# medical-genomics-group/hydra

Hardware: AMD Instinct MI355X
Metric: Gibbs markers/sec/iter (higher is better)
Workload: dtype f64

## Files before the change

### hydra_amd/capi.py

```python
import ctypes as C
import os
import numpy as np

_HERE = os.path.dirname(os.path.abspath(__file__))
LIB_PATH = os.path.join(_HERE, "libhgibbs.so")

ABI_SYMBOLS = [
    "hgibbs_last_error", "hgibbs_version", "hgibbs_create", "hgibbs_destroy", "hgibbs_comm_unique_id",
    "hgibbs_comm_init", "hgibbs_comm_init_external", "hgibbs_p2p_export", "hgibbs_p2p_import", "hgibbs_load_bed", "hgibbs_synth_bed", "hgibbs_dims", "hgibbs_get_bed",
    "hgibbs_marker_stats", "hgibbs_set_residual", "hgibbs_get_residual", "hgibbs_reduce_eps", "hgibbs_add_scalar",
    "hgibbs_update_marker", "hgibbs_dot_marker", "hgibbs_set_covariates", "hgibbs_cov_dot", "hgibbs_cov_update",
    "hydra_chain_set_covariates", "hydra_chain_gamma", "hgibbs_set_components", "hydra_chain_restore",
    "hydra_rng_to_boost_words", "hydra_rng_from_boost_words", "hgibbs_set_model", "hgibbs_set_beta", "hgibbs_get_beta",
    "hgibbs_beta_sqnorm", "hgibbs_sweep", "hgibbs_set_option", "hgibbs_last_sweep_stats", "hgibbs_stream_ceiling", "hgibbs_debug_times", "hgibbs_resident_trace", "hydra_chain_create",
    "hydra_chain_destroy", "hydra_chain_iterate", "hydra_chain_state", "hydra_chain_csv_line", "hydra_chain_order",
    "hydra_chain_last_nnz", "hgibbs_score", "hgibbs_last_score_ms", "hgibbs_ld", "hgibbs_last_ld_ms",
    "hgibbs_marker_dots", "hgibbs_last_marker_dots_ms", "hgibbs_king", "hgibbs_king_pairs", "hgibbs_king_pairs_get", "hgibbs_last_king_ms",
    "hgibbs_pca", "hgibbs_last_pca_ms",
    "hgibbs_grand_seed", "hgibbs_grand_next", "hgibbs_ars_sample", "hgibbs_w_init", "hgibbs_w_marker_stats", "hgibbs_w_set_model",
    "hgibbs_w_reduce", "hgibbs_w_refresh_vi", "hgibbs_w_get_vi", "hgibbs_w_marker_sums", "hgibbs_w_sweep", "hgibbs_w_last_sweep_stats", "hgibbs_w_ars_device_probe",
    "hgibbs_w_get_beta", "hgibbs_w_set_beta", "hydraw_chain_create", "hydraw_chain_destroy", "hydraw_chain_set_covariates",
    "hydraw_chain_reseed_ars", "hydraw_chain_iterate", "hydraw_chain_state", "hydraw_chain_gamma", "hydraw_chain_order",
    "hydraw_chain_last_nnz", "hydraw_chain_csv_line", "hydraw_chain_restore",
]


class RngState(C.Structure):
    _fields_ = [("x", C.c_uint32 * 624), ("idx", C.c_uint32)]


class SweepStats(C.Structure):
    _fields_ = [("launches", C.c_uint64), ("nnz_updates", C.c_uint64), ("device_ms", C.c_double),
                ("kernel_ms_avg", C.c_double), ("carried_columns", C.c_uint64), ("working_launches", C.c_uint64),
                ("accepted_markers", C.c_uint64), ("streamed_columns", C.c_uint64), ("tiles_per_workgroup_min", C.c_uint32),
                ("tiles_per_workgroup_max", C.c_uint32), ("engine", C.c_uint32), ("walker", C.c_uint32), ("eps_sum_drift", C.c_double),
                ("rounds", C.c_uint64), ("events", C.c_uint64), ("advances", C.c_uint64), ("chunks", C.c_uint64), ("refolds", C.c_uint64), ("pivots", C.c_uint64), ("predicted", C.c_uint64), ("shader_mhz", C.c_double),
                ("ticks", C.c_uint64 * 16), ("refill", C.c_uint32), ("reserved_", C.c_uint32)]


class PcaReport(C.Structure):
    _fields_ = [("iters_run", C.c_int32), ("m_used", C.c_uint32), ("ritz_change", C.c_double), ("resid", C.c_double * 32)]


class RestartState(C.Structure):
    _fields_ = [("iteration", C.c_uint32), ("sigmaE", C.c_double), ("mu", C.c_double),
                ("sigmaG", C.POINTER(C.c_double)), ("estPi", C.POINTER(C.c_double)), ("beta", C.POINTER(C.c_double)),
                ("components", C.POINTER(C.c_int32)), ("eps", C.POINTER(C.c_double)), ("order", C.POINTER(C.c_int32)),
                ("gamma", C.POINTER(C.c_double)), ("xI", C.POINTER(C.c_int32)), ("rng", RngState)]


class GrandState(C.Structure):
    _fields_ = [("r", C.c_int32 * 31), ("f", C.c_int32), ("b", C.c_int32)]


class WSweepStats(C.Structure):
    _fields_ = [("launches", C.c_uint64), ("nnz_updates", C.c_uint64), ("ars_draws", C.c_uint64), ("ars_evals", C.c_uint64),
                ("device_ms", C.c_double), ("sums_kernel_ms", C.c_double)]


class WModelDesc(C.Structure):
    _fields_ = [("seed", C.c_uint32), ("shuffle", C.c_int32), ("G", C.c_int32), ("K", C.c_int32),
                ("groups", C.POINTER(C.c_int32)), ("mS", C.POINTER(C.c_double)), ("quad_points", C.c_int32)]


class WRestartState(C.Structure):
    _fields_ = [("iteration", C.c_uint32), ("mu", C.c_double), ("alpha", C.c_double), ("sigmaG", C.POINTER(C.c_double)),
                ("pi", C.POINTER(C.c_double)), ("beta", C.POINTER(C.c_double)), ("components", C.POINTER(C.c_int32)),
                ("eps", C.POINTER(C.c_double)), ("order", C.POINTER(C.c_int32)), ("gamma", C.POINTER(C.c_double)),
                ("xI", C.POINTER(C.c_int32)), ("rng", RngState), ("ars_seed", C.c_uint32)]


LOGDENS_FN = C.CFUNCTYPE(C.c_double, C.c_double, C.c_void_p)


class ModelDesc(C.Structure):
    _fields_ = [("seed", C.c_uint32), ("shuffle", C.c_int32), ("G", C.c_int32), ("K", C.c_int32),
                ("groups", C.POINTER(C.c_int32)), ("mS", C.POINTER(C.c_double))]


ALLREDUCE_FN = C.CFUNCTYPE(C.c_int, C.c_void_p, C.c_void_p, C.c_size_t, C.c_int)


class HgError(RuntimeError):
    pass


_lib = None


def lib():
    global _lib
    if _lib is not None:
        return _lib
    path = os.environ.get("HGIBBS_LIB", LIB_PATH)
    if not os.path.exists(path):
        raise HgError("%s not built: run `python -c 'import __graft_entry__ as g; g.build()'` "
                      "(there is no CPU fallback)" % path)
    L = C.CDLL(path)
    vp, dp, ip = C.c_void_p, C.POINTER(C.c_double), C.POINTER(C.c_int32)
    u8p, u64p, u32p = C.POINTER(C.c_uint8), C.POINTER(C.c_uint64), C.POINTER(C.c_uint32)
    L.hgibbs_last_error.restype = C.c_char_p
    L.hgibbs_create.argtypes = [C.c_int, C.POINTER(vp)]
    L.hgibbs_destroy.argtypes = [vp]
    L.hgibbs_comm_unique_id.argtypes = [C.c_void_p]
    L.hgibbs_comm_init.argtypes = [vp, C.c_int, C.c_int, C.c_void_p]
    L.hgibbs_comm_init_external.argtypes = [vp, C.c_int, C.c_int, ALLREDUCE_FN, C.c_void_p]
    L.hgibbs_p2p_export.argtypes = [vp, C.c_void_p]
    L.hgibbs_p2p_import.argtypes = [vp, C.c_void_p]
    L.hgibbs_load_bed.argtypes = [vp, u8p, C.c_uint64, C.c_uint32, C.c_uint32, u8p, C.c_uint32, C.c_uint32, C.c_uint32]
    L.hgibbs_synth_bed.argtypes = [vp, C.c_uint32, C.c_uint32, C.c_uint32, C.c_uint32, C.c_uint64, C.c_double]
    L.hgibbs_dims.argtypes = [vp, u32p, u32p, u32p, u32p]
    L.hgibbs_get_bed.argtypes = [vp, C.c_uint32, C.c_uint32, u8p, C.c_uint64]
    L.hgibbs_marker_stats.argtypes = [vp, dp, dp, u64p, u64p, u64p]
    L.hgibbs_set_residual.argtypes = [vp, dp]
    L.hgibbs_get_residual.argtypes = [vp, dp]
    L.hgibbs_reduce_eps.argtypes = [vp, dp, dp]
    L.hgibbs_add_scalar.argtypes = [vp, C.c_double]
    L.hgibbs_update_marker.argtypes = [vp, C.c_uint32, C.c_double]
    L.hgibbs_dot_marker.argtypes = [vp, C.c_uint32, dp]
    L.hgibbs_set_covariates.argtypes = [vp, dp, C.c_int]
    L.hgibbs_cov_dot.argtypes = [vp, C.c_int, C.c_double, dp]
    L.hgibbs_cov_update.argtypes = [vp, C.c_int, C.c_double]
    L.hydra_chain_set_covariates.argtypes = [vp, dp, C.c_int]
    L.hydra_chain_gamma.argtypes = [vp, dp, ip]
    L.hgibbs_set_components.argtypes = [vp, ip]
    L.hydra_chain_restore.argtypes = [vp, C.POINTER(RestartState)]
    L.hydra_rng_to_boost_words.argtypes = [C.POINTER(RngState), u32p]
    L.hydra_rng_from_boost_words.argtypes = [u32p, C.POINTER(RngState)]
    L.hgibbs_set_model.argtypes = [vp, C.c_int, C.c_int, ip, dp, dp]
    L.hgibbs_set_beta.argtypes = [vp, dp]
    L.hgibbs_get_beta.argtypes = [vp, dp, ip, dp]
    L.hgibbs_beta_sqnorm.argtypes = [vp, dp]
    L.hgibbs_sweep.argtypes = [vp, ip, C.c_double, dp, dp, u8p, C.POINTER(RngState), ip, u64p]
    L.hgibbs_set_option.argtypes = [vp, C.c_char_p, C.c_int64]
    L.hgibbs_last_sweep_stats.argtypes = [vp, C.POINTER(SweepStats)]
    L.hgibbs_stream_ceiling.argtypes = [vp, C.c_uint64, C.c_int, dp]
    L.hgibbs_debug_times.argtypes = [vp, C.POINTER(C.c_uint64)]
    L.hgibbs_resident_trace.argtypes = [vp, C.POINTER(C.c_uint64), C.c_uint64]
    L.hydra_chain_create.argtypes = [vp, C.POINTER(ModelDesc), dp, C.POINTER(vp)]
    L.hydra_chain_destroy.argtypes = [vp]
    L.hydra_chain_iterate.argtypes = [vp]
    L.hydra_chain_state.argtypes = [vp, dp, dp, dp, dp, ip, ip, C.POINTER(RngState)]
    L.hydra_chain_csv_line.argtypes = [vp, C.c_uint32, C.c_char_p, C.c_size_t]
    L.hydra_chain_order.argtypes = [vp]
    L.hydra_chain_order.restype = ip
    L.hydra_chain_last_nnz.argtypes = [vp]
    gp = C.POINTER(GrandState)
    L.hgibbs_grand_seed.argtypes = [gp, C.c_uint32]
    L.hgibbs_grand_seed.restype = None
    L.hgibbs_grand_next.argtypes = [gp]
    L.hgibbs_grand_next.restype = C.c_int32
    L.hgibbs_ars_sample.argtypes = [dp, C.c_double, C.c_double, LOGDENS_FN, C.c_void_p, gp, dp, ip]
    L.hgibbs_w_init.argtypes = [vp, ip]
    L.hgibbs_w_marker_stats.argtypes = [vp, dp, dp, dp]
    L.hgibbs_w_set_model.argtypes = [vp, C.c_int, C.c_int, ip, dp, C.c_int]
    L.hgibbs_w_reduce.argtypes = [vp, C.c_int, C.c_int, C.c_double, C.c_double, C.c_double, dp]
    L.hgibbs_w_refresh_vi.argtypes = [vp, C.c_double]
    L.hgibbs_w_get_vi.argtypes = [vp, dp, dp]
    L.hgibbs_w_marker_sums.argtypes = [vp, C.c_uint32, C.c_double, C.c_double, dp, dp, dp]
    L.hgibbs_w_sweep.argtypes = [vp, ip, C.c_double, dp, dp, C.c_double, C.POINTER(RngState), gp, ip, dp, u64p]
    L.hgibbs_w_last_sweep_stats.argtypes = [vp, C.POINTER(WSweepStats)]
    L.hgibbs_w_ars_device_probe.argtypes = [vp, dp, C.c_double, C.c_double, C.c_uint32, C.c_uint32, dp, dp, dp]
    L.hgibbs_w_get_beta.argtypes = [vp, dp, ip]
    L.hgibbs_w_set_beta.argtypes = [vp, dp, ip]
    L.hydraw_chain_create.argtypes = [vp, C.POINTER(WModelDesc), dp, ip, C.POINTER(vp)]
    L.hydraw_chain_destroy.argtypes = [vp]
    L.hydraw_chain_set_covariates.argtypes = [vp, dp, C.c_int]
    L.hydraw_chain_reseed_ars.argtypes = [vp, C.c_uint32]
    L.hydraw_chain_iterate.argtypes = [vp]
    L.hydraw_chain_state.argtypes = [vp, dp, dp, dp, dp, ip, ip, C.POINTER(RngState), gp]
    L.hydraw_chain_gamma.argtypes = [vp, dp, ip]
    L.hydraw_chain_order.argtypes = [vp]
    L.hydraw_chain_order.restype = C.POINTER(C.c_int32)
    L.hydraw_chain_last_nnz.argtypes = [vp]
    L.hydraw_chain_last_nnz.restype = C.c_uint64
    L.hydraw_chain_csv_line.argtypes = [vp, C.c_uint32, C.c_char_p, C.c_size_t]
    L.hydraw_chain_restore.argtypes = [vp, C.POINTER(WRestartState)]
    L.hydra_chain_last_nnz.restype = C.c_uint64
    L.hgibbs_score.argtypes = [vp, C.c_int, dp, dp, dp]
    L.hgibbs_last_score_ms.argtypes = [vp, dp]
    L.hgibbs_ld.argtypes = [vp, C.c_uint32, C.c_uint32, C.c_uint32, dp, C.POINTER(C.c_int64)]
    L.hgibbs_last_ld_ms.argtypes = [vp, dp]
    L.hgibbs_marker_dots.argtypes = [vp, C.c_uint32, C.c_uint32, C.c_int, dp, dp, dp]
    L.hgibbs_last_marker_dots_ms.argtypes = [vp, dp]
    L.hgibbs_king.argtypes = [vp, C.c_uint32, C.c_uint32, C.c_uint32, C.c_uint32, C.POINTER(C.c_int32)]
    L.hgibbs_king_pairs.argtypes = [vp, C.c_double, C.POINTER(C.c_uint64)]
    L.hgibbs_king_pairs_get.argtypes = [vp, C.POINTER(C.c_uint32), C.POINTER(C.c_int32), dp]
    L.hgibbs_last_king_ms.argtypes = [vp, dp]
    L.hgibbs_pca.argtypes = [vp, C.c_int, C.c_int, C.c_int, C.c_double, dp, C.c_uint64, dp, dp, dp, C.POINTER(PcaReport)]
    L.hgibbs_last_pca_ms.argtypes = [vp, dp]
    _lib = L
    return L


def check(rc):
    if rc != 0:
        raise HgError(lib().hgibbs_last_error().decode(errors="replace"))


def _dp(a):
    return a.ctypes.data_as(C.POINTER(C.c_double))


def _ip(a):
    return a.ctypes.data_as(C.POINTER(C.c_int32))


def _u8(a):
    return a.ctypes.data_as(C.POINTER(C.c_uint8))


def _u64(a):
    return a.ctypes.data_as(C.POINTER(C.c_uint64))


class Device:

    def __init__(self, device_id=0):
        self.L = lib()
        self.h = C.c_void_p()
        check(self.L.hgibbs_create(device_id, C.byref(self.h)))
        self.M = self.n_local = self.n_global = self.row_begin = 0
        self.G = self.K = 0

    def close(self):
        if self.h:
            self.L.hgibbs_destroy(self.h)
            self.h = C.c_void_p()

    def __del__(self):
        try:
            self.close()
        except Exception:
            pass

    @staticmethod
    def unique_id():
        buf = (C.c_uint8 * 128)()
        check(lib().hgibbs_comm_unique_id(buf))
        return bytes(buf)

    def comm_init(self, nranks, rank, uid):
        buf = (C.c_uint8 * 128).from_buffer_copy(uid) if uid else None
        check(self.L.hgibbs_comm_init(self.h, nranks, rank, buf))

    def comm_init_external(self, nranks, rank, allreduce):
        def cb(user, buf, count, dtype):
            try:
                ty = C.c_double if dtype == 0 else C.c_uint64
                arr = np.ctypeslib.as_array(C.cast(buf, C.POINTER(ty)), shape=(count,))
                allreduce(arr)
                return 0
            except Exception:
                import traceback
                traceback.print_exc()
                return 1
        self._cb = ALLREDUCE_FN(cb)
        check(self.L.hgibbs_comm_init_external(self.h, nranks, rank, self._cb, None))

    def p2p_export(self):
        buf = (C.c_uint8 * 64)()
        check(self.L.hgibbs_p2p_export(self.h, buf))
        return bytes(buf)

    def p2p_import(self, handles):
        blob = b"".join(handles)
        buf = (C.c_uint8 * len(blob)).from_buffer_copy(blob)
        check(self.L.hgibbs_p2p_import(self.h, buf))

    def _dims(self):
        a, b, c, d = C.c_uint32(), C.c_uint32(), C.c_uint32(), C.c_uint32()
        check(self.L.hgibbs_dims(self.h, C.byref(a), C.byref(b), C.byref(c), C.byref(d)))
        self.n_global, self.n_local, self.M, self.row_begin = a.value, b.value, c.value, d.value

    def load_bed(self, bed, n_total, keep=None, row_begin=0, row_end=None, n_global=None):
        bed = np.ascontiguousarray(bed, dtype=np.uint8)
        M, stride = bed.shape
        kept = int(np.count_nonzero(keep)) if keep is not None else n_total
        if row_end is None:
            row_end = kept
        if n_global is None:
            n_global = kept
        kp = _u8(np.ascontiguousarray(keep, dtype=np.uint8)) if keep is not None else None
        check(self.L.hgibbs_load_bed(self.h, _u8(bed), stride, n_total, M, kp, row_begin, row_end, n_global))
        self._dims()

    def synth_bed(self, n_global, M, seed=42, missing_rate=0.0, row_begin=0, row_end=None):
        if row_end is None:
            row_end = n_global
        check(self.L.hgibbs_synth_bed(self.h, n_global, M, row_begin, row_end, seed, missing_rate))
        self._dims()

    def get_bed(self, m0=0, mcount=None):
        if mcount is None:
            mcount = self.M - m0
        out = np.zeros((mcount, (self.n_local + 3) // 4), dtype=np.uint8)
        check(self.L.hgibbs_get_bed(self.h, m0, mcount, _u8(out), out.shape[1]))
        return out

    def marker_stats(self):
        M = self.M
        mave, mstd = np.zeros(M), np.zeros(M)
        n1, n2, nm = (np.zeros(M, dtype=np.uint64) for _ in range(3))
        check(self.L.hgibbs_marker_stats(self.h, _dp(mave), _dp(mstd), _u64(n1), _u64(n2), _u64(nm)))
        return mave, mstd, n1, n2, nm

    def set_residual(self, eps):
        eps = np.ascontiguousarray(eps, dtype=np.float64)
        assert eps.shape[0] == self.n_local
        check(self.L.hgibbs_set_residual(self.h, _dp(eps)))

    def get_residual(self):
        out = np.zeros(self.n_local)
        check(self.L.hgibbs_get_residual(self.h, _dp(out)))
        return out

    def reduce_eps(self):
        s, q = C.c_double(), C.c_double()
        check(self.L.hgibbs_reduce_eps(self.h, C.byref(s), C.byref(q)))
        return s.value, q.value

    def add_scalar(self, c):
        check(self.L.hgibbs_add_scalar(self.h, c))

    def set_covariates(self, X):
        X = np.ascontiguousarray(X, dtype=np.float64)
        assert X.shape[0] == self.n_local
        check(self.L.hgibbs_set_covariates(self.h, _dp(X), X.shape[1]))

    def update_marker(self, marker, dbeta):
        check(self.L.hgibbs_update_marker(self.h, marker, dbeta))

    def dot_marker(self, marker):
        v = C.c_double()
        check(self.L.hgibbs_dot_marker(self.h, marker, C.byref(v)))
        return v.value

    def set_model(self, groups, cVa, cVaI):
        cVa = np.ascontiguousarray(cVa, dtype=np.float64)
        cVaI = np.ascontiguousarray(cVaI, dtype=np.float64)
        G, K = cVa.shape
        g = _ip(np.ascontiguousarray(groups, dtype=np.int32)) if groups is not None else None
        check(self.L.hgibbs_set_model(self.h, G, K, g, _dp(cVa), _dp(cVaI)))
        self.G, self.K = G, K

    def set_beta(self, beta):
        beta = np.ascontiguousarray(beta, dtype=np.float64)
        check(self.L.hgibbs_set_beta(self.h, _dp(beta)))

    def get_beta(self):
        beta, comp, acum = np.zeros(self.M), np.zeros(self.M, dtype=np.int32), np.zeros(self.M)
        check(self.L.hgibbs_get_beta(self.h, _dp(beta), _ip(comp), _dp(acum)))
        return beta, comp, acum

    def beta_sqnorm(self):
        out = np.zeros(self.G)
        check(self.L.hgibbs_beta_sqnorm(self.h, _dp(out)))
        return out

    def stream_ceiling(self, nbytes=2 << 30, reps=10):
        out = C.c_double()
        check(self.L.hgibbs_stream_ceiling(self.h, nbytes, reps, C.byref(out)))
        return out.value

    def set_option(self, name, value):
        check(self.L.hgibbs_set_option(self.h, name.encode(), int(value)))

    def score(self, a, o):
        a = np.ascontiguousarray(np.atleast_2d(a), dtype=np.float64)
        o = np.ascontiguousarray(np.atleast_2d(o), dtype=np.float64)
        if a.shape != o.shape or a.shape[1] != self.M:
            raise ValueError("a and o must both be (S, %d)" % self.M)
        out = np.zeros((self.n_local, a.shape[0]))
        check(self.L.hgibbs_score(self.h, a.shape[0], _dp(a), _dp(o), _dp(out)))
        return out

    def last_score_ms(self):
        v = C.c_double()
        check(self.L.hgibbs_last_score_ms(self.h, C.byref(v)))
        return v.value

    def ld(self, W, m0=0, count=None, r=True, sums=True):
        if count is None:
            count = self.M - m0
        rr = np.zeros((count, W)) if r else None
        ss = np.zeros((count, W, 4), dtype=np.int64) if sums else None
        check(self.L.hgibbs_ld(self.h, m0, count, W, _dp(rr) if r else None,
                               ss.ctypes.data_as(C.POINTER(C.c_int64)) if sums else None))
        return rr, ss

    def last_ld_ms(self):
        v = C.c_double()
        check(self.L.hgibbs_last_ld_ms(self.h, C.byref(v)))
        return v.value

    def marker_dots(self, U, m0=0, count=None, raw=False):
        U = np.ascontiguousarray(np.atleast_2d(U), dtype=np.float64)
        if U.shape[1] != self.n_local:
            raise ValueError("U must be (K, %d)" % self.n_local)
        if count is None:
            count = self.M - m0
        K = U.shape[0]
        out = np.zeros((count, K))
        rr = np.zeros((count, K, 2)) if raw else None
        check(self.L.hgibbs_marker_dots(self.h, m0, count, K, _dp(U), _dp(out), _dp(rr) if raw else None))
        return (out, rr) if raw else out

    def last_marker_dots_ms(self):
        v = C.c_double()
        check(self.L.hgibbs_last_marker_dots_ms(self.h, C.byref(v)))
        return v.value

    def king(self, a0=0, acount=None, b0=0, bcount=None):
        if acount is None:
            acount = self.n_local - a0
        if bcount is None:
            bcount = self.n_local - b0
        out = np.zeros((acount, bcount, 5), dtype=np.int32)
        check(self.L.hgibbs_king(self.h, a0, acount, b0, bcount, out.ctypes.data_as(C.POINTER(C.c_int32))))
        return out

    def king_pairs(self, cutoff):
        n = C.c_uint64()
        check(self.L.hgibbs_king_pairs(self.h, float(cutoff), C.byref(n)))
        P = n.value
        ab = np.zeros((P, 2), dtype=np.uint32)
        cnt = np.zeros((P, 5), dtype=np.int32)
        kin = np.zeros(P)
        check(self.L.hgibbs_king_pairs_get(self.h, ab.ctypes.data_as(C.POINTER(C.c_uint32)), cnt.ctypes.data_as(C.POINTER(C.c_int32)), _dp(kin)))
        return ab, cnt, kin

    def last_king_ms(self):
        v = C.c_double()
        check(self.L.hgibbs_last_king_ms(self.h, C.byref(v)))
        return v.value

    def pca(self, K, L=None, iters=20, tol=1e-10, Q0=None, seed=1, loadings=False):
        if L is None:
            L = min(32, (K + 8 + 7) // 8 * 8)
        q = None
        if Q0 is not None:
            q = np.ascontiguousarray(Q0, dtype=np.float64)
            if q.shape != (L, self.n_local):
                raise ValueError("Q0 must be (%d, %d)" % (L, self.n_local))
        kk = max(int(K), 0)
        val = np.zeros(kk)
        pcs = np.zeros((kk, self.n_local))
        ld = np.zeros((kk, self.M)) if loadings else None
        rep = PcaReport()
        check(self.L.hgibbs_pca(self.h, int(K), int(L), int(iters), float(tol), _dp(q) if q is not None else None, int(seed) & (2 ** 64 - 1),
                                _dp(val), _dp(pcs), _dp(ld) if loadings else None, C.byref(rep)))
        return val, pcs, ld, {"iters_run": rep.iters_run, "m_used": rep.m_used, "ritz_change": rep.ritz_change,
                              "resid": np.array(rep.resid[:kk], dtype=np.float64)}

    def last_pca_ms(self):
        v = (C.c_double * 4)()
        check(self.L.hgibbs_last_pca_ms(self.h, v))
        return [v[i] for i in range(4)]

    def debug_times(self):
        t = (C.c_uint64 * 48)()
        check(self.L.hgibbs_debug_times(self.h, t))
        return [int(x) for x in t]

    def sweep(self, order, sigmaE, sigmaG, estPi, adaV, rng):
        order = np.ascontiguousarray(order, dtype=np.int32)
        sigmaG = np.ascontiguousarray(sigmaG, dtype=np.float64)
        estPi = np.ascontiguousarray(estPi, dtype=np.float64)
        adaV = np.ascontiguousarray(adaV, dtype=np.uint8)
        cass = np.zeros((self.G, self.K), dtype=np.int32)
        nnz = C.c_uint64()
        check(self.L.hgibbs_sweep(self.h, _ip(order), float(sigmaE), _dp(sigmaG), _dp(estPi), _u8(adaV), C.byref(rng),
                                  _ip(cass), C.byref(nnz)))
        return cass, nnz.value

    def resident_trace(self):
        out = np.zeros((10, 4096), dtype=np.uint64)
        check(self.L.hgibbs_resident_trace(self.h, out.ctypes.data_as(C.POINTER(C.c_uint64)), out.size))
        return out

    def sweep_stats(self):
        s = SweepStats()
        check(self.L.hgibbs_last_sweep_stats(self.h, C.byref(s)))
        return {"launches": s.launches, "nnz_updates": s.nnz_updates, "device_ms": s.device_ms,
                "kernel_ms_avg": s.kernel_ms_avg, "carried_columns": s.carried_columns, "working_launches": s.working_launches,
                "accepted_markers": s.accepted_markers, "streamed_columns": s.streamed_columns,
                "tiles_per_workgroup_min": s.tiles_per_workgroup_min, "tiles_per_workgroup_max": s.tiles_per_workgroup_max,
                "engine": s.engine, "walker": s.walker, "refill": s.refill, "eps_sum_drift": s.eps_sum_drift, "rounds": s.rounds, "events": s.events,
                "advances": s.advances, "chunks": s.chunks, "refolds": s.refolds, "pivots": s.pivots, "predicted": s.predicted, "shader_mhz": s.shader_mhz, "ticks": list(s.ticks)}


class Chain:

    def __init__(self, dev, y, mS=None, groups=None, seed=1222, shuffle=1):
        self.dev = dev
        self.L = dev.L
        if mS is None:
            mS = np.array([[0.0, 0.0001, 0.001, 0.01]])
        self.mS = np.ascontiguousarray(mS, dtype=np.float64)
        self.G, self.K = self.mS.shape
        self.groups = None if groups is None else np.ascontiguousarray(groups, dtype=np.int32)
        y = np.ascontiguousarray(y, dtype=np.float64)
        assert y.shape[0] == dev.n_global
        d = ModelDesc(seed, shuffle, self.G, self.K, _ip(self.groups) if self.groups is not None else None, _dp(self.mS))
        self.h = C.c_void_p()
        check(self.L.hydra_chain_create(dev.h, C.byref(d), _dp(y), C.byref(self.h)))
        dev.G, dev.K = self.G, self.K

    def __del__(self):
        try:
            if self.h:
                self.L.hydra_chain_destroy(self.h)
        except Exception:
            pass

    def set_covariates(self, X):
        X = np.ascontiguousarray(X, dtype=np.float64)
        assert X.shape[0] == self.dev.n_global
        self.C = X.shape[1]
        check(self.L.hydra_chain_set_covariates(self.h, _dp(X), self.C))

    def gamma(self):
        g, xi = np.zeros(self.C), np.zeros(self.C, dtype=np.int32)
        check(self.L.hydra_chain_gamma(self.h, _dp(g), _ip(xi)))
        return g, xi

    def iterate(self):
        check(self.L.hydra_chain_iterate(self.h))

    def state(self):
        G, K = self.G, self.K
        sE, mu = C.c_double(), C.c_double()
        sG, pi = np.zeros(G), np.zeros((G, K))
        m0, cass = np.zeros(G, dtype=np.int32), np.zeros((G, K), dtype=np.int32)
        rng = RngState()
        check(self.L.hydra_chain_state(self.h, C.byref(sE), C.byref(mu), _dp(sG), _dp(pi), _ip(m0), _ip(cass), C.byref(rng)))
        return {"sigmaE": sE.value, "mu": mu.value, "sigmaG": sG, "estPi": pi, "m0": m0, "cass": cass,
                "rng_x": np.array(rng.x, dtype=np.uint32), "rng_idx": int(rng.idx)}

    def order(self):
        return np.ctypeslib.as_array(self.L.hydra_chain_order(self.h), shape=(self.dev.M,)).copy()

    def rng_words(self):
        rng = RngState()
        check(self.L.hydra_chain_state(self.h, None, None, None, None, None, None, C.byref(rng)))
        out = np.zeros(624, dtype=np.uint32)
        check(self.L.hydra_rng_to_boost_words(C.byref(rng), out.ctypes.data_as(C.POINTER(C.c_uint32))))
        return out

    def restore(self, iteration, sigmaE, mu, sigmaG, estPi, beta, components, eps, order, rng_words, gamma=None, xI=None):
        f64 = lambda a: np.ascontiguousarray(a, dtype=np.float64)
        i32 = lambda a: np.ascontiguousarray(a, dtype=np.int32)
        keep = [f64(sigmaG), f64(estPi), f64(beta), i32(components), f64(eps), i32(order)]
        st = RestartState()
        st.iteration, st.sigmaE, st.mu = iteration, sigmaE, mu
        st.sigmaG, st.estPi, st.beta = _dp(keep[0]), _dp(keep[1]), _dp(keep[2])
        st.components, st.eps, st.order = _ip(keep[3]), _dp(keep[4]), _ip(keep[5])
        if gamma is not None:
            keep += [f64(gamma), i32(xI)]
            st.gamma, st.xI = _dp(keep[6]), _ip(keep[7])
        w = np.ascontiguousarray(rng_words, dtype=np.uint32)
        check(self.L.hydra_rng_from_boost_words(w.ctypes.data_as(C.POINTER(C.c_uint32)), C.byref(st.rng)))
        check(self.L.hydra_chain_restore(self.h, C.byref(st)))

    def last_nnz(self):
        return int(self.L.hydra_chain_last_nnz(self.h))

    def csv_line(self, it):
        buf = C.create_string_buffer(50000)
        n = self.L.hydra_chain_csv_line(self.h, it, buf, 50000)
        return buf.raw[:n].decode()


def ars_sample(logdens, xinit, xl, xr, grand):
    L = lib()
    cb = LOGDENS_FN(lambda x, _d: logdens(x))
    xi = np.ascontiguousarray(xinit, dtype=np.float64)
    out, ne = C.c_double(0.0), C.c_int(0)
    err = L.hgibbs_ars_sample(_dp(xi), xl, xr, cb, None, C.byref(grand), C.byref(out), C.byref(ne))
    return err, out.value, ne.value


class BwOps:

    def __init__(self, dev, failure):
        self.dev, self.L = dev, dev.L
        self.fail = np.ascontiguousarray(failure, dtype=np.int32)
        assert self.fail.shape[0] == dev.n_global
        check(self.L.hgibbs_w_init(dev.h, _ip(self.fail)))

    def marker_stats(self):
        M = self.dev.M
        a, b, c = np.zeros(M), np.zeros(M), np.zeros(M)
        check(self.L.hgibbs_w_marker_stats(self.dev.h, _dp(a), _dp(b), _dp(c)))
        return a, b, c

    def set_model(self, mS, groups=None, quad=9):
        mS = np.ascontiguousarray(mS, dtype=np.float64)
        self.G, self.K = mS.shape
        g = None if groups is None else np.ascontiguousarray(groups, dtype=np.int32)
        check(self.L.hgibbs_w_set_model(self.dev.h, self.G, self.K, _ip(g) if g is not None else None, _dp(mS), quad))

    def reduce(self, kind, col=0, p0=0.0, p1=0.0, p2=0.0):
        out = C.c_double()
        check(self.L.hgibbs_w_reduce(self.dev.h, kind, col, p0, p1, p2, C.byref(out)))
        return out.value

    def refresh_vi(self, alpha):
        check(self.L.hgibbs_w_refresh_vi(self.dev.h, alpha))

    def get_vi(self):
        v, s = np.zeros(self.dev.n_local), C.c_double()
        check(self.L.hgibbs_w_get_vi(self.dev.h, _dp(v), C.byref(s)))
        return v, s.value

    def marker_sums(self, marker, beta_old, alpha):
        a, b, c = C.c_double(), C.c_double(), C.c_double()
        check(self.L.hgibbs_w_marker_sums(self.dev.h, marker, beta_old, alpha, C.byref(a), C.byref(b), C.byref(c)))
        return a.value, b.value, c.value

    def get_beta(self):
        b, c = np.zeros(self.dev.M), np.zeros(self.dev.M, dtype=np.int32)
        check(self.L.hgibbs_w_get_beta(self.dev.h, _dp(b), _ip(c)))
        return b, c

    def sweep_stats(self):
        st = WSweepStats()
        check(self.L.hgibbs_w_last_sweep_stats(self.dev.h, C.byref(st)))
        return {f: getattr(st, f) for f, _ in st._fields_}


class BwChain:

    def __init__(self, dev, y, failure, mS=None, groups=None, seed=1222, shuffle=1, quad=9):
        self.dev, self.L = dev, dev.L
        if mS is None:
            mS = np.array([[0.0, 0.001, 0.01]])
        self.mS = np.ascontiguousarray(mS, dtype=np.float64)
        self.G, self.K = self.mS.shape
        self.groups = None if groups is None else np.ascontiguousarray(groups, dtype=np.int32)
        y = np.ascontiguousarray(y, dtype=np.float64)
        self.fail = np.ascontiguousarray(failure, dtype=np.int32)
        assert y.shape[0] == dev.n_global and self.fail.shape[0] == dev.n_global
        d = WModelDesc(seed, shuffle, self.G, self.K, _ip(self.groups) if self.groups is not None else None, _dp(self.mS), quad)
        self.h = C.c_void_p()
        self.C = 0
        check(self.L.hydraw_chain_create(dev.h, C.byref(d), _dp(y), _ip(self.fail), C.byref(self.h)))

    def __del__(self):
        try:
            if self.h:
                self.L.hydraw_chain_destroy(self.h)
        except Exception:
            pass

    def set_covariates(self, X):
        X = np.ascontiguousarray(X, dtype=np.float64)
        self.C = X.shape[1]
        check(self.L.hydraw_chain_set_covariates(self.h, _dp(X), self.C))

    def reseed_ars(self, seed):
        check(self.L.hydraw_chain_reseed_ars(self.h, seed))

    def rng_words(self):
        st = self.state()
        rng = RngState()
        rng.x[:] = list(st["rng_x"])
        rng.idx = st["rng_idx"]
        out = np.zeros(624, dtype=np.uint32)
        check(self.L.hydra_rng_to_boost_words(C.byref(rng), out.ctypes.data_as(C.POINTER(C.c_uint32))))
        return out

    def restore(self, iteration, mu, alpha, sigmaG, pi, beta, components, eps, order, rng_words, ars_seed, gamma=None, xI=None):
        f64 = lambda a: np.ascontiguousarray(a, dtype=np.float64)
        i32 = lambda a: np.ascontiguousarray(a, dtype=np.int32)
        keep = [f64(sigmaG), f64(pi), f64(beta), i32(components), f64(eps), i32(order)]
        st = WRestartState()
        st.iteration, st.mu, st.alpha, st.ars_seed = iteration, mu, alpha, ars_seed
        st.sigmaG, st.pi, st.beta = _dp(keep[0]), _dp(keep[1]), _dp(keep[2])
        st.components, st.eps, st.order = _ip(keep[3]), _dp(keep[4]), _ip(keep[5])
        if gamma is not None:
            keep += [f64(gamma), i32(xI)]
            st.gamma, st.xI = _dp(keep[6]), _ip(keep[7])
        w = np.ascontiguousarray(rng_words, dtype=np.uint32)
        check(self.L.hydra_rng_from_boost_words(w.ctypes.data_as(C.POINTER(C.c_uint32)), C.byref(st.rng)))
        check(self.L.hydraw_chain_restore(self.h, C.byref(st)))

    def iterate(self):
        check(self.L.hydraw_chain_iterate(self.h))

    def state(self):
        G, K = self.G, self.K
        mu, alpha = C.c_double(), C.c_double()
        sG, pi = np.zeros(G), np.zeros((G, K))
        m0, cass = np.zeros(G, dtype=np.int32), np.zeros((G, K), dtype=np.int32)
        rng, gr = RngState(), GrandState()
        check(self.L.hydraw_chain_state(self.h, C.byref(mu), C.byref(alpha), _dp(sG), _dp(pi), _ip(m0), _ip(cass), C.byref(rng), C.byref(gr)))
        return {"mu": mu.value, "alpha": alpha.value, "sigmaG": sG, "pi": pi, "m0": m0, "cass": cass,
                "rng_x": np.array(rng.x, dtype=np.uint32), "rng_idx": int(rng.idx), "grand": gr}

    def gamma(self):
        g, xi = np.zeros(self.C), np.zeros(self.C, dtype=np.int32)
        check(self.L.hydraw_chain_gamma(self.h, _dp(g), _ip(xi)))
        return g, xi

    def beta(self):
        b, c = np.zeros(self.dev.M), np.zeros(self.dev.M, dtype=np.int32)
        check(self.L.hgibbs_w_get_beta(self.dev.h, _dp(b), _ip(c)))
        return b, c

    def order(self):
        return np.ctypeslib.as_array(self.L.hydraw_chain_order(self.h), shape=(self.dev.M,)).copy()

    def last_nnz(self):
        return int(self.L.hydraw_chain_last_nnz(self.h))

    def sweep_stats(self):
        st = WSweepStats()
        check(self.L.hgibbs_w_last_sweep_stats(self.dev.h, C.byref(st)))
        return {f: getattr(st, f) for f, _ in st._fields_}

    def csv_line(self, it):
        buf = C.create_string_buffer(50000)
        n = self.L.hydraw_chain_csv_line(self.h, it, buf, 50000)
        return buf.raw[:n].decode()
```

### hydra_amd/csrc/hg_rng.h

```cpp
#pragma once

#include <math.h>
#include <stdint.h>
#if !defined(__HIP_DEVICE_COMPILE__)
#include <vector>
#endif

#include "hg_zig_tables.h"

#if defined(__HIP__)
#include <hip/hip_runtime.h>
#define HG_HD __host__ __device__ __forceinline__
#else
#define HG_HD inline
#endif

namespace hg {

constexpr int MT_N = 624;
constexpr int MT_M = 397;

HG_HD uint32_t mt_temper(uint32_t z)
{
    z ^= (z >> 11);
    z ^= (z << 7) & 0x9d2c5680u;
    z ^= (z << 15) & 0xefc60000u;
    z ^= (z >> 18);
    return z;
}

HG_HD uint32_t mt_mix(uint32_t cur, uint32_t nxt, uint32_t far)
{
    uint32_t y = (cur & 0x80000000u) | (nxt & 0x7fffffffu);
    return far ^ (y >> 1) ^ ((y & 1u) ? 0x9908b0dfu : 0u);
}

struct Mt {
    uint32_t* x;
    uint32_t idx;
    HG_HD void seed(uint32_t s)
    {
        x[0] = s;
        for (uint32_t i = 1; i < MT_N; ++i) x[i] = 1812433253u * (x[i - 1] ^ (x[i - 1] >> 30)) + i;
        idx = MT_N;
    }
    HG_HD void twist()
    {
        for (int i = 0; i < MT_N; ++i) x[i] = mt_mix(x[i], x[(i + 1) % MT_N], x[(i + MT_M) % MT_N]);
        idx = 0;
    }
    HG_HD uint32_t next()
    {
        if (idx >= MT_N) twist();
        return mt_temper(x[idx++]);
    }
};

struct ZigTables {
    const double* nx;
    const double* ny;
    const double* ex;
    const double* ey;
};

template <class Gen>
HG_HD double unif01(Gen& g)
{
    return (double)g.next() * (1.0 / 4294967296.0);
}

template <class Gen>
HG_HD double int_float_pair(Gen& g, int& bucket)
{
    uint32_t u1 = g.next();
    bucket = (int)(u1 & 0xffu);
    double r = (double)(u1 >> 8) * (1.0 / 16777216.0);
    uint32_t u2 = g.next();
    r += (double)(u2 & 0x1fffffffu);
    r *= (1.0 / 536870912.0);
    return r;
}

template <class Gen, class Tab>
HG_HD double unit_exponential(Gen& g, const Tab& t)
{
    double shift = 0.0;
    for (;;) {
        int i;
        double r = int_float_pair(g, i);
        double x = r * t.ex[i];
        if (x < t.ex[i + 1]) return shift + x;
        if (i == 0) {
            shift += t.ex[1];
        } else {
            double y01 = unif01(g);
            double y = t.ey[i] + y01 * (t.ey[i + 1] - t.ey[i]);
            double y_above_ubound = (t.ex[i] - t.ex[i + 1]) * y01 - (t.ex[i] - x);
            double y_above_lbound = y - (t.ey[i + 1] + (t.ex[i + 1] - x) * t.ey[i + 1]);
            if (y_above_ubound < 0 && (y_above_lbound < 0 || y < exp(-x))) return x + shift;
        }
    }
}

template <class Gen, class Tab>
HG_HD double unit_normal(Gen& g, const Tab& t)
{
    for (;;) {
        int i;
        double r = int_float_pair(g, i);
        int sign = (i & 1) * 2 - 1;
        i >>= 1;
        double x = r * t.nx[i];
        if (x < t.nx[i + 1]) return x * sign;
        if (i == 0) {
            const double tail_start = t.nx[1];
            for (;;) {
                double xt = unit_exponential(g, t) / tail_start;
                double yt = unit_exponential(g, t) / 1.0;
                if (2 * yt > xt * xt) return (xt + tail_start) * sign;
            }
        }
        double y01 = unif01(g);
        double y = t.ny[i] + y01 * (t.ny[i + 1] - t.ny[i]);
        double y_above_ubound, y_above_lbound;
        if (t.nx[i] >= 1) {
            y_above_ubound = (t.nx[i] - t.nx[i + 1]) * y01 - (t.nx[i] - x);
            y_above_lbound = y - (t.ny[i] + (t.nx[i] - x) * t.ny[i] * t.nx[i]);
        } else {
            y_above_lbound = (t.nx[i] - t.nx[i + 1]) * y01 - (t.nx[i] - x);
            y_above_ubound = y - (t.ny[i] + (t.nx[i] - x) * t.ny[i] * t.nx[i]);
        }
        if (y_above_ubound < 0 && (y_above_lbound < 0 || y < exp(-(x * x / 2)))) return x * sign;
    }
}

template <class Gen, class Tab>
HG_HD double norm_rng_sd(Gen& g, const Tab& t, double mean, double sigma)
{
    return unit_normal(g, t) * sigma + mean;
}

inline ZigTables host_tables() { return ZigTables{HG_ZIG_NORMAL_X, HG_ZIG_NORMAL_Y, HG_ZIG_EXP_X, HG_ZIG_EXP_Y}; }

inline double norm_rng(Mt& g, double mean, double sigma2)
{
    ZigTables t = host_tables();
    return norm_rng_sd(g, t, mean, sqrt(sigma2));
}

inline double rgamma(Mt& g, double alpha, double beta)
{
    ZigTables t = host_tables();
    if (alpha == 1.0) {
        return unit_exponential(g, t) / 1.0 * beta;
    } else if (alpha > 1.0) {
        const double pi = 3.14159265358979323846;
        for (;;) {
            double y = tan(pi * unif01(g));
            double x = sqrt(2.0 * alpha - 1.0) * y + alpha - 1.0;
            if (x <= 0.0) continue;
            if (unif01(g) > (1.0 + y * y) * exp((alpha - 1.0) * log(x / (alpha - 1.0)) - sqrt(2.0 * alpha - 1.0) * y))
                continue;
            return x * beta;
        }
    } else {
        const double p = exp(1.0) / (alpha + exp(1.0));
        for (;;) {
            double u = unif01(g);
            double y = unit_exponential(g, t) / 1.0;
            double x, q;
            if (u < p) {
                x = exp(-y / alpha);
                q = p * exp(-x);
            } else {
                x = 1.0 + y;
                q = p + (1.0 - p) * pow(x, alpha - 1.0);
            }
            if (u >= q) continue;
            return x * beta;
        }
    }
}

inline double inv_gamma_rng(Mt& g, double shape, double scale) { return 1.0 / rgamma(g, shape, 1.0 / scale); }
inline double inv_scaled_chisq_rng(Mt& g, double dof, double scale) { return inv_gamma_rng(g, 0.5 * dof, 0.5 * dof * scale); }
inline double beta_rng(Mt& g, double a, double b)
{
    double x = rgamma(g, a, 1.0);
    double y = rgamma(g, b, 1.0);
    return x / (x + y);
}
inline void dirichlet_rng(Mt& g, const double* alpha, int len, double* out)
{
    double s = 0.0;
    for (int i = 0; i < len; ++i) out[i] = rgamma(g, alpha[i], 1.0);
    for (int i = 0; i < len; ++i) s += out[i];
    for (int i = 0; i < len; ++i) out[i] /= s;
}

inline void mt_to_boost_words(const uint32_t* x, uint32_t idx, uint32_t* out )
{
    const uint32_t UP = 0x80000000u, LO = 0x7fffffffu, A = 0x9908b0dfu;
    if (idx > (uint32_t)MT_N) idx = MT_N;
    for (uint32_t j = 0; j < idx; ++j) out[j + MT_N - idx] = x[j];
    if (idx == (uint32_t)MT_N) return;
    auto unmix = [&](uint32_t y) {
        if (y & UP) return ((y ^ A) << 1) | 1u;
        return y << 1;
    };
    std::vector<uint32_t> w(MT_N + 1, 0u);
    w[MT_N] = x[0];
    uint32_t have_low_of = MT_N;
    (void)have_low_of;
    for (int k = MT_N - 1; k >= (int)idx - 1 && k >= 0; --k) {
        const uint32_t far = (k + MT_M < MT_N) ? w[k + MT_M] : x[k + MT_M - MT_N];
        const uint32_t y = unmix(x[k] ^ far);
        if (k + 1 < MT_N) w[k + 1] = (w[k + 1] & UP) | (y & LO);
        w[k] = (w[k] & LO) | (y & UP);
    }
    for (uint32_t k = idx; k < (uint32_t)MT_N; ++k) out[k - idx] = w[k];
}

template <class T>
inline void shuffle_libstdcxx6(T* first, size_t n, Mt& g)
{
    const uint64_t urngrange = 0xffffffffull;
    for (size_t i = 1; i < n; ++i) {
        const uint64_t uerange = (uint64_t)i + 1;
        const uint64_t scaling = urngrange / uerange, past = uerange * scaling;
        uint64_t ret;
        do ret = g.next();
        while (ret >= past);
        ret /= scaling;
        const T t = first[i];
        first[i] = first[ret];
        first[ret] = t;
    }
}

}
```

### hydra_amd/csrc/hgibbs.hip

```cpp
#include <hip/hip_runtime.h>
#include <rccl/rccl.h>

#include <algorithm>
#include <atomic>
#include <chrono>
#include <thread>
#include <cmath>
#include <cstdarg>
#include <cstdio>
#include <cstdlib>
#include <cstring>
#include <string>
#include <vector>

#include "../../include/hgibbs.h"
#include "hg_kernels.h"
#include "hg_sweep.hip.h"
#include "hg_resident.hip.h"

using namespace hg;

static thread_local std::string g_err;

static int fail(const char* fmt, ...)
{
    char buf[1024];
    va_list ap;
    va_start(ap, fmt);
    vsnprintf(buf, sizeof buf, fmt, ap);
    va_end(ap);
    g_err = buf;
    return 1;
}

#define HIP_TRY(expr)                                                                          \
    do {                                                                                       \
        hipError_t e_ = (expr);                                                                \
        if (e_ != hipSuccess) return fail("%s:%d %s -> %s", __FILE__, __LINE__, #expr, hipGetErrorString(e_)); \
    } while (0)

#define NCCL_TRY(expr)                                                                          \
    do {                                                                                        \
        ncclResult_t r_ = (expr);                                                               \
        if (r_ != ncclSuccess) return fail("%s:%d %s -> %s", __FILE__, __LINE__, #expr, ncclGetErrorString(r_)); \
    } while (0)

extern "C" void hgibbs_set_error_(const char* msg) { g_err = msg; }

struct BwState;
static void bw_free(BwState* b);

struct hgibbs_ctx {
    int device = 0;
    int num_cu = 256;
    BwState* bw = nullptr;
    hipStream_t stream = nullptr;
    hipEvent_t ev0 = nullptr, ev1 = nullptr;

    int nranks = 1, rank = 0;
    ncclComm_t comm = nullptr;
    hgibbs_allreduce_fn ext_fn = nullptr;
    void* ext_user = nullptr;
    unsigned char* mbox = nullptr;
    void* peer_base[MAX_RANKS] = {};
    bool p2p_ready = false, p2p_enabled = true;
    uint64_t batch_seq = 0;

    uint32_t n_global = 0, n_local = 0, n_pad = 0, M = 0, row_begin = 0;
    uint64_t stride = 0;
    uint8_t* bed = nullptr;
    double* eps[2] = {nullptr, nullptr};
    uint32_t eps_cur = 0;
    double *mave = nullptr, *mstd = nullptr;
    unsigned long long* counts = nullptr;
    bool have_stats = false;
    bool any_missing = false;
    int gram_missing = -1;

    double* covX = nullptr;
    int C = 0;

    int G = 0, K = 0;
    int32_t* groups = nullptr;
    std::vector<int32_t> groups_host;
    std::vector<double> cVa, cVaI;
    double* beta = nullptr;
    int32_t* comp = nullptr;
    double* acum = nullptr;

    int32_t* order = nullptr;
    uint8_t* adaV = nullptr;
    double *s_mave = nullptr, *s_mstd = nullptr, *s_bold = nullptr;
    int32_t* s_ga = nullptr;
    uint32_t* pred = nullptr;
    uint32_t* pred_cnt = nullptr;
    unsigned long long* dbg = nullptr;
    bool debug_timing = false;
    bool w_kernel_timing = false;
    int32_t* cass = nullptr;
    double* tables = nullptr;
    uint32_t* mt = nullptr;
    double* zig = nullptr;
    SweepDesc* desc = nullptr;
    SweepDesc* desc_host = nullptr;
    double* partials = nullptr;
    double* totals = nullptr;
    double* carry = nullptr;
    double* ahead_raw = nullptr;
    double* apartials = nullptr;
    uint32_t* aticket = nullptr;
    int ahead = -1;
    int carry_on = -1;
    uint32_t* ticket = nullptr;
    double* sums = nullptr;
    double* scratch = nullptr;
    size_t scratch_n = 0;
    double* scratch_host = nullptr;
    double* beta_host = nullptr;

    uint32_t batch = 0;
    uint32_t cols_per_group = 4;
    int chunk = 0;
    uint32_t slices = 0;
    uint32_t ext_limit = 256;
    uint32_t max_seg = 0;
    bool gram = true;
    bool use_graph = false;
    bool force_split = false;

    int engine = 0;
    bool res_all_ada = false;
    unsigned long long res_sweep_id = 0;
    bool engine_pinned = false;
    uint32_t window = 0;
    uint32_t res_cus = 0;
    int res_walker = 0;
    bool res_attr_set[20] = {};
    bool res_dead = false;
    uint32_t res_probed_w = 0;
    unsigned long long res_probe_id = 0;
    bool res_not_resident = false;
    int res_early = 24;
    int res_announce = 1;
    int res_wend = 1;
    int res_walker2_ranks = 1;
    double eps_abs_bound = 0.0;
    int res_refill = 0;
    int res_pivots = 0;
    unsigned char* res_acc = nullptr;
    ResMsg* res_msg = nullptr;
    ResState* res_state = nullptr;
    ResState* res_state_host = nullptr;
    ResParams* res_params = nullptr;
    ResParams* res_params_host = nullptr;
    unsigned long long* res_progress = nullptr;
    unsigned long long* res_progress_host = nullptr;
    hipStream_t aux_stream = nullptr;
    unsigned long long* res_trace = nullptr;
    double res_timeout_s = 2.0;
    double res_deadline_s = 0.0;

    hgibbs_sweep_stats stats{};
    int score_sp = 0;
    int score_ranges = 0;
    double score_ms = 0.0;
    int ld_split = 0;
    double ld_ms = 0.0;
    int mdots_split = 0;
    double mdots_ms = 0.0;
    int king_split = 0;
    double king_ms = 0.0;
    double pca_ms[5] = {0, 0, 0, 0, 0};
    std::vector<uint32_t> king_ab;
    std::vector<int32_t> king_counts;
    std::vector<double> king_kin;
};

static int ensure_scratch(hgibbs_ctx* h, size_t n)
{
    if (h->scratch_n >= n) return 0;
    if (h->scratch) HIP_TRY(hipFree(h->scratch));
    HIP_TRY(hipMalloc(&h->scratch, n * sizeof(double)));
    h->scratch_n = n;
    return 0;
}

static constexpr size_t RES_GACC_BYTES = (size_t)2 * RS_NSH * RS_GROW * 4, RES_RACC_BYTES = (size_t)RS_RSH * RS_RB * 8, RES_RCNT_BYTES = (size_t)RS_RSH * RS_CROW * 4, RES_PACC_BYTES = (size_t)RS_RSH * RS_RB * 2 * 8;
static constexpr size_t RES_RACC2_OFF = RES_GACC_BYTES + RES_RACC_BYTES + RES_RCNT_BYTES + RES_PACC_BYTES, RES_GACC64_BYTES = (size_t)2 * RS_NSH * RS_GROW * 8;
static constexpr size_t RES_ACC_BYTES = RES_RACC2_OFF + RES_RACC_BYTES + RES_GACC64_BYTES;
static constexpr size_t MBOX_DATA_BYTES = (size_t)2 * MAX_RANKS * ROWS_CAP * sizeof(double);
static constexpr size_t MBOX_BATCH_BYTES = MBOX_DATA_BYTES + (size_t)2 * MAX_RANKS * sizeof(unsigned long long);
static constexpr size_t MBOX_RES_OFF = (MBOX_BATCH_BYTES + 4095) / 4096 * 4096;
static constexpr size_t MBOX_BYTES = MBOX_RES_OFF + RX_BYTES;

static int bulk_allreduce(hgibbs_ctx* h, void* dptr, size_t count, int dtype)
{
    if (h->nranks <= 1 && !h->comm) return 0;
    if (h->comm) {
        NCCL_TRY(ncclAllReduce(dptr, dptr, count, dtype == 0 ? ncclDouble : ncclUint64, ncclSum, h->comm, h->stream));
        return 0;
    }
    if (!h->ext_fn) return fail("multi-rank handle without a transport: call hgibbs_comm_init or hgibbs_comm_init_external");
    std::vector<unsigned char> buf(count * 8);
    HIP_TRY(hipMemcpyAsync(buf.data(), dptr, buf.size(), hipMemcpyDeviceToHost, h->stream));
    HIP_TRY(hipStreamSynchronize(h->stream));
    if (h->ext_fn(h->ext_user, buf.data(), count, dtype)) return fail("external all-reduce callback failed");
    HIP_TRY(hipMemcpyAsync(dptr, buf.data(), buf.size(), hipMemcpyHostToDevice, h->stream));
    HIP_TRY(hipStreamSynchronize(h->stream));
    return 0;
}

namespace {

__host__ __device__ inline uint64_t mix64(uint64_t z)
{
    z += 0x9e3779b97f4a7c15ull;
    z = (z ^ (z >> 30)) * 0xbf58476d1ce4e5b9ull;
    z = (z ^ (z >> 27)) * 0x94d049bb133111ebull;
    return z ^ (z >> 31);
}

__global__ void k_synth_bed(uint8_t* bed, uint64_t stride, uint32_t n_local, uint32_t row_begin, uint32_t marker0,
                            uint64_t seed, uint32_t miss_thr)
{
    const uint32_t marker = marker0 + blockIdx.y;
    const uint64_t b = (uint64_t)blockIdx.x * blockDim.x + threadIdx.x;
    if (b >= stride) return;
    const uint32_t up = (uint32_t)(mix64(seed ^ (0xA5A5A5A5ull + (uint64_t)marker * 0x100000001b3ull)) >> 32);
    const double p = 0.01 + 0.49 * ((double)up * (1.0 / 4294967296.0));
    const double q0 = (1.0 - p) * (1.0 - p);
    const double q1 = q0 + 2.0 * p * (1.0 - p);
    const uint32_t t0 = (uint32_t)(q0 * 4294967296.0);
    const uint32_t t1 = (uint32_t)(q1 * 4294967296.0);
    uint32_t byte = 0;
    for (int s = 0; s < 4; ++s) {
        const uint64_t il = b * 4 + s;
        uint32_t code = GC_MISS;
        if (il < n_local) {
            const uint64_t ig = (uint64_t)row_begin + il;
            const uint64_t hsh = mix64(seed + (uint64_t)marker * 0x9E3779B1ull + ig * 0xD1B54A32D192ED03ull);
            const uint32_t ug = (uint32_t)(hsh >> 32), um = (uint32_t)hsh;
            if (um < miss_thr) code = GC_MISS;
            else code = (ug < t0) ? GC_G0 : ((ug < t1) ? GC_G1 : GC_G2);
        }
        byte |= code << (2 * s);
    }
    bed[(uint64_t)marker * stride + b] = (uint8_t)byte;
}

__global__ void k_fix_padding(uint8_t* bed, uint64_t stride, uint32_t n_local, uint32_t M)
{
    const uint32_t marker = blockIdx.x * blockDim.x + threadIdx.x;
    if (marker >= M) return;
    const uint32_t bfirst = n_local >> 2;
    if ((n_local & 3u) && bfirst < stride) {
        uint8_t v = bed[(uint64_t)marker * stride + bfirst];
        for (uint32_t s = n_local & 3u; s < 4; ++s) v = (uint8_t)((v & ~(3u << (2 * s))) | (1u << (2 * s)));
        bed[(uint64_t)marker * stride + bfirst] = v;
    }
}

__global__ void k_recode_bed(uint32_t* __restrict__ bed, uint64_t ndwords)
{
    const uint64_t stride = (uint64_t)gridDim.x * blockDim.x;
    for (uint64_t i = (uint64_t)blockIdx.x * blockDim.x + threadIdx.x; i < ndwords; i += stride) bed[i] = recode_plink_to_device(bed[i]);
}

__global__ void k_compact_bed(const uint8_t* __restrict__ src, uint64_t src_stride, const uint32_t* __restrict__ src_idx,
                              uint8_t* __restrict__ dst, uint64_t dst_stride, uint32_t n_local, uint32_t mcount)
{
    const uint32_t marker = blockIdx.y;
    const uint64_t b = (uint64_t)blockIdx.x * blockDim.x + threadIdx.x;
    if (b >= dst_stride || marker >= mcount) return;
    uint32_t byte = 0;
    for (int s = 0; s < 4; ++s) {
        const uint64_t il = b * 4 + s;
        uint32_t code = 1u;
        if (il < n_local) {
            const uint32_t i = src_idx[il];
            code = (src[(uint64_t)marker * src_stride + (i >> 2)] >> (2 * (i & 3u))) & 3u;
        }
        byte |= code << (2 * s);
    }
    dst[(uint64_t)marker * dst_stride + b] = (uint8_t)byte;
}

__global__ __launch_bounds__(BLOCK) void k_counts(const uint8_t* __restrict__ bed, uint64_t stride, uint32_t n_pad,
                                                  uint32_t n_local, unsigned long long* __restrict__ counts, uint32_t M)
{
    __shared__ unsigned int sh[3][BLOCK_WAVES];
    const uint32_t marker = blockIdx.x;
    const uint32_t* col = reinterpret_cast<const uint32_t*>(bed + (uint64_t)marker * stride);
    const uint32_t nw = (uint32_t)(stride >> 2);
    unsigned int c1 = 0, c2 = 0, cm = 0;
    for (uint32_t i = threadIdx.x; i < nw; i += BLOCK) {
        uint32_t m1, m2, mm;
        code_masks(col[i], m1, m2, mm);
        c1 += __popc(m1);
        c2 += __popc(m2);
        cm += __popc(mm);
    }
    for (int off = 32; off >= 1; off >>= 1) {
        c1 += __shfl_xor(c1, off, 64);
        c2 += __shfl_xor(c2, off, 64);
        cm += __shfl_xor(cm, off, 64);
    }
    const int lane = threadIdx.x & 63, wave = threadIdx.x >> 6;
    if (lane == 0) {
        sh[0][wave] = c1;
        sh[1][wave] = c2;
        sh[2][wave] = cm;
    }
    __syncthreads();
    if (threadIdx.x == 0) {
        unsigned long long t1 = 0, t2 = 0, tm = 0;
        for (int w = 0; w < BLOCK_WAVES; ++w) {
            t1 += sh[0][w];
            t2 += sh[1][w];
            tm += sh[2][w];
        }
        counts[3ull * marker] = t1;
        counts[3ull * marker + 1] = t2;
        counts[3ull * marker + 2] = tm - (unsigned long long)(n_pad - n_local);
    }
}

__global__ void k_stats(const unsigned long long* __restrict__ counts, uint32_t N, double* mave, double* mstd, uint32_t M)
{
    const uint32_t i = blockIdx.x * blockDim.x + threadIdx.x;
    if (i >= M) return;
    const double n1 = (double)counts[3ull * i], n2 = (double)counts[3ull * i + 1], nm = (double)counts[3ull * i + 2];
    const double dN = (double)N;
    const double av = (n1 + 2.0 * n2) / (dN - nm);
    const double tmp1 = n1 * (1.0 - av) * (1.0 - av);
    const double tmp2 = n2 * (2.0 - av) * (2.0 - av);
    const unsigned long long n0 = (unsigned long long)N - counts[3ull * i] - counts[3ull * i + 1] - counts[3ull * i + 2];
    const double tmp0 = (double)n0 * (0.0 - av) * (0.0 - av);
    mave[i] = av;
    mstd[i] = sqrt((double)(N - 1) / (tmp0 + tmp1 + tmp2));
}

__global__ void k_gather_meta(const int32_t* __restrict__ order, const double* __restrict__ mave, const double* __restrict__ mstd,
                              const double* __restrict__ beta, const int32_t* __restrict__ groups, const uint8_t* __restrict__ adaV,
                              const unsigned long long* __restrict__ counts, double* s_mave, double* s_mstd, double* s_bold, int32_t* s_ga, uint32_t M)
{
    const uint32_t j = blockIdx.x * blockDim.x + threadIdx.x;
    if (j >= M) return;
    const int m = order[j];
    s_mave[j] = mave[m];
    s_mstd[j] = mstd[m];
    s_bold[j] = beta[m];
    s_ga[j] = groups[m] | (adaV[m] ? 0x40000000 : 0) | (counts[3ull * m + 2] ? 0x20000000 : 0);
}

constexpr uint32_t PRED_CHUNK = 4096;
__global__ __launch_bounds__(256) void k_pred_count(const double* __restrict__ s_bold, uint32_t M, uint32_t* cnt)
{
    __shared__ uint32_t wsum[4];
    const uint32_t base = blockIdx.x * PRED_CHUNK;
    uint32_t n = 0;
    for (uint32_t i = 0; i < PRED_CHUNK / 256; ++i) {
        const uint32_t j = base + i * 256 + threadIdx.x;
        n += (uint32_t)__popcll(__ballot(j < M && s_bold[j] != 0.0));
    }
    if ((threadIdx.x & 63) == 0) wsum[threadIdx.x >> 6] = n;
    __syncthreads();
    if (threadIdx.x == 0) cnt[blockIdx.x] = wsum[0] + wsum[1] + wsum[2] + wsum[3];
}
__global__ __launch_bounds__(1024) void k_pred_scan(uint32_t* cnt, uint32_t nchunk)
{
    __shared__ uint32_t tot[1024];
    const uint32_t per = (nchunk + 1023u) / 1024u, lo = threadIdx.x * per;
    uint32_t s = 0;
    for (uint32_t i = lo; i < lo + per && i < nchunk; ++i) s += cnt[i];
    tot[threadIdx.x] = s;
    __syncthreads();
    if (threadIdx.x == 0) {
        uint32_t run = 0;
        for (int t = 0; t < 1024; ++t) {
            const uint32_t v = tot[t];
            tot[t] = run;
            run += v;
        }
        cnt[nchunk] = run;
    }
    __syncthreads();
    uint32_t run = tot[threadIdx.x];
    for (uint32_t i = lo; i < lo + per && i < nchunk; ++i) {
        const uint32_t v = cnt[i];
        cnt[i] = run;
        run += v;
    }
}
__global__ __launch_bounds__(256) void k_pred_scatter(const double* __restrict__ s_bold, uint32_t M, const uint32_t* __restrict__ cnt, uint32_t nchunk, uint32_t* pred)
{
    __shared__ uint32_t wsum[4];
    const uint32_t base = blockIdx.x * PRED_CHUNK;
    const int lane = threadIdx.x & 63, wave = threadIdx.x >> 6;
    uint32_t run = cnt[blockIdx.x];
    for (uint32_t i = 0; i < PRED_CHUNK / 256; ++i) {
        const uint32_t j = base + i * 256 + threadIdx.x;
        const bool f = j < M && s_bold[j] != 0.0;
        const unsigned long long m = __ballot(f);
        __syncthreads();
        if (lane == 0) wsum[wave] = (uint32_t)__popcll(m);
        __syncthreads();
        uint32_t before = 0;
        for (int w = 0; w < wave; ++w) before += wsum[w];
        if (f) pred[run + before + (uint32_t)__popcll(m & ((1ull << lane) - 1ull))] = j;
        run += wsum[0] + wsum[1] + wsum[2] + wsum[3];
    }
    if (blockIdx.x == 0 && threadIdx.x < 16) pred[cnt[nchunk] + threadIdx.x] = 0xffffffffu;
}

__global__ void k_set_eps(double* eps, const double* __restrict__ src, uint32_t n_local, uint32_t n_pad)
{
    const uint32_t i = blockIdx.x * blockDim.x + threadIdx.x;
    if (i >= n_pad) return;
    eps[eps_pos(i)] = (i < n_local) ? src[i] : 0.0;
}

__global__ void k_get_eps(const double* __restrict__ eps, double* dst, uint32_t n_local)
{
    const uint32_t i = blockIdx.x * blockDim.x + threadIdx.x;
    if (i >= n_local) return;
    dst[i] = eps[eps_pos(i)];
}

__global__ void k_add_scalar(double* eps, double c, uint32_t n_local, uint32_t n_pad)
{
    const uint32_t i = blockIdx.x * blockDim.x + threadIdx.x;
    if (i >= n_local) return;
    const uint32_t p = eps_pos(i);
    eps[p] = eps[p] + c;
}

__global__ __launch_bounds__(BLOCK) void k_reduce_eps(const double* __restrict__ eps, uint32_t n_pad, double* partial)
{
    __shared__ double sh[3][BLOCK_WAVES];
    const int lane = threadIdx.x & 63, wave = threadIdx.x >> 6;
    const uint32_t tile = blockIdx.x * BLOCK_WAVES + wave;
    double e[IPT];
    load_eps16(eps, tile, lane, e);
    double s = 0.0, q = 0.0, o = 0.0;
#pragma unroll
    for (int i = 0; i < IPT; ++i) {
        const double e2 = e[i] * e[i], e4 = e2 * e2;
        s += e[i];
        q += e2;
        o += e4 * e4;
    }
    s = wave_sum(s);
    q = wave_sum(q);
    o = wave_sum(o);
    if (lane == 0) {
        sh[0][wave] = s;
        sh[1][wave] = q;
        sh[2][wave] = o;
    }
    __syncthreads();
    if (threadIdx.x == 0) {
        double ts = 0.0, tq = 0.0, to = 0.0;
        for (int w = 0; w < BLOCK_WAVES; ++w) {
            ts += sh[0][w];
            tq += sh[1][w];
            to += sh[2][w];
        }
        partial[3 * blockIdx.x] = ts;
        partial[3 * blockIdx.x + 1] = tq;
        partial[3 * blockIdx.x + 2] = to;
    }
}

__global__ __launch_bounds__(BLOCK) void k_final_sum(const double* __restrict__ partial, uint32_t nblk, uint32_t rows, double* out)
{
    __shared__ double sh[BLOCK_WAVES];
    const int lane = threadIdx.x & 63, wave = threadIdx.x >> 6;
    for (uint32_t r = 0; r < rows; ++r) {
        double v = 0.0;
        for (uint32_t b = threadIdx.x; b < nblk; b += BLOCK) v += partial[(size_t)b * rows + r];
        v = wave_sum(v);
        if (lane == 0) sh[wave] = v;
        __syncthreads();
        if (threadIdx.x == 0) {
            double t = 0.0;
            for (int w = 0; w < BLOCK_WAVES; ++w) t += sh[w];
            out[r] = t;
        }
        __syncthreads();
    }
}

__global__ __launch_bounds__(BLOCK) void k_dot_one(const uint8_t* __restrict__ bed, uint64_t stride, uint32_t marker,
                                                   const double* __restrict__ eps, double* partial)
{
    __shared__ double sh[4][BLOCK_WAVES];
    const int lane = threadIdx.x & 63, wave = threadIdx.x >> 6;
    const uint32_t tile = blockIdx.x * BLOCK_WAVES + wave;
    double e[IPT];
    load_eps16(eps, tile, lane, e);
    const uint32_t w = *reinterpret_cast<const uint32_t*>(bed + (size_t)marker * stride + ((size_t)tile << 8) + (lane << 2));
    uint32_t m1, m2, mm;
    code_masks(w, m1, m2, mm);
    double s1 = 0.0, s2 = 0.0, sm = 0.0, sa = 0.0;
#pragma unroll
    for (int s = 0; s < IPT; ++s) {
        s1 += mask_f64(e[s], ((int)(m1 << (31 - 2 * s))) >> 31);
        s2 += mask_f64(e[s], ((int)(m2 << (31 - 2 * s))) >> 31);
        sm += mask_f64(e[s], ((int)(mm << (31 - 2 * s))) >> 31);
        sa += e[s];
    }
    s1 = wave_sum(s1);
    s2 = wave_sum(s2);
    sm = wave_sum(sm);
    sa = wave_sum(sa);
    if (lane == 0) {
        sh[0][wave] = s1;
        sh[1][wave] = s2;
        sh[2][wave] = sm;
        sh[3][wave] = sa;
    }
    __syncthreads();
    if (threadIdx.x < 4) {
        double t = 0.0;
        for (int wv = 0; wv < BLOCK_WAVES; ++wv) t += sh[threadIdx.x][wv];
        partial[4 * blockIdx.x + threadIdx.x] = t;
    }
}

__global__ void k_set_cov(double* dst, const double* __restrict__ X, uint32_t n_local, uint32_t n_pad, int C, int c)
{
    const uint32_t i = blockIdx.x * blockDim.x + threadIdx.x;
    if (i >= n_pad) return;
    dst[eps_pos(i)] = (i < n_local) ? X[(size_t)i * C + c] : 0.0;
}

__global__ __launch_bounds__(BLOCK) void k_cov_dot(const double* __restrict__ x, const double* __restrict__ eps, double g, double* partial)
{
    __shared__ double sh[BLOCK_WAVES];
    const int lane = threadIdx.x & 63, wave = threadIdx.x >> 6;
    const uint32_t tile = blockIdx.x * BLOCK_WAVES + wave;
    double e[IPT], xv[IPT];
    load_eps16(eps, tile, lane, e);
    load_eps16(x, tile, lane, xv);
    double s = 0.0;
#pragma unroll
    for (int i = 0; i < IPT; ++i) s += xv[i] * (e[i] + g * xv[i]);
    s = wave_sum(s);
    if (lane == 0) sh[wave] = s;
    __syncthreads();
    if (threadIdx.x == 0) {
        double t = 0.0;
        for (int w = 0; w < BLOCK_WAVES; ++w) t += sh[w];
        partial[blockIdx.x] = t;
    }
}

__global__ __launch_bounds__(BLOCK) void k_cov_update(const double* __restrict__ x, double* eps, double dgam)
{
    const int lane = threadIdx.x & 63, wave = threadIdx.x >> 6;
    const uint32_t tile = blockIdx.x * BLOCK_WAVES + wave;
    double e[IPT], xv[IPT];
    load_eps16(eps, tile, lane, e);
    load_eps16(x, tile, lane, xv);
#pragma unroll
    for (int i = 0; i < IPT; ++i) e[i] = e[i] + dgam * xv[i];
    store_eps16(eps, tile, lane, e);
}

__global__ __launch_bounds__(BLOCK) void k_update_one(const uint8_t* __restrict__ bed, uint64_t stride, uint32_t marker,
                                                      double* eps, double v0, double v1, double v2)
{
    const int lane = threadIdx.x & 63, wave = threadIdx.x >> 6;
    const uint32_t tile = blockIdx.x * BLOCK_WAVES + wave;
    double e[IPT];
    load_eps16(eps, tile, lane, e);
    const uint32_t w = *reinterpret_cast<const uint32_t*>(bed + (size_t)marker * stride + ((size_t)tile << 8) + (lane << 2));
    apply_update16(w, v0, v1, v2, e);
    store_eps16(eps, tile, lane, e);
}

}

extern "C" {

const char* hgibbs_last_error(void) { return g_err.c_str(); }
int hgibbs_version(void) { return 1; }

int hgibbs_create(int device_id, hgibbs_t* out)
{
    if (!out) return fail("hgibbs_create: null out");
    int ndev = 0;
    HIP_TRY(hipGetDeviceCount(&ndev));
    if (ndev <= 0) return fail("hgibbs_create: no HIP device (this library has no CPU fallback)");
    if (device_id < 0 || device_id >= ndev) return fail("hgibbs_create: device %d out of range (%d devices)", device_id, ndev);
    HIP_TRY(hipSetDevice(device_id));
    hipDeviceProp_t prop;
    HIP_TRY(hipGetDeviceProperties(&prop, device_id));
    if (std::strncmp(prop.gcnArchName, "gfx950", 6) != 0)
        return fail("hgibbs_create: device %d is %s, this library is built for gfx950 only", device_id, prop.gcnArchName);
    hgibbs_ctx* h = new hgibbs_ctx();
    h->device = device_id;
    h->num_cu = prop.multiProcessorCount;
    HIP_TRY(hipStreamCreateWithFlags(&h->stream, hipStreamNonBlocking));
    HIP_TRY(hipEventCreate(&h->ev0));
    HIP_TRY(hipEventCreate(&h->ev1));
    HIP_TRY(hipMalloc(&h->mt, MT_N * sizeof(uint32_t)));
    HIP_TRY(hipMalloc(&h->zig, (129 + 129 + 257 + 257) * sizeof(double)));
    HIP_TRY(hipMemcpy(h->zig, HG_ZIG_NORMAL_X, 129 * sizeof(double), hipMemcpyHostToDevice));
    HIP_TRY(hipMemcpy(h->zig + 129, HG_ZIG_NORMAL_Y, 129 * sizeof(double), hipMemcpyHostToDevice));
    HIP_TRY(hipMemcpy(h->zig + 258, HG_ZIG_EXP_X, 257 * sizeof(double), hipMemcpyHostToDevice));
    HIP_TRY(hipMemcpy(h->zig + 515, HG_ZIG_EXP_Y, 257 * sizeof(double), hipMemcpyHostToDevice));
    HIP_TRY(hipMalloc(&h->desc, sizeof(SweepDesc) + sizeof(SweepCounters)));
    HIP_TRY(hipHostMalloc(&h->desc_host, sizeof(SweepDesc) + sizeof(SweepCounters)));
    HIP_TRY(hipMalloc(&h->ticket, (16 + MAX_GROUPS + 256) * sizeof(uint32_t)));
    HIP_TRY(hipMemset(h->ticket, 0, (16 + MAX_GROUPS + 256) * sizeof(uint32_t)));
    HIP_TRY(hipMalloc(&h->totals, (size_t)ROWS_CAP * sizeof(double)));
    HIP_TRY(hipMalloc(&h->carry, (size_t)MAX_BATCH * sizeof(double)));
    HIP_TRY(hipMalloc(&h->ahead_raw, (size_t)2 * AHEAD_MAX * 2 * sizeof(double)));
    HIP_TRY(hipMalloc(&h->apartials, (size_t)S_CAP * 2 * AHEAD_MAX * sizeof(double)));
    HIP_TRY(hipMalloc(&h->aticket, (AHEAD_MAX / 2 + 4) * sizeof(uint32_t)));
    HIP_TRY(hipMemset(h->aticket, 0, (AHEAD_MAX / 2 + 4) * sizeof(uint32_t)));
    HIP_TRY(hipMalloc(&h->sums, (NROW * MAX_BATCH + 1) * sizeof(double)));
    HIP_TRY(hipMalloc(&h->dbg, 48 * sizeof(unsigned long long)));
    HIP_TRY(hipMemset(h->dbg, 0, 48 * sizeof(unsigned long long)));
    HIP_TRY(hipHostMalloc(&h->scratch_host, 4096 * sizeof(double)));
    HIP_TRY(hipMalloc(&h->res_acc, RES_ACC_BYTES));
    HIP_TRY(hipMalloc(&h->res_msg, RS_MSG * sizeof(ResMsg)));
    HIP_TRY(hipMalloc(&h->res_state, sizeof(ResState)));
    HIP_TRY(hipHostMalloc(&h->res_state_host, sizeof(ResState)));
    HIP_TRY(hipMalloc(&h->res_params, sizeof(ResParams)));
    HIP_TRY(hipHostMalloc(&h->res_params_host, sizeof(ResParams)));
    HIP_TRY(hipMalloc(&h->res_progress, 16 * sizeof(unsigned long long)));
    HIP_TRY(hipHostMalloc(&h->res_progress_host, 16 * sizeof(unsigned long long)));
    HIP_TRY(hipStreamCreateWithFlags(&h->aux_stream, hipStreamNonBlocking));
    HIP_TRY(hipMalloc(&h->res_trace, (size_t)10 * RS_TRACE * sizeof(unsigned long long)));
    HIP_TRY(hipMemset(h->res_trace, 0, (size_t)10 * RS_TRACE * sizeof(unsigned long long)));
    *out = h;
    return 0;
}

int hgibbs_destroy(hgibbs_t h)
{
    if (!h) return 0;
    (void)hipSetDevice(h->device);
    (void)hipStreamSynchronize(h->stream);
    if (h->comm) ncclCommDestroy(h->comm);
    bw_free(h->bw);
    for (int r = 0; r < MAX_RANKS; ++r)
        if (h->peer_base[r] && h->peer_base[r] != h->mbox) (void)hipIpcCloseMemHandle(h->peer_base[r]);
    if (h->mbox) (void)hipFree(h->mbox);
    void* ptrs[] = {h->bed, h->eps[0], h->eps[1], h->mave, h->mstd, h->counts, h->groups, h->beta, h->comp, h->acum, h->order,
                    h->adaV, h->covX, h->s_mave, h->s_mstd, h->s_bold, h->s_ga, h->pred, h->pred_cnt, h->dbg, h->cass, h->tables, h->mt, h->zig, h->desc, h->partials, h->totals, h->ticket, h->sums, h->scratch, h->carry, h->ahead_raw, h->apartials, h->aticket, h->res_acc, h->res_msg, h->res_state, h->res_trace};
    for (void* p : ptrs)
        if (p) (void)hipFree(p);
    if (h->desc_host) (void)hipHostFree(h->desc_host);
    if (h->scratch_host) (void)hipHostFree(h->scratch_host);
    if (h->res_state_host) (void)hipHostFree(h->res_state_host);
    if (h->res_params) (void)hipFree(h->res_params);
    if (h->res_params_host) (void)hipHostFree(h->res_params_host);
    if (h->res_progress) (void)hipFree(h->res_progress);
    if (h->res_progress_host) (void)hipHostFree(h->res_progress_host);
    if (h->aux_stream) (void)hipStreamDestroy(h->aux_stream);
    if (h->beta_host) (void)hipHostFree(h->beta_host);
    (void)hipEventDestroy(h->ev0);
    (void)hipEventDestroy(h->ev1);
    (void)hipStreamDestroy(h->stream);
    delete h;
    return 0;
}

int hgibbs_comm_unique_id(void* id128)
{
    static_assert(sizeof(ncclUniqueId) == 128, "ncclUniqueId is 128 bytes");
    ncclUniqueId id;
    NCCL_TRY(ncclGetUniqueId(&id));
    std::memcpy(id128, &id, sizeof id);
    return 0;
}

int hgibbs_comm_init(hgibbs_t h, int nranks, int rank, const void* id128)
{
    if (!h) return fail("null handle");
    if (nranks < 1 || rank < 0 || rank >= nranks) return fail("hgibbs_comm_init: bad rank %d of %d", rank, nranks);
    h->nranks = nranks;
    h->rank = rank;
    if (nranks == 1 && !id128) return 0;
    HIP_TRY(hipSetDevice(h->device));
    ncclUniqueId id;
    std::memcpy(&id, id128, sizeof id);
    NCCL_TRY(ncclCommInitRank(&h->comm, nranks, id, rank));
    return 0;
}

extern "C" int hgibbs_comm_init_external(hgibbs_t h, int nranks, int rank, hgibbs_allreduce_fn fn, void* user)
{
    if (!h) return fail("null handle");
    if (nranks < 1 || rank < 0 || rank >= nranks) return fail("hgibbs_comm_init_external: bad rank %d of %d", rank, nranks);
    if (nranks > 1 && !fn) return fail("hgibbs_comm_init_external: null callback");
    h->nranks = nranks;
    h->rank = rank;
    h->ext_fn = fn;
    h->ext_user = user;
    return 0;
}

extern "C" int hgibbs_p2p_export(hgibbs_t h, void* handle64)
{
    static_assert(sizeof(hipIpcMemHandle_t) == 64, "hipIpcMemHandle_t is 64 bytes");
    if (!h || !handle64) return fail("hgibbs_p2p_export: null argument");
    HIP_TRY(hipSetDevice(h->device));
    if (!h->mbox) {
        void* p = nullptr;
        hipError_t e = hipExtMallocWithFlags(&p, MBOX_BYTES, hipDeviceMallocUncached);
        hipIpcMemHandle_t probe;
        if (e != hipSuccess || hipIpcGetMemHandle(&probe, p) != hipSuccess) {
            (void)hipGetLastError();
            if (e == hipSuccess) (void)hipFree(p);
            HIP_TRY(hipMalloc(&p, MBOX_BYTES));
        }
        h->mbox = (unsigned char*)p;
        HIP_TRY(hipMemset(h->mbox, 0, MBOX_BYTES));
    }
    hipIpcMemHandle_t hd;
    HIP_TRY(hipIpcGetMemHandle(&hd, h->mbox));
    std::memcpy(handle64, &hd, sizeof hd);
    return 0;
}

extern "C" int hgibbs_p2p_import(hgibbs_t h, const void* handles)
{
    if (!h || !handles) return fail("hgibbs_p2p_import: null argument");
    if (h->nranks < 2) return fail("hgibbs_p2p_import: initialise the ranks first (hgibbs_comm_init / hgibbs_comm_init_external)");
    if (h->nranks > MAX_RANKS) return fail("hgibbs_p2p_import: at most %d ranks", MAX_RANKS);
    if (!h->mbox) return fail("hgibbs_p2p_import: call hgibbs_p2p_export first");
    HIP_TRY(hipSetDevice(h->device));
    for (int r = 0; r < h->nranks; ++r) {
        if (r == h->rank) {
            h->peer_base[r] = h->mbox;
            continue;
        }
        hipIpcMemHandle_t hd;
        std::memcpy(&hd, (const unsigned char*)handles + (size_t)r * 64, sizeof hd);
        void* p = nullptr;
        HIP_TRY(hipIpcOpenMemHandle(&p, hd, hipIpcMemLazyEnablePeerAccess));
        h->peer_base[r] = p;
    }
    h->p2p_ready = true;
    return 0;
}

static int alloc_problem(hgibbs_ctx* h, uint32_t n_global, uint32_t n_local, uint32_t M, uint32_t row_begin)
{
    if (n_local == 0 || M == 0) return fail("empty problem: n_local=%u M=%u", n_local, M);
    if (h->bed) return fail("data already loaded on this handle");
    h->n_global = n_global;
    h->n_local = n_local;
    h->M = M;
    h->row_begin = row_begin;
    h->n_pad = (uint32_t)(((uint64_t)n_local + BLOCK_IND - 1) / BLOCK_IND * BLOCK_IND);
    h->stride = h->n_pad / 4;
    HIP_TRY(hipMalloc(&h->bed, (size_t)M * h->stride));
    for (int b = 0; b < 2; ++b) {
        HIP_TRY(hipMalloc(&h->eps[b], (size_t)h->n_pad * sizeof(double)));
        HIP_TRY(hipMemsetAsync(h->eps[b], 0, (size_t)h->n_pad * sizeof(double), h->stream));
    }
    HIP_TRY(hipMalloc(&h->mave, (size_t)M * sizeof(double)));
    HIP_TRY(hipMalloc(&h->mstd, (size_t)M * sizeof(double)));
    HIP_TRY(hipMalloc(&h->counts, (size_t)M * 3 * sizeof(unsigned long long)));
    HIP_TRY(hipMalloc(&h->beta, (size_t)M * sizeof(double)));
    HIP_TRY(hipMalloc(&h->comp, (size_t)M * sizeof(int32_t)));
    HIP_TRY(hipMalloc(&h->acum, (size_t)M * sizeof(double)));
    HIP_TRY(hipMalloc(&h->order, (size_t)M * sizeof(int32_t)));
    HIP_TRY(hipMalloc(&h->adaV, (size_t)M));
    HIP_TRY(hipMalloc(&h->s_mave, (size_t)M * sizeof(double)));
    HIP_TRY(hipMalloc(&h->s_mstd, (size_t)M * sizeof(double)));
    HIP_TRY(hipMalloc(&h->s_bold, (size_t)M * sizeof(double)));
    HIP_TRY(hipMalloc(&h->s_ga, (size_t)M * sizeof(int32_t)));
    HIP_TRY(hipMalloc(&h->pred, ((size_t)M + 16) * sizeof(uint32_t)));
    HIP_TRY(hipMalloc(&h->pred_cnt, ((size_t)(M + PRED_CHUNK - 1) / PRED_CHUNK + 1) * sizeof(uint32_t)));
    HIP_TRY(hipMalloc(&h->groups, (size_t)M * sizeof(int32_t)));
    HIP_TRY(hipMemsetAsync(h->beta, 0, (size_t)M * sizeof(double), h->stream));
    HIP_TRY(hipMemsetAsync(h->comp, 0, (size_t)M * sizeof(int32_t), h->stream));
    HIP_TRY(hipMemsetAsync(h->acum, 0, (size_t)M * sizeof(double), h->stream));
    HIP_TRY(hipMemsetAsync(h->groups, 0, (size_t)M * sizeof(int32_t), h->stream));
    const uint32_t nblk_x = h->n_pad / BLOCK_IND;
    HIP_TRY(hipMalloc(&h->partials, (size_t)PROWS_CAP * S_CAP * sizeof(double)));
    if (ensure_scratch(h, (size_t)nblk_x * 4 + 4096)) return 1;
    h->eps_cur = 0;
    h->have_stats = false;
    return 0;
}

int hgibbs_load_bed(hgibbs_t h, const uint8_t* bed_host, uint64_t stride_in, uint32_t n_total, uint32_t M,
                    const uint8_t* keep_host, uint32_t row_begin, uint32_t row_end, uint32_t n_global)
{
    if (!h || !bed_host) return fail("hgibbs_load_bed: null argument");
    if (row_end <= row_begin) return fail("hgibbs_load_bed: empty row range");
    if (stride_in < ((uint64_t)n_total + 3) / 4) return fail("hgibbs_load_bed: stride_in %llu < ceil(%u/4)", (unsigned long long)stride_in, n_total);
    HIP_TRY(hipSetDevice(h->device));
    const uint32_t n_local = row_end - row_begin;
    std::vector<uint32_t> kept;
    if (!keep_host) {
        if (row_end > n_total) return fail("hgibbs_load_bed: row_end %u > n_total %u", row_end, n_total);
        if (row_begin & 3u) return fail("hgibbs_load_bed: row_begin %u must be a multiple of 4", row_begin);
    } else {
        kept.reserve(n_total);
        for (uint32_t i = 0; i < n_total; ++i)
            if (keep_host[i]) kept.push_back(i);
        if (row_end > kept.size()) return fail("hgibbs_load_bed: row_end %u > kept individuals %zu", row_end, kept.size());
    }
    if (n_global < 2) return fail("hgibbs_load_bed: n_global must be at least 2");
    if (alloc_problem(h, n_global, n_local, M, row_begin)) return 1;
    HIP_TRY(hipMemsetAsync(h->bed, 0x55, (size_t)M * h->stride, h->stream));

    if (!keep_host) {
        const size_t width = ((size_t)n_local + 3) / 4;
        HIP_TRY(hipMemcpy2DAsync(h->bed, h->stride, bed_host + (row_begin >> 2), stride_in, width, M, hipMemcpyHostToDevice, h->stream));
        k_fix_padding<<<(M + 255) / 256, 256, 0, h->stream>>>(h->bed, h->stride, n_local, M);
        HIP_TRY(hipGetLastError());
    } else {
        struct Staging {
            uint32_t* idx = nullptr;
            uint8_t* src = nullptr;
            ~Staging()
            {
                if (src) (void)hipFree(src);
                if (idx) (void)hipFree(idx);
            }
        } st;
        HIP_TRY(hipMalloc(&st.idx, (size_t)n_local * sizeof(uint32_t)));
        HIP_TRY(hipMemcpyAsync(st.idx, kept.data() + row_begin, (size_t)n_local * sizeof(uint32_t), hipMemcpyHostToDevice, h->stream));
        const uint32_t slab = (uint32_t)std::max<uint64_t>(1, std::min<uint64_t>(M, (256ull << 20) / std::max<uint64_t>(1, stride_in)));
        HIP_TRY(hipMalloc(&st.src, (size_t)slab * stride_in));
        for (uint32_t m0 = 0; m0 < M; m0 += slab) {
            const uint32_t mc = std::min(slab, M - m0);
            HIP_TRY(hipMemcpyAsync(st.src, bed_host + (size_t)m0 * stride_in, (size_t)mc * stride_in, hipMemcpyHostToDevice, h->stream));
            dim3 grid((uint32_t)((h->stride + 255) / 256), mc);
            k_compact_bed<<<grid, 256, 0, h->stream>>>(st.src, stride_in, st.idx, h->bed + (size_t)m0 * h->stride, h->stride, n_local, mc);
            HIP_TRY(hipGetLastError());
        }
        HIP_TRY(hipStreamSynchronize(h->stream));
    }
    k_recode_bed<<<4096, 256, 0, h->stream>>>(reinterpret_cast<uint32_t*>(h->bed), (uint64_t)M * h->stride / 4);
    HIP_TRY(hipGetLastError());
    HIP_TRY(hipStreamSynchronize(h->stream));
    return 0;
}

int hgibbs_synth_bed(hgibbs_t h, uint32_t n_global, uint32_t M, uint32_t row_begin, uint32_t row_end, uint64_t seed,
                     double missing_rate)
{
    if (!h) return fail("null handle");
    if (row_end <= row_begin || row_end > n_global) return fail("hgibbs_synth_bed: bad row range");
    HIP_TRY(hipSetDevice(h->device));
    if (alloc_problem(h, n_global, row_end - row_begin, M, row_begin)) return 1;
    double mr = missing_rate < 0 ? 0 : (missing_rate > 1 ? 1 : missing_rate);
    const uint32_t miss_thr = (uint32_t)std::min(4294967295.0, mr * 4294967296.0);
    for (uint32_t m0 = 0; m0 < M; m0 += 32768) {
        const uint32_t mc = std::min<uint32_t>(32768, M - m0);
        dim3 grid((uint32_t)((h->stride + 255) / 256), mc);
        k_synth_bed<<<grid, 256, 0, h->stream>>>(h->bed, h->stride, h->n_local, row_begin, m0, seed, miss_thr);
        HIP_TRY(hipGetLastError());
    }
    HIP_TRY(hipStreamSynchronize(h->stream));
    return 0;
}

int hgibbs_dims(hgibbs_t h, uint32_t* n_global, uint32_t* n_local, uint32_t* M, uint32_t* row_begin)
{
    if (!h) return fail("hgibbs_dims: null handle");
    if (n_global) *n_global = h->n_global;
    if (n_local) *n_local = h->n_local;
    if (M) *M = h->M;
    if (row_begin) *row_begin = h->row_begin;
    return 0;
}

int hgibbs_get_bed(hgibbs_t h, uint32_t m0, uint32_t mcount, uint8_t* out_host, uint64_t out_stride)
{
    if (!h || !h->bed) return fail("hgibbs_get_bed: no data");
    if ((uint64_t)m0 + mcount > h->M) return fail("hgibbs_get_bed: marker range out of bounds");
    HIP_TRY(hipSetDevice(h->device));
    const size_t width = ((size_t)h->n_local + 3) / 4;
    if (out_stride < width) return fail("hgibbs_get_bed: out_stride too small");
    HIP_TRY(hipMemcpy2D(out_host, out_stride, h->bed + (size_t)m0 * h->stride, h->stride, width, mcount, hipMemcpyDeviceToHost));
    for (uint32_t m = 0; m < mcount; ++m) {
        uint8_t* row = out_host + (size_t)m * out_stride;
        for (size_t b = 0; b < width; ++b) row[b] = (uint8_t)recode_device_to_plink(row[b]);
    }
    return 0;
}

static int compute_stats(hgibbs_ctx* h)
{
    if (h->have_stats) return 0;
    k_counts<<<h->M, BLOCK, 0, h->stream>>>(h->bed, h->stride, h->n_pad, h->n_local, h->counts, h->M);
    HIP_TRY(hipGetLastError());
    if (bulk_allreduce(h, h->counts, (size_t)h->M * 3, 1)) return 1;
    k_stats<<<(h->M + 255) / 256, 256, 0, h->stream>>>(h->counts, h->n_global, h->mave, h->mstd, h->M);
    HIP_TRY(hipGetLastError());
    HIP_TRY(hipStreamSynchronize(h->stream));
    {
        std::vector<unsigned long long> c((size_t)h->M * 3);
        HIP_TRY(hipMemcpy(c.data(), h->counts, c.size() * sizeof(unsigned long long), hipMemcpyDeviceToHost));
        uint64_t nmc = 0;
        for (uint32_t i = 0; i < h->M; ++i) nmc += c[3ull * i + 2] != 0 ? 1u : 0u;
        h->any_missing = nmc != 0;
    }
    h->have_stats = true;
    return 0;
}

int hgibbs_marker_stats(hgibbs_t h, double* mave_host, double* mstd_host, uint64_t* n1_host, uint64_t* n2_host, uint64_t* nmiss_host)
{
    if (!h || !h->bed) return fail("hgibbs_marker_stats: no data loaded");
    HIP_TRY(hipSetDevice(h->device));
    if (compute_stats(h)) return 1;
    if (mave_host) HIP_TRY(hipMemcpy(mave_host, h->mave, (size_t)h->M * sizeof(double), hipMemcpyDeviceToHost));
    if (mstd_host) HIP_TRY(hipMemcpy(mstd_host, h->mstd, (size_t)h->M * sizeof(double), hipMemcpyDeviceToHost));
    if (n1_host || n2_host || nmiss_host) {
        std::vector<unsigned long long> c((size_t)h->M * 3);
        HIP_TRY(hipMemcpy(c.data(), h->counts, c.size() * sizeof(unsigned long long), hipMemcpyDeviceToHost));
        for (uint32_t i = 0; i < h->M; ++i) {
            if (n1_host) n1_host[i] = c[3ull * i];
            if (n2_host) n2_host[i] = c[3ull * i + 1];
            if (nmiss_host) nmiss_host[i] = c[3ull * i + 2];
        }
    }
    return 0;
}

int hgibbs_set_residual(hgibbs_t h, const double* eps_host)
{
    if (!h || !h->bed) return fail("hgibbs_set_residual: no data loaded");
    HIP_TRY(hipSetDevice(h->device));
    double* tmp = nullptr;
    HIP_TRY(hipMalloc(&tmp, (size_t)h->n_local * sizeof(double)));
    HIP_TRY(hipMemcpyAsync(tmp, eps_host, (size_t)h->n_local * sizeof(double), hipMemcpyHostToDevice, h->stream));
    k_set_eps<<<(h->n_pad + 255) / 256, 256, 0, h->stream>>>(h->eps[h->eps_cur], tmp, h->n_local, h->n_pad);
    HIP_TRY(hipGetLastError());
    HIP_TRY(hipStreamSynchronize(h->stream));
    HIP_TRY(hipFree(tmp));
    return 0;
}

int hgibbs_get_residual(hgibbs_t h, double* eps_host)
{
    if (!h || !h->bed) return fail("hgibbs_get_residual: no data loaded");
    HIP_TRY(hipSetDevice(h->device));
    double* tmp = nullptr;
    HIP_TRY(hipMalloc(&tmp, (size_t)h->n_local * sizeof(double)));
    k_get_eps<<<(h->n_local + 255) / 256, 256, 0, h->stream>>>(h->eps[h->eps_cur], tmp, h->n_local);
    HIP_TRY(hipGetLastError());
    HIP_TRY(hipMemcpyAsync(eps_host, tmp, (size_t)h->n_local * sizeof(double), hipMemcpyDeviceToHost, h->stream));
    HIP_TRY(hipStreamSynchronize(h->stream));
    HIP_TRY(hipFree(tmp));
    return 0;
}

static int reduce_eps_all(hgibbs_ctx* h, double out[2])
{
    const uint32_t nblk = h->n_pad / BLOCK_IND;
    k_reduce_eps<<<nblk, BLOCK, 0, h->stream>>>(h->eps[h->eps_cur], h->n_pad, h->scratch);
    k_final_sum<<<1, BLOCK, 0, h->stream>>>(h->scratch, nblk, 3, h->sums);
    HIP_TRY(hipGetLastError());
    if (bulk_allreduce(h, h->sums, 3, 0)) return 1;
    HIP_TRY(hipMemcpyAsync(h->scratch_host, h->sums, 3 * sizeof(double), hipMemcpyDeviceToHost, h->stream));
    HIP_TRY(hipStreamSynchronize(h->stream));
    out[0] = h->scratch_host[0];
    out[1] = h->scratch_host[1];
    h->eps_abs_bound = std::pow(std::max(h->scratch_host[2], 0.0), 0.125);
    return 0;
}

int hgibbs_reduce_eps(hgibbs_t h, double* sum, double* sqn)
{
    if (!h || !h->bed) return fail("hgibbs_reduce_eps: no data loaded");
    HIP_TRY(hipSetDevice(h->device));
    double r[2];
    if (reduce_eps_all(h, r)) return 1;
    if (sum) *sum = r[0];
    if (sqn) *sqn = r[1];
    return 0;
}

int hgibbs_add_scalar(hgibbs_t h, double c)
{
    if (!h || !h->bed) return fail("hgibbs_add_scalar: no data loaded");
    HIP_TRY(hipSetDevice(h->device));
    k_add_scalar<<<(h->n_local + 255) / 256, 256, 0, h->stream>>>(h->eps[h->eps_cur], c, h->n_local, h->n_pad);
    HIP_TRY(hipGetLastError());
    return 0;
}

int hgibbs_update_marker(hgibbs_t h, uint32_t marker, double dbeta)
{
    if (!h || !h->bed) return fail("hgibbs_update_marker: no data loaded");
    if (marker >= h->M) return fail("hgibbs_update_marker: marker %u >= M %u", marker, h->M);
    HIP_TRY(hipSetDevice(h->device));
    if (compute_stats(h)) return 1;
    if (dbeta == 0.0) return 0;
    double ms[2];
    HIP_TRY(hipMemcpy(&ms[0], h->mave + marker, sizeof(double), hipMemcpyDeviceToHost));
    HIP_TRY(hipMemcpy(&ms[1], h->mstd + marker, sizeof(double), hipMemcpyDeviceToHost));
    const double v0 = -(ms[0] * ms[1] * dbeta);
    const double v1 = dbeta * (1.0 - ms[0]) * ms[1];
    const double v2 = dbeta * (2.0 - ms[0]) * ms[1];
    k_update_one<<<h->n_pad / BLOCK_IND, BLOCK, 0, h->stream>>>(h->bed, h->stride, marker, h->eps[h->eps_cur], v0, v1, v2);
    HIP_TRY(hipGetLastError());
    return 0;
}

int hgibbs_dot_marker(hgibbs_t h, uint32_t marker, double* num)
{
    if (!h || !h->bed || !num) return fail("hgibbs_dot_marker: bad argument");
    if (marker >= h->M) return fail("hgibbs_dot_marker: marker %u >= M %u", marker, h->M);
    HIP_TRY(hipSetDevice(h->device));
    if (compute_stats(h)) return 1;
    const uint32_t nblk = h->n_pad / BLOCK_IND;
    k_dot_one<<<nblk, BLOCK, 0, h->stream>>>(h->bed, h->stride, marker, h->eps[h->eps_cur], h->scratch);
    k_final_sum<<<1, BLOCK, 0, h->stream>>>(h->scratch, nblk, 4, h->sums);
    HIP_TRY(hipGetLastError());
    if (bulk_allreduce(h, h->sums, 4, 0)) return 1;
    HIP_TRY(hipMemcpyAsync(h->scratch_host, h->sums, 4 * sizeof(double), hipMemcpyDeviceToHost, h->stream));
    HIP_TRY(hipMemcpyAsync(h->scratch_host + 4, h->mave + marker, sizeof(double), hipMemcpyDeviceToHost, h->stream));
    HIP_TRY(hipMemcpyAsync(h->scratch_host + 5, h->mstd + marker, sizeof(double), hipMemcpyDeviceToHost, h->stream));
    HIP_TRY(hipStreamSynchronize(h->stream));
    const double S1 = h->scratch_host[0], S2 = h->scratch_host[1], SM = h->scratch_host[2], Sall = h->scratch_host[3];
    double dp = 0.0;
    dp += S1 * 1.0;
    dp += S2 * 2.0;
    double syt = Sall;
    syt -= SM;
    dp -= (h->scratch_host[4] * syt);
    dp *= h->scratch_host[5];
    *num = dp;
    return 0;
}

int hgibbs_set_covariates(hgibbs_t h, const double* X_host, int C)
{
    if (!h || !h->bed) return fail("hgibbs_set_covariates: load genotypes first");
    if (C < 0 || (C > 0 && !X_host)) return fail("hgibbs_set_covariates: bad argument");
    HIP_TRY(hipSetDevice(h->device));
    if (h->covX) HIP_TRY(hipFree(h->covX));
    h->covX = nullptr;
    h->C = C;
    if (C == 0) return 0;
    HIP_TRY(hipMalloc(&h->covX, (size_t)C * h->n_pad * sizeof(double)));
    double* tmp = nullptr;
    HIP_TRY(hipMalloc(&tmp, (size_t)h->n_local * C * sizeof(double)));
    HIP_TRY(hipMemcpyAsync(tmp, X_host, (size_t)h->n_local * C * sizeof(double), hipMemcpyHostToDevice, h->stream));
    for (int c = 0; c < C; ++c)
        k_set_cov<<<(h->n_pad + 255) / 256, 256, 0, h->stream>>>(h->covX + (size_t)c * h->n_pad, tmp, h->n_local, h->n_pad, C, c);
    HIP_TRY(hipGetLastError());
    HIP_TRY(hipStreamSynchronize(h->stream));
    HIP_TRY(hipFree(tmp));
    return 0;
}

int hgibbs_cov_dot(hgibbs_t h, int c, double gamma_old, double* num_f)
{
    if (!h || !h->covX || !num_f) return fail("hgibbs_cov_dot: no covariates set");
    if (c < 0 || c >= h->C) return fail("hgibbs_cov_dot: covariate %d outside [0,%d)", c, h->C);
    HIP_TRY(hipSetDevice(h->device));
    const uint32_t nblk = h->n_pad / BLOCK_IND;
    k_cov_dot<<<nblk, BLOCK, 0, h->stream>>>(h->covX + (size_t)c * h->n_pad, h->eps[h->eps_cur], gamma_old, h->scratch);
    k_final_sum<<<1, BLOCK, 0, h->stream>>>(h->scratch, nblk, 1, h->sums);
    HIP_TRY(hipGetLastError());
    if (bulk_allreduce(h, h->sums, 1, 0)) return 1;
    HIP_TRY(hipMemcpyAsync(h->scratch_host, h->sums, sizeof(double), hipMemcpyDeviceToHost, h->stream));
    HIP_TRY(hipStreamSynchronize(h->stream));
    *num_f = h->scratch_host[0];
    return 0;
}

int hgibbs_cov_update(hgibbs_t h, int c, double dgamma)
{
    if (!h || !h->covX) return fail("hgibbs_cov_update: no covariates set");
    if (c < 0 || c >= h->C) return fail("hgibbs_cov_update: covariate %d outside [0,%d)", c, h->C);
    HIP_TRY(hipSetDevice(h->device));
    k_cov_update<<<h->n_pad / BLOCK_IND, BLOCK, 0, h->stream>>>(h->covX + (size_t)c * h->n_pad, h->eps[h->eps_cur], dgamma);
    HIP_TRY(hipGetLastError());
    return 0;
}

int hgibbs_set_model(hgibbs_t h, int G, int K, const int32_t* groups_host, const double* cVa_host, const double* cVaI_host)
{
    if (!h || !h->bed) return fail("hgibbs_set_model: load data first");
    if (G < 1 || K < 2 || K > MAX_K) return fail("hgibbs_set_model: need G>=1 and 2<=K<=%d (got G=%d K=%d)", MAX_K, G, K);
    HIP_TRY(hipSetDevice(h->device));
    h->G = G;
    h->K = K;
    h->groups_host.assign(h->M, 0);
    if (groups_host) {
        for (uint32_t i = 0; i < h->M; ++i) {
            if (groups_host[i] < 0 || groups_host[i] >= G) return fail("hgibbs_set_model: groups[%u]=%d outside [0,%d)", i, groups_host[i], G);
            h->groups_host[i] = groups_host[i];
        }
    }
    HIP_TRY(hipMemcpy(h->groups, h->groups_host.data(), (size_t)h->M * sizeof(int32_t), hipMemcpyHostToDevice));
    h->cVa.assign(cVa_host, cVa_host + (size_t)G * K);
    h->cVaI.assign(cVaI_host, cVaI_host + (size_t)G * K);
    if (h->cass) HIP_TRY(hipFree(h->cass));
    if (h->tables) HIP_TRY(hipFree(h->tables));
    HIP_TRY(hipMalloc(&h->cass, (size_t)G * K * sizeof(int32_t)));
    HIP_TRY(hipMalloc(&h->tables, (size_t)4 * G * K * sizeof(double)));
    return 0;
}

int hgibbs_set_beta(hgibbs_t h, const double* beta_host)
{
    if (!h || !h->bed) return fail("hgibbs_set_beta: no data loaded");
    HIP_TRY(hipSetDevice(h->device));
    HIP_TRY(hipMemcpy(h->beta, beta_host, (size_t)h->M * sizeof(double), hipMemcpyHostToDevice));
    return 0;
}

int hgibbs_set_components(hgibbs_t h, const int32_t* components_host)
{
    if (!h || !h->bed || !components_host) return fail("hgibbs_set_components: bad argument");
    HIP_TRY(hipSetDevice(h->device));
    HIP_TRY(hipMemcpy(h->comp, components_host, (size_t)h->M * sizeof(int32_t), hipMemcpyHostToDevice));
    return 0;
}

int hgibbs_get_beta(hgibbs_t h, double* beta_host, int32_t* components_host, double* acum_host)
{
    if (!h || !h->bed) return fail("hgibbs_get_beta: no data loaded");
    HIP_TRY(hipSetDevice(h->device));
    HIP_TRY(hipStreamSynchronize(h->stream));
    if (beta_host) HIP_TRY(hipMemcpy(beta_host, h->beta, (size_t)h->M * sizeof(double), hipMemcpyDeviceToHost));
    if (components_host) HIP_TRY(hipMemcpy(components_host, h->comp, (size_t)h->M * sizeof(int32_t), hipMemcpyDeviceToHost));
    if (acum_host) HIP_TRY(hipMemcpy(acum_host, h->acum, (size_t)h->M * sizeof(double), hipMemcpyDeviceToHost));
    return 0;
}

int hgibbs_beta_sqnorm(hgibbs_t h, double* bsq_host)
{
    if (!h || !h->bed || h->G < 1) return fail("hgibbs_beta_sqnorm: model not set");
    HIP_TRY(hipSetDevice(h->device));
    if (!h->beta_host) HIP_TRY(hipHostMalloc(&h->beta_host, (size_t)h->M * sizeof(double)));
    HIP_TRY(hipMemcpyAsync(h->beta_host, h->beta, (size_t)h->M * sizeof(double), hipMemcpyDeviceToHost, h->stream));
    HIP_TRY(hipStreamSynchronize(h->stream));
    for (int g = 0; g < h->G; ++g) bsq_host[g] = 0.0;
    for (uint32_t i = 0; i < h->M; ++i) bsq_host[h->groups_host[i]] += h->beta_host[i] * h->beta_host[i];
    return 0;
}

int hgibbs_set_option(hgibbs_t h, const char* name, int64_t value)
{
    if (!h || !name) return fail("hgibbs_set_option: null argument");
    for (const char* o : {"cols_per_group", "slices", "gram_missing", "graph", "max_seg", "ext_limit", "gram", "carry", "ahead", "force_split", "chunk"})
        if (!std::strcmp(name, o) && h->engine == 0) h->engine_pinned = true;
    if (!std::strcmp(name, "batch") && value != 0 && h->engine == 0) h->engine_pinned = true;
    if (!std::strcmp(name, "score_sp")) {
        if (value != 0 && value != 2 && value != 4 && value != 8 && value != 16) return fail("score_sp must be 0 (automatic), 2, 4, 8 or 16");
        h->score_sp = (int)value;
    } else if (!std::strcmp(name, "ld_split")) {
        if (value < 0 || value > 65535) return fail("ld_split must be in [0,65535] (0 = automatic)");
        h->ld_split = (int)value;
    } else if (!std::strcmp(name, "king_split")) {
        if (value < 0 || value > 65535) return fail("king_split must be in [0,65535] (0 = automatic)");
        h->king_split = (int)value;
    } else if (!std::strcmp(name, "mdots_split")) {
        if (value < 0 || value > 65535) return fail("mdots_split must be in [0,65535] (0 = automatic)");
        h->mdots_split = (int)value;
    } else if (!std::strcmp(name, "score_ranges")) {
        if (value < 0 || value > 65535) return fail("score_ranges must be in [0,65535] (0 = automatic)");
        h->score_ranges = (int)value;
    } else if (!std::strcmp(name, "batch")) {
        if (value < 0 || value > MAX_BATCH) return fail("batch must be in [0,%d] (0 = auto)", MAX_BATCH);
        h->batch = (uint32_t)value;
    } else if (!std::strcmp(name, "cols_per_group")) {
        if (value != 2 && value != 4 && value != 8 && value != 16) return fail("cols_per_group must be 2, 4, 8 or 16");
        h->cols_per_group = (uint32_t)value;
    } else if (!std::strcmp(name, "slices")) {
        if (value < 0 || value > S_CAP) return fail("slices must be in [0,%d] (0 = auto)", S_CAP);
        h->slices = (uint32_t)value;
    } else if (!std::strcmp(name, "gram_missing")) {
        h->gram_missing = (int)value;
    } else if (!std::strcmp(name, "graph")) {
        h->use_graph = value != 0;
    } else if (!std::strcmp(name, "max_seg")) {
        if (value < 0 || value > MAX_SEG) return fail("hgibbs_set_option: max_seg %lld outside [0,%d]", (long long)value, MAX_SEG);
        h->max_seg = (uint32_t)value;
    } else if (!std::strcmp(name, "ext_limit")) {
        if (value < 0 || value > MAX_BATCH) return fail("ext_limit must be in [0,%d]", MAX_BATCH);
        h->ext_limit = (uint32_t)value;
    } else if (!std::strcmp(name, "gram")) {
        h->gram = value != 0;
    } else if (!std::strcmp(name, "carry")) {
        h->carry_on = value < 0 ? -1 : (value != 0 ? 1 : 0);
    } else if (!std::strcmp(name, "ahead")) {
        if (value < -1 || value > AHEAD_MAX) return fail("ahead must be in [-1,%d] (-1 = auto)", AHEAD_MAX);
        h->ahead = (int)value;

    } else if (!std::strcmp(name, "engine")) {
        if (value < 0 || value > 2) return fail("engine must be 0 (auto), 1 (batch) or 2 (resident)");
        h->engine = (int)value;
    } else if (!std::strcmp(name, "window")) {
        if (value != 0 && (value < 8 || value > RS_BMAX || (value & (value - 1)))) return fail("window must be 0 (auto) or a power of two in [8,%d]", RS_BMAX);
        h->window = (uint32_t)value;
    } else if (!std::strcmp(name, "pivots")) {
        h->res_pivots = value != 0;
    } else if (!std::strcmp(name, "early_advance")) {
        if (value < 0 || value > 255) return fail("early_advance must be in [0,255]");
        h->res_early = (int)value;
    } else if (!std::strcmp(name, "refill")) {
        if (value < 0 || value > 2) return fail("refill must be 0 (auto), 1 (fused multiply-adds) or 2 (integer matrix products)");
        h->res_refill = (int)value;
    } else if (!std::strcmp(name, "walker2_ranks")) {
        h->res_walker2_ranks = value != 0;
    } else if (!std::strcmp(name, "window_end16")) {
        h->res_wend = value != 0;
    } else if (!std::strcmp(name, "announce")) {
        h->res_announce = value != 0;
    } else if (!std::strcmp(name, "walker")) {
        if (value < 0 || value > 2) return fail("walker must be 0 (auto), 1 (first) or 2 (second)");
        h->res_walker = (int)value;
    } else if (!std::strcmp(name, "res_cus")) {
        if (value < 0 || value > 4096) return fail("res_cus must be in [0,4096]");
        h->res_cus = (uint32_t)value;
    } else if (!std::strcmp(name, "res_deadline_ms")) {
        h->res_deadline_s = (double)value * 1e-3;
    } else if (!std::strcmp(name, "res_timeout_ms")) {
        if (value < 1) return fail("res_timeout_ms must be positive");
        h->res_timeout_s = (double)value * 1e-3;
    } else if (!std::strcmp(name, "p2p")) {
        h->p2p_enabled = value != 0;
    } else if (!std::strcmp(name, "force_split")) {
        h->force_split = value != 0;
    } else if (!std::strcmp(name, "w_kernel_timing")) {
        h->w_kernel_timing = value != 0;
    } else if (!std::strcmp(name, "debug_timing")) {
        h->debug_timing = value != 0;
    } else if (!std::strcmp(name, "chunk")) {
        h->chunk = (int)value;
    } else {
        return fail("hgibbs_set_option: unknown option '%s'", name);
    }
    return 0;
}

int hgibbs_debug_times(hgibbs_t h, uint64_t* out8)
{
    if (!h || !out8) return fail("null argument");
    HIP_TRY(hipSetDevice(h->device));
    HIP_TRY(hipMemcpy(out8, h->dbg, 48 * sizeof(unsigned long long), hipMemcpyDeviceToHost));
    HIP_TRY(hipMemset(h->dbg, 0, 48 * sizeof(unsigned long long)));
    return 0;
}

int hgibbs_resident_trace(hgibbs_t h, uint64_t* out, uint64_t words)
{
    if (!h || !out) return fail("null argument");
    HIP_TRY(hipSetDevice(h->device));
    const uint64_t n = std::min<uint64_t>(words, (uint64_t)10 * RS_TRACE);
    HIP_TRY(hipMemcpy(out, h->res_trace, n * sizeof(unsigned long long), hipMemcpyDeviceToHost));
    return 0;
}

int hgibbs_stream_ceiling(hgibbs_t h, uint64_t bytes, int reps, double* gbps)
{
    if (!h || !gbps || bytes < (1u << 20) || reps < 1) return fail("hgibbs_stream_ceiling: bad argument");
    HIP_TRY(hipSetDevice(h->device));
    void *a = nullptr, *b = nullptr;
    HIP_TRY(hipMalloc(&a, bytes));
    HIP_TRY(hipMalloc(&b, bytes));
    HIP_TRY(hipMemsetAsync(a, 1, bytes, h->stream));
    HIP_TRY(hipMemcpyAsync(b, a, bytes, hipMemcpyDeviceToDevice, h->stream));
    HIP_TRY(hipEventRecord(h->ev0, h->stream));
    for (int i = 0; i < reps; ++i) HIP_TRY(hipMemcpyAsync((i & 1) ? a : b, (i & 1) ? b : a, bytes, hipMemcpyDeviceToDevice, h->stream));
    HIP_TRY(hipEventRecord(h->ev1, h->stream));
    HIP_TRY(hipEventSynchronize(h->ev1));
    float ms = 0.f;
    HIP_TRY(hipEventElapsedTime(&ms, h->ev0, h->ev1));
    HIP_TRY(hipFree(a));
    HIP_TRY(hipFree(b));
    *gbps = 2.0 * (double)bytes * reps / (ms * 1e-3) / 1e9;
    return 0;
}

int hgibbs_last_sweep_stats(hgibbs_t h, hgibbs_sweep_stats* out)
{
    if (!h || !out) return fail("null argument");
    *out = h->stats;
    return 0;
}

}

using ResKernel = void (*)(ResParams, const ResParams*);

static const ResKernel RES_BUILDS[] = {
    k_sweep_resident<1, 0, 0>, k_sweep_resident<1, 0, 1>, k_sweep_resident<1, 1, 0>, k_sweep_resident<1, 1, 1>,
    k_sweep_resident<2, 0, 0>, k_sweep_resident<2, 0, 1>, k_sweep_resident<2, 1, 0>, k_sweep_resident<2, 1, 1>,
    k_sweep_limb<1, 0, 0>,     k_sweep_limb<1, 0, 1>,     k_sweep_limb<1, 1, 0>,     k_sweep_limb<1, 1, 1>,
    k_sweep_limb<2, 0, 0>,     k_sweep_limb<2, 0, 1>,     k_sweep_limb<2, 1, 0>,     k_sweep_limb<2, 1, 1>,
    k_sweep_limb4<0, 0>,       k_sweep_limb4<0, 1>,       k_sweep_limb4<1, 0>,       k_sweep_limb4<1, 1>,
};
static_assert(sizeof(RES_BUILDS) / sizeof(RES_BUILDS[0]) == sizeof(hgibbs_ctx::res_attr_set), "one LDS opt-in flag per resident build");

struct SweepPlan {
    bool resident = false;
    const char* why = nullptr;
    int T = 1;
    uint32_t W = 0;
    uint32_t B = 0;
    int refill = 1;
    int walker = 1;
    int pivots = 0;
    uint32_t wend_mask = 0;
    size_t streamer_lds = 0;
    size_t lds = 0;
    int slot = 0;
    ResKernel kern = nullptr;
};

static SweepPlan plan_sweep(const hgibbs_ctx* h)
{
    SweepPlan pl;
    auto refuse = [&](const char* why) {
        pl.why = why;
        return pl;
    };
    if (h->nranks > 1 && !(h->p2p_ready && h->p2p_enabled)) return refuse("several ranks without peer mailboxes (hgibbs_p2p_import): the RCCL / host exchange lives in the batch engine");
    if (h->nranks > RX_MAXR) return refuse("more than eight ranks");
    if (h->force_split) return refuse("force_split");
    if (h->G * h->K > 256 || h->K > MAX_K || h->K < 2) return refuse("mixture size");
    const uint32_t cus = h->res_cus ? std::min<uint32_t>(h->res_cus, (uint32_t)h->num_cu) : (uint32_t)h->num_cu;
    if (cus < 2) return refuse("fewer than two compute units");
    pl.refill = h->res_refill ? h->res_refill : (h->res_pivots || !(h->eps_abs_bound < 32.0)) ? 1 : 2;
    const uint32_t ntile = h->n_pad / TILE;
    uint32_t T = (ntile + (cus - 1) - 1) / (cus - 1);
    if (T > (uint32_t)RS_TMAX) {
        const bool four = T <= (uint32_t)RL_TMAX && h->nranks <= 1 && pl.refill == 2 && (h->res_refill == 2 || h->eps_abs_bound < 16.0);
        if (!four) return refuse(T <= (uint32_t)RL_TMAX ? "more than 2048 individuals per compute unit need the second form of the streaming workgroups on one rank (option refill, |eps| < 32)"
                                                       : "more individuals than the compute units hold (4096 each)");
        T = (uint32_t)RL_TMAX;
    }
    if ((h->stride & 1023u) || (uint64_t)h->M * (h->stride >> 10) >= (1ull << 32)) return refuse("a shard's BED columns are addressed in 32 bits of KiB");
    pl.T = (int)T;
    pl.W = (ntile + T - 1) / T;
    pl.B = h->window ? h->window : (uint32_t)RS_BMAX;
    while (pl.B * T > 512u) pl.B >>= 1;
    const bool w2_ok = h->res_all_ada && h->G * h->K <= HT_LDS && h->G <= RS_FG && (h->nranks <= 1 || h->res_walker2_ranks);
    pl.walker = w2_ok ? (h->res_walker == 1 ? 1 : 2) : (h->res_walker == 2 ? 0 : 1);
    pl.pivots = (h->nranks > 1 || h->any_missing || pl.refill == 2) ? 0 : h->res_pivots;
    pl.wend_mask = (pl.walker == 2 && pl.B >= 32u && h->res_wend) ? 15u : 0u;
    pl.streamer_lds = pl.refill == 2 ? rl_streamer_lds(pl.B, pl.T) : h->any_missing ? rs_streamer_lds_miss(pl.B, pl.T) : rs_streamer_lds(pl.B, pl.T);
    pl.lds = std::max(pl.streamer_lds, pl.walker == 2 ? rs_walker2_lds(pl.B) : rs_walker_lds(pl.B));
    const int form = pl.refill == 2 ? (pl.T == RL_TMAX ? 4 : 1 + pl.T) : pl.T - 1;
    pl.slot = 4 * form + (h->debug_timing ? 2 : 0) + (h->any_missing ? 1 : 0);
    pl.kern = RES_BUILDS[pl.slot];
    pl.resident = true;
    return pl;
}

static int res_opt_in(hgibbs_ctx* h, const SweepPlan& pl)
{
    if (!h->res_attr_set[pl.slot]) {
        HIP_TRY(hipFuncSetAttribute((const void*)pl.kern, hipFuncAttributeMaxDynamicSharedMemorySize, 160 * 1024));
        h->res_attr_set[pl.slot] = true;
    }
    return 0;
}

template <class P>
static void fill_sweep_common(const hgibbs_ctx* h, P& p, double sigmaE, double eps_sum)
{
    const int GK = h->G * h->K;
    p.bed = h->bed;
    p.stride = h->stride;
    p.n_pad = h->n_pad;
    p.n_local = h->n_local;
    p.M = h->M;
    p.n_minus_1 = (double)(h->n_global - 1);
    p.n_total = (double)h->n_global;
    p.eps_sum = eps_sum;
    p.order = h->order;
    p.s_mave = h->s_mave;
    p.s_mstd = h->s_mstd;
    p.s_bold = h->s_bold;
    p.s_ga = h->s_ga;
    p.beta = h->beta;
    p.comp = h->comp;
    p.acum = h->acum;
    p.cass = h->cass;
    p.K = h->K;
    p.GK = GK;
    p.denom = h->tables;
    p.logpi = h->tables + (size_t)GK;
    p.hlog = h->tables + (size_t)2 * GK;
    p.sdk = h->tables + (size_t)3 * GK;
    p.i_2sigE = 1.0 / (2.0 * sigmaE);
    p.mt = h->mt;
    p.zig = ZigTables{h->zig, h->zig + 129, h->zig + 258, h->zig + 515};
}

static int resident_probe(hgibbs_ctx* h, const SweepPlan& pl)
{
    if (res_opt_in(h, pl)) return 1;
    ResParams p{};
    p.W = pl.W;
    p.B = pl.B;
    p.M = 0xffffffffu;
    p.state = h->res_state;
    p.progress = h->res_progress;
    p.rdv_timeout = (unsigned long long)(std::min(h->res_timeout_s, 1.0) * 1e8);
    p.nranks = h->nranks > 1 ? h->nranks : 1;
    p.rank = h->nranks > 1 ? h->rank : 0;
    for (int r = 0; r < RX_MAXR; ++r) p.mbox[r] = (h->nranks > 1 && r < h->nranks) ? (unsigned char*)h->peer_base[r] + MBOX_RES_OFF : nullptr;
    p.sweep_id = ++h->res_probe_id;
    const size_t lds = std::max(pl.streamer_lds, std::max(rs_walker_lds(pl.B), rs_walker2_lds(pl.B)));
    if (hipMemsetAsync(h->res_progress, 0, 16 * sizeof(unsigned long long), h->stream) != hipSuccess || hipMemsetAsync(h->res_state, 0, sizeof(ResState), h->stream) != hipSuccess) return 1;
    pl.kern<<<dim3(pl.W + 1), RS_BLOCK, lds, h->stream>>>(p, h->res_params);
    if (hipGetLastError() != hipSuccess) return 1;
    if (hipMemcpyAsync(h->res_state_host, h->res_state, sizeof(ResState), hipMemcpyDeviceToHost, h->stream) != hipSuccess || hipStreamSynchronize(h->stream) != hipSuccess) return 1;
    h->scratch_host[0] = h->res_state_host->error ? 1.0 : 0.0;
    if (hipMemcpyAsync(h->sums, h->scratch_host, sizeof(double), hipMemcpyHostToDevice, h->stream) != hipSuccess) return 1;
    if (bulk_allreduce(h, h->sums, 1, 0)) return 1;
    if (hipMemcpyAsync(h->scratch_host, h->sums, sizeof(double), hipMemcpyDeviceToHost, h->stream) != hipSuccess || hipStreamSynchronize(h->stream) != hipSuccess) return 1;
    if (h->scratch_host[0] != 0.0) {
        h->res_not_resident = true;
        return 1;
    }
    h->res_probed_w = pl.W + 1;
    return 0;
}

static int sweep_resident(hgibbs_ctx* h, const SweepPlan& pl, const double r0[2], double sigmaE, hgibbs_rng_state* rng, int32_t* cass_host, uint64_t* nnz_updates)
{
    if (!pl.walker) return fail("hgibbs_sweep: the second walker does not apply (frozen markers, more than %d groups or %d table entries, or several ranks with walker2_ranks = 0)", RS_FG, HT_LDS);
    static const bool timing = std::getenv("HGIBBS_TIMING") != nullptr;
    const auto t_0 = std::chrono::steady_clock::now();
    ResParams p{};
    fill_sweep_common(h, p, sigmaE, r0[0]);
    p.eps = h->eps[h->eps_cur];
    p.rng_idx = rng->idx;
    p.W = pl.W;
    p.B = pl.B;
    p.nsh = std::min<uint32_t>(RS_NSH, pl.W);
    p.rsh = std::min<uint32_t>(RS_RSH, pl.W);
    p.gacc = reinterpret_cast<uint32_t*>(h->res_acc);
    p.racc = reinterpret_cast<unsigned long long*>(h->res_acc + RES_GACC_BYTES);
    p.rcnt = reinterpret_cast<uint32_t*>(h->res_acc + RES_GACC_BYTES + RES_RACC_BYTES);
    p.pacc = reinterpret_cast<unsigned long long*>(h->res_acc + RES_GACC_BYTES + RES_RACC_BYTES + RES_RCNT_BYTES);
    p.racc2 = reinterpret_cast<unsigned long long*>(h->res_acc + RES_RACC2_OFF);
    p.gacc64 = reinterpret_cast<unsigned long long*>(h->res_acc + RES_RACC2_OFF + RES_RACC_BYTES);
    p.counts = h->counts;
    p.msg = h->res_msg;
    p.state = h->res_state;
    {
        const double bound = 16.0 * std::sqrt(1024.0 * (h->nranks > 1 ? RS_TMAX : pl.T) * std::max(r0[1], 1e-300)) + 1.0;
        int ex = 50 - (int)std::ceil(std::log2(bound));
        ex = std::max(-40, std::min(ex, 60));
        p.fx_scale = std::ldexp(1.0, ex);
        p.fx_unscale = std::ldexp(1.0, -ex);
    }
    p.timeout = (unsigned long long)(h->res_timeout_s * 1e8);
    p.rdv_timeout = (unsigned long long)(std::min(h->res_timeout_s, 0.1) * 1e8);
    p.dbg = h->debug_timing ? 1 : 0;
    p.pivots = pl.pivots;
    p.nranks = h->nranks > 1 ? h->nranks : 1;
    p.rank = h->nranks > 1 ? h->rank : 0;
    for (int r = 0; r < RX_MAXR; ++r) p.mbox[r] = (h->nranks > 1 && r < h->nranks) ? (unsigned char*)h->peer_base[r] + MBOX_RES_OFF : nullptr;
    p.all_ada = h->res_all_ada ? 1 : 0;
    p.walker = pl.walker;
    p.pred = h->pred;
    p.early_advance = p.nranks > 1 ? 0 : h->res_early;
    p.announce = h->res_announce;
    p.wend_mask = pl.wend_mask;
    {
        const uint32_t nchunk = (h->M + PRED_CHUNK - 1) / PRED_CHUNK;
        k_pred_count<<<nchunk, 256, 0, h->stream>>>(h->s_bold, h->M, h->pred_cnt);
        k_pred_scan<<<1, 1024, 0, h->stream>>>(h->pred_cnt, nchunk);
        k_pred_scatter<<<nchunk, 256, 0, h->stream>>>(h->s_bold, h->M, h->pred_cnt, nchunk, h->pred);
        HIP_TRY(hipGetLastError());
    }
    p.sweep_id = ++h->res_sweep_id;
    p.trace = h->res_trace;
    p.progress = h->res_progress;
    HIP_TRY(hipMemsetAsync(h->res_progress, 0, 16 * sizeof(unsigned long long), h->stream));

    HIP_TRY(hipMemsetAsync(h->res_acc, 0, RES_ACC_BYTES, h->stream));
    HIP_TRY(hipMemsetAsync(h->res_msg, 0, RS_MSG * sizeof(ResMsg), h->stream));
    HIP_TRY(hipMemsetAsync(h->res_state, 0, sizeof(ResState), h->stream));
    if (res_opt_in(h, pl)) return 1;
    {
        int per_cu = 0;
        HIP_TRY(hipOccupancyMaxActiveBlocksPerMultiprocessor(&per_cu, pl.kern, RS_BLOCK, pl.lds));
        if (per_cu < 1 || (uint64_t)per_cu * (uint64_t)h->num_cu < (uint64_t)pl.W + 1)
            return fail("hgibbs_sweep: the resident grid of %u workgroups does not fit the device (%d per compute unit, %d units)", pl.W + 1, per_cu, h->num_cu);
    }
    if (std::getenv("HGIBBS_DEBUG"))
        std::fprintf(stderr, "[hgibbs] resident sweep: T %d, %u streaming workgroups, window %u, LDS %zu B, fixed-point scale 2^%d\n", pl.T, pl.W, pl.B, pl.lds, (int)std::log2(p.fx_scale));
    HIP_TRY(hipEventRecord(h->ev0, h->stream));
    *h->res_params_host = p;
    HIP_TRY(hipMemcpyAsync(h->res_params, h->res_params_host, sizeof(ResParams), hipMemcpyHostToDevice, h->stream));
    pl.kern<<<dim3(pl.W + 1), RS_BLOCK, pl.lds, h->stream>>>(p, h->res_params);
    HIP_TRY(hipGetLastError());
    k_res_finish<<<dim3((h->M + 255u) / 256u), 256, 0, h->stream>>>(p);
    HIP_TRY(hipGetLastError());
    HIP_TRY(hipEventRecord(h->ev1, h->stream));
    HIP_TRY(hipMemcpyAsync(h->res_state_host, h->res_state, sizeof(ResState), hipMemcpyDeviceToHost, h->stream));
    {
        auto t_start = std::chrono::steady_clock::now();
        auto t_probe = t_start;
        unsigned long long last_round = ~0ull;
        const double limit_s = h->res_deadline_s > 0.0 ? h->res_deadline_s : 30.0 + 20.0 * h->res_timeout_s;
        for (;;) {
            const hipError_t q = hipStreamQuery(h->stream);
            if (q == hipSuccess) break;
            if (q != hipErrorNotReady) return fail("hgibbs_sweep: resident engine: %s", hipGetErrorString(q));
            const auto now = std::chrono::steady_clock::now();
            const double el = std::chrono::duration<double>(now - t_start).count();
            if (std::chrono::duration<double>(now - t_probe).count() > std::min(1.0, 0.25 * limit_s)) {
                t_probe = now;
                if (hipMemcpyAsync(h->res_progress_host, h->res_progress, 16 * sizeof(unsigned long long), hipMemcpyDeviceToHost, h->aux_stream) == hipSuccess &&
                    hipStreamSynchronize(h->aux_stream) == hipSuccess && (h->res_progress_host[0] >> 8) != last_round) {
                    last_round = h->res_progress_host[0] >> 8;
                    t_start = now;
                    continue;
                }
            }
            if (el > limit_s) {
                const unsigned long long* pr = h->res_progress_host;
                const unsigned long long w0 = pr[0], w1 = pr[1];
                h->res_progress_host[8] = 3ull;
                (void)hipMemcpyAsync(h->res_progress + 2, h->res_progress_host + 8, sizeof(unsigned long long), hipMemcpyHostToDevice, h->aux_stream);
                (void)hipStreamSynchronize(h->aux_stream);
                const auto t_abort = std::chrono::steady_clock::now();
                bool back = false;
                while (std::chrono::duration<double>(std::chrono::steady_clock::now() - t_abort).count() < 5.0 + 3.0 * h->res_timeout_s) {
                    if (hipStreamQuery(h->stream) != hipErrorNotReady) {
                        back = true;
                        break;
                    }
                    std::this_thread::sleep_for(std::chrono::milliseconds(2));
                }
                if (!back) h->res_dead = true;
                return fail("hgibbs_sweep: the resident kernel made no progress for %.0f s: walker at round %llu stage %llu, streaming workgroup 0 at message %llu stage %llu; it was told to stop and %s", el,
                            (unsigned long long)(w0 >> 8), (unsigned long long)(w0 & 255u), (unsigned long long)(w1 >> 8), (unsigned long long)(w1 & 255u),
                            back ? "did (the sweep's results are void)" : "did NOT come back: this handle cannot be used any more");
            }
            if (el > 0.002) std::this_thread::sleep_for(std::chrono::microseconds(el > 0.5 ? 2000 : 50));
        }
    }
    const auto t_kernel = std::chrono::steady_clock::now();
    const ResState& st = *h->res_state_host;
    if (st.error == 6u) {
        h->res_not_resident = true;
        fail("hgibbs_sweep: the resident grid of %u workgroups was not resident at once (the device is shared)", pl.W + 1);
        return 2;
    }
    if (st.error)
        return fail("hgibbs_sweep: resident engine abort code %u at cursor %u (2 = rng staging overrun, 3 = a workgroup timed out, 5 = raw dot outside the fixed-point range)", st.error, st.cursor);
    if (st.cursor != h->M) return fail("hgibbs_sweep: resident engine stopped at cursor %u of %u", st.cursor, h->M);
    float ms = 0.f;
    HIP_TRY(hipEventElapsedTime(&ms, h->ev0, h->ev1));
    rng->idx = st.rng_idx;
    HIP_TRY(hipMemcpy(rng->x, h->mt, MT_N * sizeof(uint32_t), hipMemcpyDeviceToHost));
    if (cass_host) HIP_TRY(hipMemcpy(cass_host, h->cass, (size_t)h->G * h->K * sizeof(int32_t), hipMemcpyDeviceToHost));
    if (nnz_updates) *nnz_updates = st.nnz;
    hgibbs_sweep_stats& s = h->stats;
    s = hgibbs_sweep_stats{};
    s.launches = 1;
    s.nnz_updates = st.nnz;
    s.device_ms = ms;
    s.working_launches = st.rounds;
    s.kernel_ms_avg = st.rounds ? ms / (double)st.rounds : 0.0;
    s.accepted_markers = st.cursor;
    s.streamed_columns = h->M;
    s.tiles_per_workgroup_min = s.tiles_per_workgroup_max = (uint32_t)pl.T;
    s.engine = 2;
    s.walker = (uint32_t)pl.walker;
    s.refill = (uint32_t)pl.refill;
    s.rounds = st.rounds;
    s.events = st.events;
    s.advances = st.advances;
    s.chunks = st.chunks;
    s.refolds = st.refolds;
    s.pivots = st.pivots;
    s.predicted = st.predicted;
    for (int i = 0; i < 16; ++i) s.ticks[i] = st.t[i];
    s.shader_mhz = st.wall_ticks ? 100.0 * (double)st.shader_ticks / (double)st.wall_ticks : 0.0;
    {
        double r1[2];
        if (reduce_eps_all(h, r1)) return 1;
        s.eps_sum_drift = std::fabs(r1[0] - r0[0]);
    }
    if (timing) {
        auto ms = [](auto a, auto b) { return std::chrono::duration<double, std::milli>(b - a).count(); };
        std::fprintf(stderr, "[hgibbs] resident sweep: host until the kernel is back %.3f ms (device %.3f), results + drift %.3f\n", ms(t_0, t_kernel), (double)s.device_ms,
                     ms(t_kernel, std::chrono::steady_clock::now()));
    }
    return 0;
}

struct BatchBuild {
    uint32_t cpg;
    int tier, mg, nomiss, dbg;
    void (*kern)(SweepParams);
    void (*draw)(SweepParams);
};
static const BatchBuild BATCH_BUILDS[] = {
    {2, 2, 0, 0, 0, k_sweep_batch<2, 2, 0>, k_sweep_draw<2, 0>},
    {4, 2, 0, 0, 0, k_sweep_batch<4, 2, 0>, k_sweep_draw<2, 0>},
    {4, 2, 0, 1, 0, k_sweep_batch<4, 2, 0, 1>, k_sweep_draw<2, 0>},
    {4, 2, 0, 0, 1, k_sweep_batch<4, 2, 0, 0, 1>, k_sweep_draw<2, 0>},
    {4, 2, 0, 1, 1, k_sweep_batch<4, 2, 0, 1, 1>, k_sweep_draw<2, 0>},
    {8, 2, 0, 0, 0, k_sweep_batch<8, 2, 0>, k_sweep_draw<2, 0>},
    {16, 2, 0, 0, 0, k_sweep_batch<16, 2, 0>, k_sweep_draw<2, 0>},
    {4, 4, 0, 0, 0, k_sweep_batch<4, 4, 0>, k_sweep_draw<4, 0>},
    {4, 4, 0, 1, 0, k_sweep_batch<4, 4, 0, 1>, k_sweep_draw<4, 0>},
    {4, 4, 0, 0, 1, k_sweep_batch<4, 4, 0, 0, 1>, k_sweep_draw<4, 0>},
    {4, 4, 0, 1, 1, k_sweep_batch<4, 4, 0, 1, 1>, k_sweep_draw<4, 0>},
    {8, 4, 0, 0, 0, k_sweep_batch<8, 4, 0>, k_sweep_draw<4, 0>},
    {4, 2, 1, 0, 0, k_sweep_batch<4, 2, 1>, k_sweep_draw<2, 1>},
    {4, 2, 1, 0, 1, k_sweep_batch<4, 2, 1, 0, 1>, k_sweep_draw<2, 1>},
    {8, 2, 1, 0, 0, k_sweep_batch<8, 2, 1>, k_sweep_draw<2, 1>},
};

static int sweep_batch(hgibbs_ctx* h, const double r0[2], double sigmaE, hgibbs_rng_state* rng, int32_t* cass_host, uint64_t* nnz_updates)
{
    const int G = h->G, K = h->K;
    const uint32_t M = h->M;
    const uint32_t cpg = h->cols_per_group;
    const uint32_t batch = h->batch ? h->batch : ((h->n_local >= 20000u || h->nranks > 1) ? 256u : 128u);
    const uint32_t ngroups = (batch + cpg - 1) / cpg;
    SweepDesc d0{};
    d0.cursor = 0;
    for (int q = 0; q < MAX_SEG; ++q) {
        d0.pend_marker[q] = -1;
        d0.seg_end[q] = batch;
    }
    d0.cur = h->eps_cur;
    d0.rng_idx = rng->idx;
    d0.seq = h->batch_seq;
    *h->desc_host = d0;
    SweepCounters* const cnt_host = reinterpret_cast<SweepCounters*>(h->desc_host + 1);
    *cnt_host = SweepCounters{};
    cnt_host->tiles_min = 0xffffffffu;
    HIP_TRY(hipMemcpyAsync(h->desc, h->desc_host, sizeof(SweepDesc) + sizeof(SweepCounters), hipMemcpyHostToDevice, h->stream));

    SweepParams p{};
    fill_sweep_common(h, p, sigmaE, r0[0]);
    p.eps0 = h->eps[0];
    p.eps1 = h->eps[1];
    p.gram = h->gram ? 1 : 0;
    p.dbg = (h->debug_timing && h->cols_per_group == 4) ? h->dbg : nullptr;
    p.desc = h->desc;
    p.counters = reinterpret_cast<SweepCounters*>(h->desc + 1);
    p.partials = h->partials;
    p.ticket = h->ticket;
    p.gticket = h->ticket + 16;
    p.entered = h->ticket + 16 + MAX_GROUPS;
    p.totals = h->totals;
    p.carry = h->carry;
    p.ahead_raw = h->ahead_raw;
    p.apartials = h->apartials;
    p.aticket = h->aticket;
    p.aqueue = h->aticket + AHEAD_MAX / 2;
    const bool carry_auto = h->n_local >= 400000u;
    p.carry_on = ((h->carry_on < 0 ? carry_auto : h->carry_on != 0) && h->gram) ? 1u : 0u;
    p.ahead_cols = (uint32_t)(h->ahead >= 0 ? h->ahead : 0);
    p.cols_per_group = cpg;
    p.batch_cap = ngroups * cpg;
    p.batch_limit = batch;
    p.ext_limit = h->ext_limit;
    p.max_seg = h->max_seg ? std::min<uint32_t>(h->max_seg, MAX_SEG) : ((h->n_local <= (h->nranks > 1 ? 400000u : 300000u)) ? 4u : 2u);
    const bool mg_wanted = h->gram_missing != 0;
    const bool mg = mg_wanted && h->gram && h->any_missing && (cpg == 4 || cpg == 8) && (h->max_seg == 0 || h->max_seg == 2);
    const int tier = (!mg && p.max_seg > 2 && h->gram && (cpg == 4 || cpg == 8)) ? 4 : 2;
    if (p.max_seg > (uint32_t)tier) p.max_seg = (uint32_t)tier;
    const int nr = sweep_rows(tier, mg ? 1 : 0);
    const size_t lds = sweep_lds_bytes(p.batch_cap, cpg, K, nr);
    if (std::getenv("HGIBBS_DEBUG")) std::fprintf(stderr, "[hgibbs] sweep LDS %zu B = %zu granules of 1280 B (3 per CU up to 42)\n", lds, (lds + 1279) / 1280);
    const bool use_p2p = h->nranks > 1 && h->p2p_ready && h->p2p_enabled && !h->force_split;
    const bool split = (h->nranks > 1 && !use_p2p) || h->force_split;
    if (h->nranks > 1 && split && !h->comm && !h->ext_fn)
        return fail("hgibbs_sweep: %d ranks but no per-batch transport (hgibbs_comm_init for RCCL, hgibbs_comm_init_external or hgibbs_p2p_import)", h->nranks);
    p.sums_out = split ? h->sums : nullptr;
    p.p2p.nranks = use_p2p ? h->nranks : 0;
    p.p2p.rank = h->rank;
    for (int r = 0; r < MAX_RANKS; ++r) {
        p.p2p.data[r] = (use_p2p && r < h->nranks) ? (double*)h->peer_base[r] : nullptr;
        p.p2p.flags[r] = (use_p2p && r < h->nranks) ? (unsigned long long*)((unsigned char*)h->peer_base[r] + MBOX_DATA_BYTES) : nullptr;
    }

    const uint32_t ntg = h->n_pad / BLOCK_IND;
    const uint32_t S = std::min<uint32_t>(h->slices ? h->slices : S_CAP, ntg);
    p.slices_max = S;
    const uint32_t ccg = (uint32_t)carried_cpg(tier, mg ? 1 : 0);
    const uint32_t groups_max = 1u + (batch + ccg - 1) / ccg + ngroups;
    if (groups_max > (uint32_t)MAX_GROUPS || (uint64_t)groups_max * group_rows((int)cpg, tier, mg ? 1 : 0) > (uint64_t)PROWS_CAP)
        return fail("hgibbs_sweep: %u groups of %d partial rows exceed the partial buffer", groups_max, group_rows((int)cpg, tier, mg ? 1 : 0));
    uint64_t total_launches = 0;
    const bool nomiss = !h->any_missing && cpg == 4;
    const bool dbg = h->debug_timing && cpg == 4;
    const BatchBuild* build = nullptr;
    for (const BatchBuild& b : BATCH_BUILDS)
        if (b.cpg == cpg && b.tier == tier && b.mg == (mg ? 1 : 0) && b.nomiss == (nomiss ? 1 : 0) && b.dbg == (dbg ? 1 : 0)) build = &b;
    if (!build) return fail("hgibbs_sweep: no build of the sweep kernel for %u columns per group, tier %d, missing-call Gram %d", cpg, tier, (int)mg);
    void (*const kern)(SweepParams) = build->kern;
    {
        int per_cu = 0;
        HIP_TRY(hipOccupancyMaxActiveBlocksPerMultiprocessor(&per_cu, kern, BLOCK, lds));
        if (per_cu < 1) return fail("hgibbs_sweep: the sweep kernel does not fit a compute unit with %zu bytes of LDS", lds);
        p.resident = (uint32_t)per_cu * (uint32_t)h->num_cu;
        if (std::getenv("HGIBBS_DEBUG")) std::fprintf(stderr, "[hgibbs] sweep build: tier %d mg %d cpg %u, LDS %zu B, %d workgroups per CU, %u resident\n", tier, (int)mg, cpg, lds, per_cu, p.resident);
    }
    {
        const uint32_t s_min = std::max<uint32_t>(1u, std::min<uint32_t>(S, p.resident / std::max<uint32_t>(1u, groups_max)));
        if ((ntg + s_min - 1) / s_min > 1000u) p.gram = 0;
    }
    const dim3 grid(std::min<uint32_t>(S * groups_max, p.resident));
    auto launch_one = [&]() { kern<<<grid, BLOCK, lds, h->stream>>>(p); };
    constexpr int GRAPH_N = 64;
    hipGraph_t graph = nullptr;
    hipGraphExec_t gexec = nullptr;
    if (h->use_graph && !split) {
        HIP_TRY(hipStreamBeginCapture(h->stream, hipStreamCaptureModeThreadLocal));
        for (int i = 0; i < GRAPH_N; ++i) launch_one();
        HIP_TRY(hipStreamEndCapture(h->stream, &graph));
        HIP_TRY(hipGraphInstantiate(&gexec, graph, nullptr, nullptr, 0));
    }
    HIP_TRY(hipEventRecord(h->ev0, h->stream));
    double avg_accept = std::max(1.0, (double)batch * 0.5);
    for (;;) {
        const SweepDesc& dh = *h->desc_host;
        const uint32_t remaining = M - std::min(M, dh.cursor);
        int n = h->chunk > 0 ? h->chunk : (int)std::min<double>(2048.0, std::max(8.0, 1.25 * remaining / avg_accept + 2));
        if (gexec) {
            n = (n + GRAPH_N - 1) / GRAPH_N * GRAPH_N;
            for (int i = 0; i < n; i += GRAPH_N) HIP_TRY(hipGraphLaunch(gexec, h->stream));
        }
        for (int i = 0; i < n && !gexec; ++i) {
            launch_one();
            if (split) {
                if (h->comm) NCCL_TRY(ncclAllReduce(h->sums, h->sums, nr * MAX_BATCH, ncclDouble, ncclSum, h->comm, h->stream));
                else if (h->nranks > 1 && bulk_allreduce(h, h->sums, (size_t)nr * MAX_BATCH, 0)) return 1;
                build->draw<<<1, BLOCK, lds, h->stream>>>(p);
            }
        }
        total_launches += (uint64_t)n;
        HIP_TRY(hipGetLastError());
        HIP_TRY(hipMemcpyAsync(h->desc_host, h->desc, sizeof(SweepDesc) + sizeof(SweepCounters), hipMemcpyDeviceToHost, h->stream));
        HIP_TRY(hipStreamSynchronize(h->stream));
        if (dh.error) return fail("hgibbs_sweep: device abort code %u at cursor %u (1 = logL overflow, 2 = rng staging overrun, 3 = peer exchange timed out, 4 = LDS base misaligned)", dh.error, dh.cursor);
        if (cnt_host->launches > 0) avg_accept = std::max(1.0, (double)cnt_host->accepted_sum / (double)cnt_host->launches);
        if (dh.cursor >= M && dh.pend_marker[0] < 0) break;
        if (total_launches > 2ull * M + 4096)
            return fail("hgibbs_sweep: no progress after %llu launches (cursor %u of %u)", (unsigned long long)total_launches, dh.cursor, M);
    }
    HIP_TRY(hipEventRecord(h->ev1, h->stream));
    HIP_TRY(hipEventSynchronize(h->ev1));
    float ms = 0.f;
    HIP_TRY(hipEventElapsedTime(&ms, h->ev0, h->ev1));
    if (gexec) (void)hipGraphExecDestroy(gexec);
    if (graph) (void)hipGraphDestroy(graph);

    h->eps_cur = h->desc_host->cur;
    h->batch_seq = h->desc_host->seq;
    rng->idx = h->desc_host->rng_idx;
    HIP_TRY(hipMemcpy(rng->x, h->mt, MT_N * sizeof(uint32_t), hipMemcpyDeviceToHost));
    if (cass_host) HIP_TRY(hipMemcpy(cass_host, h->cass, (size_t)G * K * sizeof(int32_t), hipMemcpyDeviceToHost));
    if (nnz_updates) *nnz_updates = cnt_host->nnz;
    h->stats.launches = total_launches;
    h->stats.nnz_updates = cnt_host->nnz;
    h->stats.carried_columns = cnt_host->carried_sum;
    if (std::getenv("HGIBBS_DEBUG")) std::fprintf(stderr, "[hgibbs] sweep: %llu launches, %llu columns carried\n", (unsigned long long)total_launches, (unsigned long long)cnt_host->carried_sum);
    h->stats.device_ms = ms;
    h->stats.working_launches = cnt_host->launches;
    h->stats.accepted_markers = cnt_host->accepted_sum;
    h->stats.streamed_columns = cnt_host->streamed_sum;
    h->stats.tiles_per_workgroup_min = cnt_host->tiles_max ? cnt_host->tiles_min : 0u;
    h->stats.tiles_per_workgroup_max = cnt_host->tiles_max;
    h->stats.kernel_ms_avg = cnt_host->launches ? ms / (double)cnt_host->launches : 0.0;
    h->stats.engine = 1;
    h->stats.rounds = h->stats.events = h->stats.advances = h->stats.chunks = h->stats.refolds = h->stats.pivots = 0;
    h->stats.shader_mhz = 0.0;
    for (int i = 0; i < 16; ++i) h->stats.ticks[i] = 0;
    {
        double r[2];
        if (reduce_eps_all(h, r)) return 1;
        h->stats.eps_sum_drift = std::fabs(r[0] - r0[0]);
    }
    return 0;
}

extern "C" {

int hgibbs_sweep(hgibbs_t h, const int32_t* order_host, double sigmaE, const double* sigmaG_host, const double* estPi_host,
                 const uint8_t* adaV_host, hgibbs_rng_state* rng, int32_t* cass_host, uint64_t* nnz_updates)
{
    if (!h || !h->bed) return fail("hgibbs_sweep: no data loaded");
    if (h->res_dead) return fail("hgibbs_sweep: a resident kernel of this handle never came back: the handle cannot be used any more");
    if (h->G < 1) return fail("hgibbs_sweep: model not set");
    if (!order_host || !sigmaG_host || !estPi_host || !adaV_host || !rng) return fail("hgibbs_sweep: null argument");
    const auto t_prep0 = std::chrono::steady_clock::now();
    HIP_TRY(hipSetDevice(h->device));
    if (compute_stats(h)) return 1;
    const int G = h->G, K = h->K;
    const uint32_t M = h->M;
    for (uint32_t i = 0; i < M; ++i)
        if (order_host[i] < 0 || (uint32_t)order_host[i] >= M) return fail("hgibbs_sweep: order[%u]=%d outside [0,%u)", i, order_host[i], M);
    if (rng->idx > (uint32_t)MT_N) return fail("hgibbs_sweep: rng idx %u > 624", rng->idx);

    const double dNm1 = (double)(h->n_global - 1);
    std::vector<double> tab((size_t)4 * G * K, 0.0);
    double* denom = tab.data();
    double* logpi = denom + (size_t)G * K;
    double* hlog = logpi + (size_t)G * K;
    double* sdk = hlog + (size_t)G * K;
    for (int g = 0; g < G; ++g) {
        const double sigE_G = sigmaE / sigmaG_host[g];
        const double sigG_E = sigmaG_host[g] / sigmaE;
        for (int k = 0; k < K; ++k) {
            logpi[g * K + k] = log(estPi_host[g * K + k]);
            if (k >= 1) {
                denom[g * K + k] = dNm1 + sigE_G * h->cVaI[g * K + k];
                hlog[g * K + k] = 0.5 * log(sigG_E * dNm1 * h->cVa[g * K + k] + 1.0);
                sdk[g * K + k] = sqrt(sigmaE / denom[g * K + k]);
            }
        }
    }
    HIP_TRY(hipMemcpyAsync(h->tables, tab.data(), tab.size() * sizeof(double), hipMemcpyHostToDevice, h->stream));
    HIP_TRY(hipMemcpyAsync(h->order, order_host, (size_t)M * sizeof(int32_t), hipMemcpyHostToDevice, h->stream));
    HIP_TRY(hipMemcpyAsync(h->adaV, adaV_host, (size_t)M, hipMemcpyHostToDevice, h->stream));
    HIP_TRY(hipMemcpyAsync(h->mt, rng->x, MT_N * sizeof(uint32_t), hipMemcpyHostToDevice, h->stream));
    HIP_TRY(hipMemsetAsync(h->cass, 0, (size_t)G * K * sizeof(int32_t), h->stream));
    HIP_TRY(hipMemsetAsync(h->ticket, 0, (16 + MAX_GROUPS + 256) * sizeof(uint32_t), h->stream));
    HIP_TRY(hipMemsetAsync(h->aticket, 0, (AHEAD_MAX / 2 + 4) * sizeof(uint32_t), h->stream));
    k_gather_meta<<<(M + 255) / 256, 256, 0, h->stream>>>(h->order, h->mave, h->mstd, h->beta, h->groups, h->adaV, h->counts, h->s_mave, h->s_mstd,
                                                       h->s_bold, h->s_ga, M);
    HIP_TRY(hipGetLastError());
    HIP_TRY(hipStreamSynchronize(h->stream));
    h->res_all_ada = std::memchr(adaV_host, 0, (size_t)M) == nullptr;
    if (std::getenv("HGIBBS_TIMING"))
        std::fprintf(stderr, "[hgibbs] sweep preparation (checks, tables, order / adaV upload, metadata gather) %.3f ms\n",
                     std::chrono::duration<double, std::milli>(std::chrono::steady_clock::now() - t_prep0).count());

    double r0[2];
    if (reduce_eps_all(h, r0)) return 1;

    SweepPlan plan = plan_sweep(h);
    {
        if (h->engine == 1 || (h->engine == 0 && h->engine_pinned)) plan.resident = false;
        if (h->engine == 0 && h->res_not_resident && plan.resident) {
            plan.resident = false;
            plan.why = "an earlier resident grid was not resident at once (the device is shared)";
        }
        if (h->nranks > 1) {
            h->scratch_host[0] = plan.resident ? 0.0 : 1.0;
            HIP_TRY(hipMemcpyAsync(h->sums, h->scratch_host, sizeof(double), hipMemcpyHostToDevice, h->stream));
            if (bulk_allreduce(h, h->sums, 1, 0)) return 1;
            HIP_TRY(hipMemcpyAsync(h->scratch_host, h->sums, sizeof(double), hipMemcpyDeviceToHost, h->stream));
            HIP_TRY(hipStreamSynchronize(h->stream));
            if (h->scratch_host[0] != 0.0) {
                if (plan.resident) plan.why = "another rank cannot run it";
                plan.resident = false;
            }
            if (plan.resident && h->res_probed_w != plan.W + 1 && resident_probe(h, plan)) {
                plan.resident = false;
                plan.why = "some rank's resident grid is not resident at once (a shared device)";
            }
        }
        if (h->engine == 2 && !plan.resident) return fail("hgibbs_sweep: the resident engine does not apply: %s", plan.why ? plan.why : "the batch engine was asked for by an option");
        if (std::getenv("HGIBBS_DEBUG"))
            std::fprintf(stderr, "[hgibbs] engine: %s%s%s\n", plan.resident ? "resident" : "batch", plan.why ? " -- resident refused: " : "", plan.why ? plan.why : "");
    }
    if (plan.resident) {
        const int rc = sweep_resident(h, plan, r0, sigmaE, rng, cass_host, nnz_updates);
        if (rc != 2 || h->engine == 2 || h->nranks > 1) return rc ? 1 : 0;
        if (std::getenv("HGIBBS_DEBUG")) std::fprintf(stderr, "[hgibbs] engine: the resident grid was not resident at once -- this sweep and the following ones run on the batch engine\n");
        if (reduce_eps_all(h, r0)) return 1;
    }
    return sweep_batch(h, r0, sigmaE, rng, cass_host, nnz_updates);
}

}

#include "hg_bayesw.hip.h"
#include "hg_ops.hip.h"
#include "hg_score.hip.h"
#include "hg_ld.hip.h"
#include "hg_mdots.hip.h"
#include "hg_king.hip.h"
#include "hg_pca.hip.h"
```

### hydra_amd/csrc/hydra_chain.cpp

```cpp
#include <algorithm>
#include <cmath>
#include <cstdio>
#include <cstring>
#include <string>
#include <chrono>
#include <cstdio>
#include <cstdlib>
#include <vector>

#include "../../include/hgibbs.h"
#include "hg_rng.h"

extern "C" void hgibbs_set_error_(const char* msg);

namespace {
const double V0E = 0.0001, S02E = 0.0001, V0G = 0.0001, S02G = 0.0001;
}

struct hydra_chain {
    hgibbs_t dev = nullptr;
    uint32_t N = 0, M = 0;
    int G = 1, K = 0;
    int shuffle = 1;
    std::vector<int32_t> groups, MtotGrp, order, cass, m0;
    std::vector<double> cVa, cVaI, priorPi, estPi, sigmaG;
    std::vector<uint8_t> adaV;
    double sigmaE = 0.0, mu = 0.0;
    hgibbs_rng_state rng{};
    uint64_t last_nnz = 0;
    int C = 0;
    std::vector<double> gamma;
    std::vector<unsigned int> xI;
    uint32_t row_begin = 0, n_local = 0;
    uint32_t iteration = 0;
};

static int cfail(const std::string& m)
{
    hgibbs_set_error_(m.c_str());
    return 1;
}

extern "C" {

int hydra_chain_create(hgibbs_t dev, const hydra_model_desc* model, const double* y_host, hydra_chain_t* out)
{
    if (!dev || !model || !y_host || !out) return cfail("hydra_chain_create: null argument");
    uint32_t n_global = 0, n_local = 0, M = 0, row_begin = 0;
    if (hgibbs_dims(dev, &n_global, &n_local, &M, &row_begin)) return 1;
    if (n_global < 2 || M == 0) return cfail("hydra_chain_create: load genotypes first (hgibbs_load_bed / hgibbs_synth_bed)");
    if (model->K < 2) return cfail("hydra_chain_create: K must be >= 2 (zero component + at least one mixture)");
    hydra_chain* c = new hydra_chain();
    c->dev = dev;
    c->N = n_global;
    c->M = M;
    c->row_begin = row_begin;
    c->n_local = n_local;
    c->G = model->G;
    c->K = model->K;
    c->shuffle = model->shuffle;
    const int G = c->G, K = c->K, km1 = K - 1;

    c->groups.assign(M, 0);
    if (model->groups) c->groups.assign(model->groups, model->groups + M);
    for (uint32_t i = 0; i < M; ++i)
        if (c->groups[i] < 0 || c->groups[i] >= G) {
            delete c;
            return cfail("hydra_chain_create: group index out of range");
        }

    c->cVa.assign((size_t)G * K, 0.0);
    c->cVaI.assign((size_t)G * K, 0.0);
    c->priorPi.assign((size_t)G * K, 0.0);
    for (int g = 0; g < G; ++g) {
        c->priorPi[g * K] = 0.5;
        double s = 0.0;
        for (int k = 1; k <= km1; ++k) {
            const double v = model->mS[g * K + k];
            if (!(v > 0.0)) {
                delete c;
                return cfail("FATAL  : mixture value can only be strictly positive");
            }
            c->cVa[g * K + k] = v;
            c->cVaI[g * K + k] = 1.0 / v;
            s += v;
        }
        for (int k = 1; k <= km1; ++k) c->priorPi[g * K + k] = c->priorPi[g * K] * c->cVa[g * K + k] / s;
    }
    c->estPi = c->priorPi;
    c->sigmaG.assign(G, 0.0);
    c->cass.assign((size_t)G * K, 0);
    c->m0.assign(G, 0);
    c->MtotGrp.assign(G, 0);
    for (uint32_t i = 0; i < M; ++i) c->MtotGrp[c->groups[i]] += 1;

    if (hgibbs_set_model(dev, G, K, c->groups.data(), c->cVa.data(), c->cVaI.data())) {
        delete c;
        return 1;
    }

    hg::Mt gen{c->rng.x, 0};
    gen.seed(model->seed);
    for (int g = 0; g < G; ++g) c->sigmaG[g] = hg::beta_rng(gen, 1.0, 1.0);
    for (int g = 0; g < G; ++g)
        if (c->MtotGrp[g] == 0) c->sigmaG[g] = 0.0;
    c->rng.idx = gen.idx;

    if (hgibbs_marker_stats(dev, nullptr, nullptr, nullptr, nullptr, nullptr)) {
        delete c;
        return 1;
    }

    c->order.resize(M);
    for (uint32_t i = 0; i < M; ++i) c->order[i] = (int32_t)i;

    std::vector<double> y(y_host, y_host + n_global);
    {
        double mean = 0.0;
        for (uint32_t i = 0; i < n_global; ++i) mean += y[i];
        mean /= n_global;
        for (uint32_t i = 0; i < n_global; ++i) y[i] -= mean;
        double sqn = 0.0;
        for (uint32_t i = 0; i < n_global; ++i) sqn += y[i] * y[i];
        sqn = sqrt((double)(n_global - 1) / sqn);
        for (uint32_t i = 0; i < n_global; ++i) y[i] *= sqn;
    }
    double se = 0.0;
    for (uint32_t i = 0; i < n_global; ++i) se += y[i] * y[i];
    c->sigmaE = se / (double)n_global * 0.5;
    if (hgibbs_set_residual(dev, y.data() + row_begin)) {
        delete c;
        return 1;
    }

    c->adaV.assign(M, 1);
    for (uint32_t i = 0; i < M; ++i)
        if (c->sigmaG[c->groups[i]] == 0.0) c->adaV[i] = 0;

    std::vector<double> zeros(M, 0.0);
    if (hgibbs_set_beta(dev, zeros.data())) {
        delete c;
        return 1;
    }
    *out = c;
    return 0;
}

int hydra_chain_destroy(hydra_chain_t c)
{
    delete c;
    return 0;
}

int hydra_chain_iterate(hydra_chain_t c)
{
    if (!c) return cfail("hydra_chain_iterate: null chain");
    const int G = c->G, K = c->K;
    const double dN = (double)c->N;
    hg::Mt gen{c->rng.x, c->rng.idx};
    static const bool timing = std::getenv("HGIBBS_TIMING") != nullptr;
    auto tnow = [] { return std::chrono::steady_clock::now(); };
    auto tms = [](std::chrono::steady_clock::time_point a, std::chrono::steady_clock::time_point b) { return std::chrono::duration<double, std::milli>(b - a).count(); };
    const auto t_0 = tnow();

    if (hgibbs_add_scalar(c->dev, c->mu)) return 1;
    double epssum = 0.0;
    if (hgibbs_reduce_eps(c->dev, &epssum, nullptr)) return 1;
    c->mu = hg::norm_rng(gen, epssum / dN, c->sigmaE / dN);
    if (hgibbs_add_scalar(c->dev, -c->mu)) return 1;

    const auto t_mu = tnow();
    if (c->shuffle) {
        hg::shuffle_libstdcxx6(c->order.data(), c->order.size(), gen);
    }
    std::fill(c->m0.begin(), c->m0.end(), 0);
    const auto t_shuffle = tnow();

    c->rng.idx = gen.idx;
    if (hgibbs_sweep(c->dev, c->order.data(), c->sigmaE, c->sigmaG.data(), c->estPi.data(), c->adaV.data(), &c->rng,
                     c->cass.data(), &c->last_nnz))
        return 1;
    gen.idx = c->rng.idx;
    const auto t_sweep = tnow();

    std::vector<double> bsq(G, 0.0);
    if (hgibbs_beta_sqnorm(c->dev, bsq.data())) return 1;
    const auto t_bsq = tnow();
    std::vector<double> dirin(K), pi(K);
    for (int g = 0; g < G; ++g) {
        if (c->MtotGrp[g] == 0) continue;
        c->m0[g] = c->MtotGrp[g] - c->cass[g * K];
        int rowsum = 0;
        for (int k = 0; k < K; ++k) rowsum += c->cass[g * K + k];
        if (c->m0[g] == 0 || rowsum == 0) {
            for (uint32_t i = 0; i < c->M; ++i)
                if (c->groups[i] == g) c->adaV[i] = 0;
            c->sigmaG[g] = 0.0;
            continue;
        }
        const double dm0 = (double)c->m0[g];
        c->sigmaG[g] = hg::inv_scaled_chisq_rng(gen, V0G + dm0, (bsq[g] * dm0 + V0G * S02G) / (V0G + dm0));
        for (int k = 0; k < K; ++k) dirin[k] = (double)c->cass[g * K + k] + 1.0;
        hg::dirichlet_rng(gen, dirin.data(), K, pi.data());
        for (int k = 0; k < K; ++k) c->estPi[g * K + k] = pi[k];
    }

    if (c->C > 0) {
        hg::shuffle_libstdcxx6(c->xI.data(), c->xI.size(), gen);
        const double sigmaF = 1.0;
        const double sigE_sigF = c->sigmaE / sigmaF;
        const double dNm1 = (double)(c->N - 1);
        for (int i = 0; i < c->C; ++i) {
            const int col = (int)c->xI[i];
            const double gamma_old = c->gamma[col];
            double num_f = 0.0;
            if (hgibbs_cov_dot(c->dev, col, gamma_old, &num_f)) return 1;
            const double denom_f = dNm1 + sigE_sigF;
            c->gamma[col] = hg::norm_rng(gen, num_f / denom_f, c->sigmaE / denom_f);
            if (hgibbs_cov_update(c->dev, col, gamma_old - c->gamma[col])) return 1;
        }
    }

    double e_sqn = 0.0;
    if (hgibbs_reduce_eps(c->dev, nullptr, &e_sqn)) return 1;
    c->sigmaE = hg::inv_scaled_chisq_rng(gen, V0E + dN, (e_sqn + V0E * S02E) / (V0E + dN));
    c->rng.idx = gen.idx;
    c->iteration += 1;
    if (timing)
        std::fprintf(stderr, "[hydra_chain] iteration %u: mu %.3f  shuffle %.3f  sweep call %.3f  beta sqnorm %.3f  hyper-parameters + sigmaE %.3f  | %.3f ms\n", c->iteration - 1,
                     tms(t_0, t_mu), tms(t_mu, t_shuffle), tms(t_shuffle, t_sweep), tms(t_sweep, t_bsq), tms(t_bsq, tnow()), tms(t_0, tnow()));
    return 0;
}

int hydra_chain_state(hydra_chain_t c, double* sigmaE, double* mu, double* sigmaG, double* estPi, int32_t* m0, int32_t* cass,
                      hgibbs_rng_state* rng)
{
    if (!c) return cfail("hydra_chain_state: null chain");
    if (sigmaE) *sigmaE = c->sigmaE;
    if (mu) *mu = c->mu;
    if (sigmaG) std::copy(c->sigmaG.begin(), c->sigmaG.end(), sigmaG);
    if (estPi) std::copy(c->estPi.begin(), c->estPi.end(), estPi);
    if (m0) std::copy(c->m0.begin(), c->m0.end(), m0);
    if (cass) std::copy(c->cass.begin(), c->cass.end(), cass);
    if (rng) *rng = c->rng;
    return 0;
}

int hydra_chain_set_covariates(hydra_chain_t c, const double* X_host, int C)
{
    if (!c) return cfail("hydra_chain_set_covariates: null chain");
    if (C < 0 || (C > 0 && !X_host)) return cfail("hydra_chain_set_covariates: bad argument");
    if (c->iteration != 0) return cfail("hydra_chain_set_covariates: call before the first iteration");
    c->C = C;
    c->gamma.assign(C, 0.0);
    c->xI.resize(C);
    for (int i = 0; i < C; ++i) c->xI[i] = (unsigned)i;
    return hgibbs_set_covariates(c->dev, C ? X_host + (size_t)c->row_begin * C : nullptr, C);
}

int hydra_chain_restore(hydra_chain_t c, const hydra_restart_state* st)
{
    if (!c || !st || !st->sigmaG || !st->estPi || !st->beta || !st->components || !st->eps || !st->order)
        return cfail("hydra_chain_restore: null argument");
    if (c->C > 0 && (!st->gamma || !st->xI)) return cfail("hydra_chain_restore: covariates set but no gamma/xI given");
    const int G = c->G, K = c->K;
    c->sigmaE = st->sigmaE;
    c->mu = st->mu;
    std::copy(st->sigmaG, st->sigmaG + G, c->sigmaG.begin());
    std::copy(st->estPi, st->estPi + (size_t)G * K, c->estPi.begin());
    for (uint32_t i = 0; i < c->M; ++i) {
        if (st->order[i] < 0 || (uint32_t)st->order[i] >= c->M) return cfail("hydra_chain_restore: marker index out of range");
        c->order[i] = st->order[i];
    }
    for (int i = 0; i < c->C; ++i) {
        c->gamma[i] = st->gamma[i];
        c->xI[i] = (unsigned)st->xI[i];
    }
    c->rng = st->rng;
    if (hgibbs_set_beta(c->dev, st->beta)) return 1;
    if (hgibbs_set_components(c->dev, st->components)) return 1;
    if (hgibbs_set_residual(c->dev, st->eps)) return 1;
    for (uint32_t i = 0; i < c->M; ++i) c->adaV[i] = (c->sigmaG[c->groups[i]] == 0.0) ? 0 : 1;
    c->iteration = st->iteration + 1;
    return 0;
}

int hydra_rng_to_boost_words(const hgibbs_rng_state* st, uint32_t* words624)
{
    if (!st || !words624) return cfail("hydra_rng_to_boost_words: null argument");
    hg::mt_to_boost_words(st->x, st->idx, words624);
    return 0;
}

int hydra_rng_from_boost_words(const uint32_t* words624, hgibbs_rng_state* st)
{
    if (!st || !words624) return cfail("hydra_rng_from_boost_words: null argument");
    std::memcpy(st->x, words624, 624 * sizeof(uint32_t));
    st->idx = 624;
    return 0;
}

int hydra_chain_gamma(hydra_chain_t c, double* gamma_out, int32_t* xI_out)
{
    if (!c) return cfail("hydra_chain_gamma: null chain");
    for (int i = 0; i < c->C; ++i) {
        if (gamma_out) gamma_out[i] = c->gamma[i];
        if (xI_out) xI_out[i] = (int32_t)c->xI[i];
    }
    return 0;
}

uint64_t hydra_chain_last_nnz(hydra_chain_t c) { return c ? c->last_nnz : 0; }

int hydra_chain_csv_line(hydra_chain_t c, uint32_t iteration, char* buf, size_t len)
{
    if (!c || !buf) return -1;
    const int G = c->G, K = c->K;
    size_t o = 0;
    o += snprintf(buf + o, len - o, "%5d, %4d", (int)iteration, G);
    double sg = 0.0;
    for (int g = 0; g < G; ++g) {
        o += snprintf(buf + o, len - o, ", %20.15f", c->sigmaG[g]);
        sg += c->sigmaG[g];
    }
    int m0sum = 0;
    for (int g = 0; g < G; ++g) m0sum += c->m0[g];
    o += snprintf(buf + o, len - o, ", %20.15f, %20.15f, %7d, %4d, %2d", c->sigmaE, sg / (c->sigmaE + sg), m0sum, G, K);
    for (int g = 0; g < G; ++g)
        for (int k = 0; k < K; ++k) o += snprintf(buf + o, len - o, ", %20.15f", c->estPi[g * K + k]);
    o += snprintf(buf + o, len - o, "\n");
    return (int)o;
}

const int32_t* hydra_chain_order(hydra_chain_t c) { return c ? c->order.data() : nullptr; }

}
```

### hydra_amd/csrc/hydraw_chain.cpp

```cpp
#include <hip/hip_runtime.h>

#include <algorithm>
#include <cmath>
#include <cstdio>
#include <cstring>
#include <string>
#include <vector>

#include "../../include/hgibbs.h"
#include "hg_ars.h"
#include "hg_bayesw_math.h"
#include "hg_rng.h"

extern "C" void hgibbs_set_error_(const char* msg);

using namespace hg;

struct hydraw_chain {
    hgibbs_t dev = nullptr;
    uint32_t N = 0, M = 0;
    int G = 1, K = 0, quad = 0, shuffle = 1;
    std::vector<int32_t> groups, MtotGrp, order, cass, m0, fail;
    std::vector<double> pi, sigmaG;
    double mu = 0.0, alpha = 0.0, d = 0.0, sumSigmaG = 0.0;
    hgibbs_rng_state rng{};
    hgibbs_grand_state grand{};
    uint64_t last_nnz = 0;
    int C = 0;
    std::vector<double> gamma, sum_failure_fix;
    std::vector<unsigned int> xI;
    uint32_t iteration = 0;
    uint32_t row_begin = 0;
};

static int wfail(const std::string& m)
{
    hgibbs_set_error_(m.c_str());
    return 1;
}

namespace {

struct GrandUniform {
    GlibcRand* g;
    double operator()() { return g->uniform(); }
};

struct DeviceDensity {
    hgibbs_t dev;
    int kind, col;
    double alpha, lin, prior_var, ef;
    bool failed = false;
    double operator()(double x)
    {
        double s = 0.0;
        int rc;
        if (kind == 1) {
            rc = hgibbs_w_reduce(dev, 1, 0, x, 0.0, 0.0, &s);
            if (rc) failed = true;
            return (bw::ALPHA_0 + lin - 1) * std::log(x) + x * (ef - bw::KAPPA_0) - s;
        }
        rc = hgibbs_w_reduce(dev, kind, col, 0.0, x, alpha, &s);
        if (rc) failed = true;
        return -alpha * x * lin - s - x * x / (2 * prior_var);
    }
};

template <class F>
int draw(F& f, const double (&xinit)[4], double xl, double xr, hgibbs_grand_state* grand, double& out, const char* what)
{
    GrandUniform u{reinterpret_cast<GlibcRand*>(grand)};
    ars::Hull hull;
    int neval = 0;
    const int err = ars::sample(xinit, xl, xr, f, u, hull, out, neval);
    if (f.failed) return 1;
    if (err) return wfail(std::string("Error code = ") + std::to_string(err) + " (ARS on " + what + ")");
    return 0;
}

}

extern "C" {

int hydraw_chain_create(hgibbs_t dev, const hydraw_model_desc* model, const double* y_host, const int32_t* failure_host, hydraw_chain_t* out)
{
    if (!dev || !model || !y_host || !failure_host || !out) return wfail("hydraw_chain_create: null argument");
    uint32_t n_global = 0, n_local = 0, M = 0, row_begin = 0;
    if (hgibbs_dims(dev, &n_global, &n_local, &M, &row_begin)) return 1;
    if (n_global < 2 || M == 0) return wfail("hydraw_chain_create: load genotypes first (hgibbs_load_bed / hgibbs_synth_bed)");
    if (model->K < 2) return wfail("hydraw_chain_create: K must be >= 2 (zero component + at least one mixture)");
    if (hgibbs_w_init(dev, failure_host)) return 1;
    if (hgibbs_w_set_model(dev, model->G, model->K, model->groups, model->mS, model->quad_points)) return 1;
    if (hgibbs_w_marker_stats(dev, nullptr, nullptr, nullptr)) return 1;
    hydraw_chain* c = new hydraw_chain();
    c->dev = dev;
    c->N = n_global;
    c->M = M;
    c->row_begin = row_begin;
    c->G = model->G;
    c->K = model->K;
    c->quad = model->quad_points;
    c->shuffle = model->shuffle;
    const int G = c->G, K = c->K;
    c->groups.assign(M, 0);
    if (model->groups) c->groups.assign(model->groups, model->groups + M);
    c->MtotGrp.assign(G, 0);
    for (uint32_t i = 0; i < M; ++i) c->MtotGrp[c->groups[i]] += 1;
    c->pi.assign((size_t)G * K, 1.0 / M);
    const unsigned int_div = (unsigned)(K - 1 - 1) / (unsigned)M;
    for (int g = 0; g < G; ++g) {
        c->pi[(size_t)g * K + 0] = 0.99;
        c->pi[(size_t)g * K + 1] = 1 - c->pi[(size_t)g * K + 0] - int_div;
    }
    c->fail.assign(failure_host, failure_host + n_global);
    c->cass.assign((size_t)G * K, 0);
    c->m0.assign(G, 0);
    c->order.resize(M);
    for (uint32_t i = 0; i < M; ++i) c->order[i] = (int32_t)i;

    double s = 0.0;
    for (uint32_t i = 0; i < n_global; ++i) s += y_host[i];
    c->mu = s / (double)n_global;
    double ss = 0.0;
    for (uint32_t i = 0; i < n_global; ++i) ss += (y_host[i] - c->mu) * (y_host[i] - c->mu);
    const double denominator = (6 * ss / (double)(n_global - 1));
    c->alpha = bw::PI_BW / std::sqrt(denominator);
    std::vector<double> eps(n_global);
    for (uint32_t i = 0; i < n_global; ++i) eps[i] = y_host[i] - c->mu;
    if (hgibbs_set_residual(dev, eps.data() + row_begin)) {
        delete c;
        return 1;
    }
    c->sigmaG.assign(G, bw::PI_SQUARED / (6 * std::pow(c->alpha, 2)) / G);
    c->sumSigmaG = 0.0;
    for (int g = 0; g < G; ++g) c->sumSigmaG += c->sigmaG[g];
    c->d = 0.0;
    for (uint32_t i = 0; i < n_global; ++i) c->d += (double)failure_host[i];

    hgibbs_grand_seed(&c->grand, model->seed);
    Mt gen{c->rng.x, 0};
    gen.seed(model->seed);
    c->rng.idx = gen.idx;
    *out = c;
    return 0;
}

int hydraw_chain_destroy(hydraw_chain_t c)
{
    delete c;
    return 0;
}

int hydraw_chain_set_covariates(hydraw_chain_t c, const double* X_host, int C)
{
    if (!c) return wfail("hydraw_chain_set_covariates: null chain");
    if (C < 0 || (C > 0 && !X_host)) return wfail("hydraw_chain_set_covariates: bad argument");
    if (c->iteration != 0) return wfail("hydraw_chain_set_covariates: call before the first iteration");
    c->C = C;
    c->gamma.assign(C, 0.0);
    c->xI.resize(C);
    for (int i = 0; i < C; ++i) c->xI[i] = (unsigned)i;
    c->sum_failure_fix.assign(C, 0.0);
    for (int k = 0; k < C; ++k) {
        double s = 0.0;
        for (uint32_t i = 0; i < c->N; ++i) s += X_host[(size_t)i * C + k] * (double)c->fail[i];
        c->sum_failure_fix[k] = s;
    }
    return hgibbs_set_covariates(c->dev, C ? X_host + (size_t)c->row_begin * C : nullptr, C);
}

int hydraw_chain_reseed_ars(hydraw_chain_t c, uint32_t seed)
{
    if (!c) return wfail("hydraw_chain_reseed_ars: null chain");
    hgibbs_grand_seed(&c->grand, seed);
    return 0;
}

int hydraw_chain_restore(hydraw_chain_t c, const hydraw_restart_state* st)
{
    if (!c || !st || !st->sigmaG || !st->pi || !st->beta || !st->components || !st->eps || !st->order)
        return wfail("hydraw_chain_restore: null argument");
    if (c->C > 0 && (!st->gamma || !st->xI)) return wfail("hydraw_chain_restore: covariates set but no gamma/xI given");
    const int G = c->G, K = c->K;
    for (uint32_t i = 0; i < c->M; ++i)
        if (st->order[i] < 0 || (uint32_t)st->order[i] >= c->M) return wfail("hydraw_chain_restore: marker index out of range");
    c->mu = st->mu;
    c->alpha = st->alpha;
    std::copy(st->sigmaG, st->sigmaG + G, c->sigmaG.begin());
    std::copy(st->pi, st->pi + (size_t)G * K, c->pi.begin());
    std::copy(st->order, st->order + c->M, c->order.begin());
    for (int i = 0; i < c->C; ++i) {
        c->gamma[i] = st->gamma[i];
        c->xI[i] = (unsigned)st->xI[i];
    }
    c->sumSigmaG = 0.0;
    for (int g = 0; g < G; ++g) c->sumSigmaG += c->sigmaG[g];
    c->rng = st->rng;
    hgibbs_grand_seed(&c->grand, st->ars_seed);
    if (hgibbs_w_set_beta(c->dev, st->beta, st->components)) return 1;
    if (hgibbs_set_residual(c->dev, st->eps)) return 1;
    c->iteration = st->iteration + 1;
    return 0;
}

int hydraw_chain_iterate(hydraw_chain_t c)
{
    if (!c) return wfail("hydraw_chain_iterate: null chain");
    const int G = c->G, K = c->K;
    Mt gen{c->rng.x, c->rng.idx};

    {
        const double mu = c->mu;
        const double xinit[4] = {0.95 * mu, mu, 1.005 * mu, 1.01 * mu};
        if (hgibbs_add_scalar(c->dev, mu)) return 1;
        DeviceDensity f{c->dev, 0, 0, c->alpha, c->d, bw::SIGMA_MU, 0.0};
        double x = 0.0;
        if (draw(f, xinit, 0.8 * mu, 1.1 * mu, &c->grand, x, "mu")) return 1;
        c->mu = x;
        if (hgibbs_add_scalar(c->dev, -c->mu)) return 1;
    }
    if (c->C > 0) {
        hg::shuffle_libstdcxx6(c->xI.data(), c->xI.size(), gen);
        for (int i = 0; i < c->C; ++i) {
            const int col = (int)c->xI[i];
            const double gamma_old = c->gamma[col];
            const double xinit[4] = {gamma_old - 0.075 / 30, gamma_old, gamma_old + 0.075 / 60, gamma_old + 0.075 / 30};
            if (hgibbs_cov_update(c->dev, col, gamma_old)) return 1;
            DeviceDensity f{c->dev, 2, col, c->alpha, c->sum_failure_fix[col], bw::SIGMA_MU, 0.0};
            double x = 0.0;
            if (draw(f, xinit, gamma_old - 0.075, gamma_old + 0.075, &c->grand, x, "a covariate effect")) return 1;
            c->gamma[col] = x;
            if (hgibbs_cov_update(c->dev, col, -c->gamma[col])) return 1;
        }
    }
    {
        const double a = c->alpha;
        const double xinit[4] = {a * 0.5, a, a * 1.05, a * 1.10};
        double ef = 0.0;
        if (hgibbs_w_reduce(c->dev, 3, 0, 0.0, 0.0, 0.0, &ef)) return 1;
        DeviceDensity f{c->dev, 1, 0, 0.0, c->d, 0.0, ef};
        double x = 0.0;
        if (draw(f, xinit, 0.0, a * 1.30, &c->grand, x, "alpha")) return 1;
        c->alpha = x;
    }
    if (hgibbs_w_refresh_vi(c->dev, c->alpha)) return 1;

    if (c->shuffle) {
        hg::shuffle_libstdcxx6(c->order.data(), c->order.size(), gen);
    }
    std::fill(c->m0.begin(), c->m0.end(), 0);
    c->rng.idx = gen.idx;
    std::vector<double> bsq(G, 0.0);
    if (hgibbs_w_sweep(c->dev, c->order.data(), c->alpha, c->sigmaG.data(), c->pi.data(), c->sumSigmaG, &c->rng, &c->grand, c->cass.data(),
                       bsq.data(), &c->last_nnz))
        return 1;
    gen.idx = c->rng.idx;

    for (int g = 0; g < G; ++g) c->m0[g] = c->MtotGrp[g] - c->cass[(size_t)g * K];
    for (int g = 0; g < G; ++g)
        c->sigmaG[g] = inv_gamma_rng(gen, (double)(bw::ALPHA_SIGMA + 0.5 * c->m0[g]), (double)(bw::BETA_SIGMA + 0.5 * (double)c->m0[g] * bsq[g]));
    std::vector<double> dirin(K), out(K);
    for (int g = 0; g < G; ++g) {
        for (int k = 0; k < K; ++k) dirin[k] = (double)(c->cass[(size_t)g * K + k] + 1);
        dirichlet_rng(gen, dirin.data(), K, out.data());
        for (int k = 0; k < K; ++k) c->pi[(size_t)g * K + k] = out[k];
    }
    c->sumSigmaG = 0.0;
    for (int g = 0; g < G; ++g) c->sumSigmaG += c->sigmaG[g];
    c->rng.idx = gen.idx;
    c->iteration += 1;
    return 0;
}

int hydraw_chain_state(hydraw_chain_t c, double* mu, double* alpha, double* sigmaG, double* pi, int32_t* m0, int32_t* cass,
                       hgibbs_rng_state* rng, hgibbs_grand_state* ars_rng)
{
    if (!c) return wfail("hydraw_chain_state: null chain");
    if (mu) *mu = c->mu;
    if (alpha) *alpha = c->alpha;
    if (sigmaG) std::copy(c->sigmaG.begin(), c->sigmaG.end(), sigmaG);
    if (pi) std::copy(c->pi.begin(), c->pi.end(), pi);
    if (m0) std::copy(c->m0.begin(), c->m0.end(), m0);
    if (cass) std::copy(c->cass.begin(), c->cass.end(), cass);
    if (rng) *rng = c->rng;
    if (ars_rng) *ars_rng = c->grand;
    return 0;
}

int hydraw_chain_gamma(hydraw_chain_t c, double* gamma_out, int32_t* xI_out)
{
    if (!c) return wfail("hydraw_chain_gamma: null chain");
    for (int i = 0; i < c->C; ++i) {
        if (gamma_out) gamma_out[i] = c->gamma[i];
        if (xI_out) xI_out[i] = (int32_t)c->xI[i];
    }
    return 0;
}

const int32_t* hydraw_chain_order(hydraw_chain_t c) { return c ? c->order.data() : nullptr; }
uint64_t hydraw_chain_last_nnz(hydraw_chain_t c) { return c ? c->last_nnz : 0; }

int hydraw_chain_csv_line(hydraw_chain_t c, uint32_t iteration, char* buf, size_t len)
{
    if (!c || !buf) return -1;
    const int G = c->G, K = c->K;
    double sg = 0.0;
    int m0s = 0;
    for (int g = 0; g < G; ++g) {
        sg += c->sigmaG[g];
        m0s += c->m0[g];
    }
    size_t n = (size_t)std::snprintf(buf, len, "%5d, %20.15f, %20.15f, %20.15f, %20.15f, %7d, %7d, %2d", iteration, c->mu, sg, c->alpha,
                                     sg / (sg + bw::PI_SQUARED / (6 * c->alpha * c->alpha)), m0s, G, K);
    for (int g = 0; g < G && n < len; ++g) n += (size_t)std::snprintf(buf + n, len - n, ", %20.15f", c->sigmaG[g]);
    for (int i = 0; i < G * K && n < len; ++i) n += (size_t)std::snprintf(buf + n, len - n, ", %20.15f", c->pi[i]);
    if (n < len) n += (size_t)std::snprintf(buf + n, len - n, "\n");
    return (int)n;
}

}
```

### include/hgibbs.h

```cpp
#ifndef HGIBBS_H
#define HGIBBS_H

#include <stddef.h>
#include <stdint.h>

#ifdef __cplusplus
extern "C" {
#endif

typedef struct hgibbs_ctx* hgibbs_t;

typedef struct {
    uint32_t x[624];
    uint32_t idx;
} hgibbs_rng_state;

const char* hgibbs_last_error(void);
int hgibbs_version(void);

int hgibbs_create(int device_id, hgibbs_t* out);
int hgibbs_destroy(hgibbs_t h);

int hgibbs_comm_unique_id(void* id128);
int hgibbs_comm_init(hgibbs_t h, int nranks, int rank, const void* id128);
typedef int (*hgibbs_allreduce_fn)(void* user, void* buf_host, size_t count, int dtype);
int hgibbs_comm_init_external(hgibbs_t h, int nranks, int rank, hgibbs_allreduce_fn fn, void* user);
int hgibbs_p2p_export(hgibbs_t h, void* handle64);
int hgibbs_p2p_import(hgibbs_t h, const void* handles );

int hgibbs_load_bed(hgibbs_t h, const uint8_t* bed_host, uint64_t stride_in, uint32_t n_total, uint32_t M,
                    const uint8_t* keep_host, uint32_t row_begin, uint32_t row_end, uint32_t n_global);
int hgibbs_synth_bed(hgibbs_t h, uint32_t n_global, uint32_t M, uint32_t row_begin, uint32_t row_end,
                     uint64_t seed, double missing_rate);
int hgibbs_dims(hgibbs_t h, uint32_t* n_global, uint32_t* n_local, uint32_t* M, uint32_t* row_begin);
int hgibbs_get_bed(hgibbs_t h, uint32_t m0, uint32_t mcount, uint8_t* out_host, uint64_t out_stride);

int hgibbs_marker_stats(hgibbs_t h, double* mave_host, double* mstd_host, uint64_t* n1_host, uint64_t* n2_host,
                        uint64_t* nmiss_host);

int hgibbs_set_residual(hgibbs_t h, const double* eps_host);
int hgibbs_get_residual(hgibbs_t h, double* eps_host);
int hgibbs_reduce_eps(hgibbs_t h, double* sum, double* sqn);
int hgibbs_add_scalar(hgibbs_t h, double c);
int hgibbs_update_marker(hgibbs_t h, uint32_t marker, double dbeta);
int hgibbs_dot_marker(hgibbs_t h, uint32_t marker, double* num);

int hgibbs_set_covariates(hgibbs_t h, const double* X_host, int C);
int hgibbs_cov_dot(hgibbs_t h, int c, double gamma_old, double* num_f);
int hgibbs_cov_update(hgibbs_t h, int c, double dgamma);

int hgibbs_set_model(hgibbs_t h, int G, int K, const int32_t* groups_host, const double* cVa_host,
                     const double* cVaI_host);

int hgibbs_set_beta(hgibbs_t h, const double* beta_host);
int hgibbs_set_components(hgibbs_t h, const int32_t* components_host);
int hgibbs_get_beta(hgibbs_t h, double* beta_host, int32_t* components_host, double* acum_host);
int hgibbs_beta_sqnorm(hgibbs_t h, double* bsq_host );

int hgibbs_sweep(hgibbs_t h, const int32_t* order_host, double sigmaE, const double* sigmaG_host,
                 const double* estPi_host, const uint8_t* adaV_host, hgibbs_rng_state* rng, int32_t* cass_host,
                 uint64_t* nnz_updates);

int hgibbs_set_option(hgibbs_t h, const char* name, int64_t value);
typedef struct {
    uint64_t launches;
    uint64_t nnz_updates;
    double device_ms;
    double kernel_ms_avg;
    uint64_t carried_columns;
    uint64_t working_launches;
    uint64_t accepted_markers;
    uint64_t streamed_columns;
    uint32_t tiles_per_workgroup_min;
    uint32_t tiles_per_workgroup_max;
    uint32_t engine;
    uint32_t walker;
    double eps_sum_drift;
    uint64_t rounds, events, advances, chunks, refolds;
    uint64_t pivots;
    uint64_t predicted;
    double shader_mhz;
    uint64_t ticks[16];
    uint32_t refill;
    uint32_t reserved_;
} hgibbs_sweep_stats;
int hgibbs_last_sweep_stats(hgibbs_t h, hgibbs_sweep_stats* out);
int hgibbs_stream_ceiling(hgibbs_t h, uint64_t bytes, int reps, double* gbps);
int hgibbs_debug_times(hgibbs_t h, uint64_t* out48);
int hgibbs_resident_trace(hgibbs_t h, uint64_t* out, uint64_t words);

int hgibbs_score(hgibbs_t h, int S, const double* a, const double* o, double* out);
int hgibbs_last_score_ms(hgibbs_t h, double* ms);

int hgibbs_ld(hgibbs_t h, uint32_t m0, uint32_t count, uint32_t W, double* r_host, int64_t* sums_host);
int hgibbs_last_ld_ms(hgibbs_t h, double* ms);

int hgibbs_marker_dots(hgibbs_t h, uint32_t m0, uint32_t count, int K, const double* U, double* out, double* raw);
int hgibbs_last_marker_dots_ms(hgibbs_t h, double* ms);

int hgibbs_king(hgibbs_t h, uint32_t a0, uint32_t acount, uint32_t b0, uint32_t bcount, int32_t* counts);
int hgibbs_king_pairs(hgibbs_t h, double cutoff, uint64_t* npairs);
int hgibbs_king_pairs_get(hgibbs_t h, uint32_t* ab, int32_t* counts, double* kin);
int hgibbs_last_king_ms(hgibbs_t h, double* ms);

typedef struct {
    int32_t iters_run;
    uint32_t m_used;
    double ritz_change;
    double resid[32];
} hgibbs_pca_report;
int hgibbs_pca(hgibbs_t h, int K, int L, int iters, double tol, const double* Q0, uint64_t seed, double* eigval, double* pcs,
               double* loadings, hgibbs_pca_report* rep);
int hgibbs_last_pca_ms(hgibbs_t h, double* ms4);

typedef struct hydra_chain* hydra_chain_t;

typedef struct {
    uint32_t seed;
    int32_t shuffle;
    int32_t G, K;
    const int32_t* groups;
    const double* mS;
} hydra_model_desc;

int hydra_chain_create(hgibbs_t dev, const hydra_model_desc* model, const double* y_host, hydra_chain_t* out);
int hydra_chain_destroy(hydra_chain_t c);
int hydra_chain_set_covariates(hydra_chain_t c, const double* X_host, int C);
int hydra_chain_gamma(hydra_chain_t c, double* gamma_out , int32_t* xI_out );
int hydra_chain_iterate(hydra_chain_t c);
int hydra_chain_state(hydra_chain_t c, double* sigmaE, double* mu, double* sigmaG , double* estPi ,
                      int32_t* m0 , int32_t* cass , hgibbs_rng_state* rng);
int hydra_chain_csv_line(hydra_chain_t c, uint32_t iteration, char* buf, size_t len);
const int32_t* hydra_chain_order(hydra_chain_t c);

typedef struct {
    int32_t r[31];
    int32_t f, b;
} hgibbs_grand_state;
void hgibbs_grand_seed(hgibbs_grand_state* st, uint32_t seed);
int32_t hgibbs_grand_next(hgibbs_grand_state* st);

int hgibbs_ars_sample(const double* xinit4, double xl, double xr, double (*logdens)(double, void*), void* data,
                      hgibbs_grand_state* rng, double* xsamp, int* neval);

typedef struct {
    uint64_t launches;
    uint64_t nnz_updates;
    uint64_t ars_draws, ars_evals;
    double device_ms;
    double sums_kernel_ms;
} hgibbs_w_sweep_stats;

int hgibbs_w_init(hgibbs_t h, const int32_t* failure_host);
int hgibbs_w_marker_stats(hgibbs_t h, double* mave, double* sd, double* sum_failure);
int hgibbs_w_set_model(hgibbs_t h, int G, int K, const int32_t* groups_host, const double* mS, int quad_points);
int hgibbs_w_reduce(hgibbs_t h, int kind, int col, double p0, double p1, double p2, double* out);
int hgibbs_w_refresh_vi(hgibbs_t h, double alpha);
int hgibbs_w_get_vi(hgibbs_t h, double* vi_host , double* vi_sum);
int hgibbs_w_marker_sums(hgibbs_t h, uint32_t marker, double beta_old, double alpha, double* vi_sum, double* vi_1, double* vi_2);
int hgibbs_w_sweep(hgibbs_t h, const int32_t* order_host, double alpha, const double* sigmaG, const double* pi, double sumSigmaG,
                   hgibbs_rng_state* rng, hgibbs_grand_state* ars_rng, int32_t* cass_host, double* beta_sqnorm, uint64_t* nnz_updates);
int hgibbs_w_last_sweep_stats(hgibbs_t h, hgibbs_w_sweep_stats* out);
int hgibbs_w_ars_device_probe(hgibbs_t h, const double* dens9, double beta_old, double safe_limit, uint32_t seed, uint32_t ndraws,
                              double* us_per_draw, double* evals_per_draw, double* last_draw);
int hgibbs_w_get_beta(hgibbs_t h, double* beta, int32_t* components);
int hgibbs_w_set_beta(hgibbs_t h, const double* beta, const int32_t* components);

typedef struct hydraw_chain* hydraw_chain_t;
typedef struct {
    uint32_t seed;
    int32_t shuffle;
    int32_t G, K;
    const int32_t* groups;
    const double* mS;
    int32_t quad_points;
} hydraw_model_desc;
int hydraw_chain_create(hgibbs_t dev, const hydraw_model_desc* model, const double* y_host, const int32_t* failure_host, hydraw_chain_t* out);
int hydraw_chain_destroy(hydraw_chain_t c);
int hydraw_chain_set_covariates(hydraw_chain_t c, const double* X_host, int C);
int hydraw_chain_reseed_ars(hydraw_chain_t c, uint32_t seed);
int hydraw_chain_iterate(hydraw_chain_t c);
int hydraw_chain_state(hydraw_chain_t c, double* mu, double* alpha, double* sigmaG, double* pi, int32_t* m0, int32_t* cass,
                       hgibbs_rng_state* rng, hgibbs_grand_state* ars_rng);
int hydraw_chain_gamma(hydraw_chain_t c, double* gamma_out, int32_t* xI_out);
const int32_t* hydraw_chain_order(hydraw_chain_t c);
uint64_t hydraw_chain_last_nnz(hydraw_chain_t c);
int hydraw_chain_csv_line(hydraw_chain_t c, uint32_t iteration, char* buf, size_t len);
typedef struct {
    uint32_t iteration;
    double mu, alpha;
    const double* sigmaG;
    const double* pi;
    const double* beta;
    const int32_t* components;
    const double* eps;
    const int32_t* order;
    const double* gamma;
    const int32_t* xI;
    hgibbs_rng_state rng;
    uint32_t ars_seed;
} hydraw_restart_state;
int hydraw_chain_restore(hydraw_chain_t c, const hydraw_restart_state* st);

typedef struct {
    uint32_t iteration;
    double sigmaE, mu;
    const double* sigmaG;
    const double* estPi;
    const double* beta;
    const int32_t* components;
    const double* eps;
    const int32_t* order;
    const double* gamma;
    const int32_t* xI;
    hgibbs_rng_state rng;
} hydra_restart_state;
int hydra_chain_restore(hydra_chain_t c, const hydra_restart_state* st);
int hydra_rng_to_boost_words(const hgibbs_rng_state* st, uint32_t* words624);
int hydra_rng_from_boost_words(const uint32_t* words624, hgibbs_rng_state* st);
uint64_t hydra_chain_last_nnz(hydra_chain_t c);

#ifdef __cplusplus
}
#endif
#endif
```

Before: 8.789 million.

## Cut host-side per-iteration overhead around the resident Gibbs sweep

Replaces the libstdc++-compatible shuffle with a blocked version that generates Mersenne Twister words in bulk and computes rejection-sampled indices in a vectorisable loop. It moves the order bounds check onto the device, caches occupancy queries and the adaV upload, stages transfers through pinned buffers, and reads the RNG and counts back asynchronously. Beta squared norms now compact non-zero effects on the GPU and copy back only those. The aim is less per-iteration host latency and PCIe traffic. The cost is more code paths, and the fast shuffle must reproduce the original random sequence exactly.

Measured after the change: 9.117 million, median of 6. 1.04x the previous value.

```diff
diff --git a/hydra_amd/capi.py b/hydra_amd/capi.py
--- a/hydra_amd/capi.py
+++ b/hydra_amd/capi.py
@@ -11,7 +11,7 @@
     "hgibbs_marker_stats", "hgibbs_set_residual", "hgibbs_get_residual", "hgibbs_reduce_eps", "hgibbs_add_scalar",
     "hgibbs_update_marker", "hgibbs_dot_marker", "hgibbs_set_covariates", "hgibbs_cov_dot", "hgibbs_cov_update",
     "hydra_chain_set_covariates", "hydra_chain_gamma", "hgibbs_set_components", "hydra_chain_restore",
-    "hydra_rng_to_boost_words", "hydra_rng_from_boost_words", "hgibbs_set_model", "hgibbs_set_beta", "hgibbs_get_beta",
+    "hydra_rng_to_boost_words", "hydra_rng_from_boost_words", "hydra_rng_shuffle", "hgibbs_set_model", "hgibbs_set_beta", "hgibbs_get_beta",
     "hgibbs_beta_sqnorm", "hgibbs_sweep", "hgibbs_set_option", "hgibbs_last_sweep_stats", "hgibbs_stream_ceiling", "hgibbs_debug_times", "hgibbs_resident_trace", "hydra_chain_create",
     "hydra_chain_destroy", "hydra_chain_iterate", "hydra_chain_state", "hydra_chain_csv_line", "hydra_chain_order",
     "hydra_chain_last_nnz", "hgibbs_score", "hgibbs_last_score_ms", "hgibbs_ld", "hgibbs_last_ld_ms",
@@ -127,6 +127,7 @@
     L.hydra_chain_restore.argtypes = [vp, C.POINTER(RestartState)]
     L.hydra_rng_to_boost_words.argtypes = [C.POINTER(RngState), u32p]
     L.hydra_rng_from_boost_words.argtypes = [u32p, C.POINTER(RngState)]
+    L.hydra_rng_shuffle.argtypes = [C.POINTER(RngState), ip, C.c_uint32]
     L.hgibbs_set_model.argtypes = [vp, C.c_int, C.c_int, ip, dp, dp]
     L.hgibbs_set_beta.argtypes = [vp, dp]
     L.hgibbs_get_beta.argtypes = [vp, dp, ip, dp]
@@ -214,6 +215,12 @@
     return a.ctypes.data_as(C.POINTER(C.c_uint64))
 
 
+def rng_shuffle(rng, v):
+    if v.dtype != np.int32 or not v.flags.c_contiguous:
+        raise ValueError("rng_shuffle: a contiguous int32 array is required")
+    check(lib().hydra_rng_shuffle(C.byref(rng), _ip(v), v.size))
+
+
 class Device:
 
     def __init__(self, device_id=0):
diff --git a/hydra_amd/csrc/hg_rng.h b/hydra_amd/csrc/hg_rng.h
--- a/hydra_amd/csrc/hg_rng.h
+++ b/hydra_amd/csrc/hg_rng.h
@@ -238,4 +238,75 @@
     }
 }
 
-}
+inline void mt_twist_bulk(uint32_t* x)
+{
+    for (int i = 0; i < MT_N - MT_M; ++i) x[i] = mt_mix(x[i], x[i + 1], x[i + MT_M]);
+    for (int i = MT_N - MT_M; i < MT_N - 1; ++i) x[i] = mt_mix(x[i], x[i + 1], x[i + MT_M - MT_N]);
+    x[MT_N - 1] = mt_mix(x[MT_N - 1], x[0], x[MT_M - 1]);
+}
+
+#define HG_SHUFFLE_INDICES_BODY                                          \
+    uint32_t bad = 0;                                                    \
+    for (uint32_t k = 0; k < len; ++k) {                                 \
+        const uint32_t ue = i0 + k + 1u;                                 \
+        const uint32_t sc = (uint32_t)(4294967295.0 / (double)ue);       \
+        q[k] = (uint32_t)((double)w[k] / (double)sc);                    \
+        bad |= (uint32_t)(w[k] >= ue * sc);                              \
+    }                                                                    \
+    return bad != 0;
+inline bool shuffle_indices_base(const uint32_t* w, uint32_t i0, uint32_t len, uint32_t* q) { HG_SHUFFLE_INDICES_BODY }
+#if defined(__x86_64__) && !defined(__HIP_DEVICE_COMPILE__)
+__attribute__((target("avx2"))) inline bool shuffle_indices_avx2(const uint32_t* w, uint32_t i0, uint32_t len, uint32_t* q) { HG_SHUFFLE_INDICES_BODY }
+inline bool shuffle_indices(const uint32_t* w, uint32_t i0, uint32_t len, uint32_t* q)
+{
+    static const bool avx2 = __builtin_cpu_supports("avx2");
+    return avx2 ? shuffle_indices_avx2(w, i0, len, q) : shuffle_indices_base(w, i0, len, q);
+}
+#else
+inline bool shuffle_indices(const uint32_t* w, uint32_t i0, uint32_t len, uint32_t* q) { return shuffle_indices_base(w, i0, len, q); }
+#endif
+#undef HG_SHUFFLE_INDICES_BODY
+
+template <class T>
+inline void shuffle_libstdcxx6_fast(T* first, size_t n, Mt& g)
+{
+    constexpr uint32_t BLK = 4096;
+    uint32_t w[BLK], q[BLK];
+    size_t i = 1;
+    while (i < n) {
+        const uint32_t want = (uint32_t)((n - i < (size_t)BLK) ? n - i : (size_t)BLK);
+        uint32_t have = 0;
+        while (have < want) {
+            if (g.idx >= (uint32_t)MT_N) {
+                mt_twist_bulk(g.x);
+                g.idx = 0;
+            }
+            const uint32_t take = ((uint32_t)MT_N - g.idx < want - have) ? (uint32_t)MT_N - g.idx : want - have;
+            const uint32_t* src = g.x + g.idx;
+            for (uint32_t k = 0; k < take; ++k) w[have + k] = mt_temper(src[k]);
+            g.idx += take;
+            have += take;
+        }
+        uint32_t done = 0, used = 0;
+        while (used < have) {
+            const uint32_t len = have - used, i0 = (uint32_t)i + done;
+            uint32_t ok = len;
+            if (shuffle_indices(w + used, i0, len, q + done)) {
+                for (ok = 0; ok < len; ++ok) {
+                    const uint32_t ue = i0 + ok + 1u;
+                    if (w[used + ok] >= ue * (0xffffffffu / ue)) break;
+                }
+            }
+            done += ok;
+            used += ok + (ok < len ? 1u : 0u);
+        }
+        for (uint32_t k = 0; k < done; ++k) {
+            const T t = first[i + k];
+            first[i + k] = first[q[k]];
+            first[q[k]] = t;
+        }
+        i += done;
+    }
+}
+
+}
diff --git a/hydra_amd/csrc/hgibbs.hip b/hydra_amd/csrc/hgibbs.hip
--- a/hydra_amd/csrc/hgibbs.hip
+++ b/hydra_amd/csrc/hgibbs.hip
@@ -117,6 +117,17 @@
     size_t scratch_n = 0;
     double* scratch_host = nullptr;
     double* beta_host = nullptr;
+    uint32_t* bsq_idx_host = nullptr;
+    uint32_t bsq_guess = 1024;
+    int32_t* order_host = nullptr;
+    uint8_t* adaV_host = nullptr;
+    bool adaV_on_device = false;
+    uint32_t* sweep_io_host = nullptr;
+    size_t sweep_io_words = 0;
+    uint32_t* order_bad = nullptr;
+    const void* occ_kern = nullptr;
+    size_t occ_lds = 0;
+    int occ_per_cu = 0;
 
     uint32_t batch = 0;
     uint32_t cols_per_group = 4;
@@ -342,11 +353,15 @@
 
 __global__ void k_gather_meta(const int32_t* __restrict__ order, const double* __restrict__ mave, const double* __restrict__ mstd,
                               const double* __restrict__ beta, const int32_t* __restrict__ groups, const uint8_t* __restrict__ adaV,
-                              const unsigned long long* __restrict__ counts, double* s_mave, double* s_mstd, double* s_bold, int32_t* s_ga, uint32_t M)
+                              const unsigned long long* __restrict__ counts, double* s_mave, double* s_mstd, double* s_bold, int32_t* s_ga, uint32_t M, uint32_t* bad)
 {
     const uint32_t j = blockIdx.x * blockDim.x + threadIdx.x;
     if (j >= M) return;
     const int m = order[j];
+    if ((uint32_t)m >= M) {
+        atomicMin(bad, j);
+        return;
+    }
     s_mave[j] = mave[m];
     s_mstd[j] = mstd[m];
     s_bold[j] = beta[m];
@@ -354,14 +369,14 @@
 }
 
 constexpr uint32_t PRED_CHUNK = 4096;
-__global__ __launch_bounds__(256) void k_pred_count(const double* __restrict__ s_bold, uint32_t M, uint32_t* cnt)
+__global__ __launch_bounds__(256) void k_pred_count(const double* __restrict__ src, uint32_t M, uint32_t* cnt)
 {
     __shared__ uint32_t wsum[4];
     const uint32_t base = blockIdx.x * PRED_CHUNK;
     uint32_t n = 0;
     for (uint32_t i = 0; i < PRED_CHUNK / 256; ++i) {
         const uint32_t j = base + i * 256 + threadIdx.x;
-        n += (uint32_t)__popcll(__ballot(j < M && s_bold[j] != 0.0));
+        n += (uint32_t)__popcll(__ballot(j < M && src[j] != 0.0));
     }
     if ((threadIdx.x & 63) == 0) wsum[threadIdx.x >> 6] = n;
     __syncthreads();
@@ -392,7 +407,7 @@
         run += v;
     }
 }
-__global__ __launch_bounds__(256) void k_pred_scatter(const double* __restrict__ s_bold, uint32_t M, const uint32_t* __restrict__ cnt, uint32_t nchunk, uint32_t* pred)
+__global__ __launch_bounds__(256) void k_pred_scatter(const double* __restrict__ src, uint32_t M, const uint32_t* __restrict__ cnt, uint32_t nchunk, uint32_t* pred, double* payload)
 {
     __shared__ uint32_t wsum[4];
     const uint32_t base = blockIdx.x * PRED_CHUNK;
@@ -400,14 +415,19 @@
     uint32_t run = cnt[blockIdx.x];
     for (uint32_t i = 0; i < PRED_CHUNK / 256; ++i) {
         const uint32_t j = base + i * 256 + threadIdx.x;
-        const bool f = j < M && s_bold[j] != 0.0;
+        const double v = j < M ? src[j] : 0.0;
+        const bool f = v != 0.0;
         const unsigned long long m = __ballot(f);
         __syncthreads();
         if (lane == 0) wsum[wave] = (uint32_t)__popcll(m);
         __syncthreads();
         uint32_t before = 0;
         for (int w = 0; w < wave; ++w) before += wsum[w];
-        if (f) pred[run + before + (uint32_t)__popcll(m & ((1ull << lane) - 1ull))] = j;
+        if (f) {
+            const uint32_t at = run + before + (uint32_t)__popcll(m & ((1ull << lane) - 1ull));
+            pred[at] = j;
+            if (payload) payload[at] = v;
+        }
         run += wsum[0] + wsum[1] + wsum[2] + wsum[3];
     }
     if (blockIdx.x == 0 && threadIdx.x < 16) pred[cnt[nchunk] + threadIdx.x] = 0xffffffffu;
@@ -651,7 +671,7 @@
         if (h->peer_base[r] && h->peer_base[r] != h->mbox) (void)hipIpcCloseMemHandle(h->peer_base[r]);
     if (h->mbox) (void)hipFree(h->mbox);
     void* ptrs[] = {h->bed, h->eps[0], h->eps[1], h->mave, h->mstd, h->counts, h->groups, h->beta, h->comp, h->acum, h->order,
-                    h->adaV, h->covX, h->s_mave, h->s_mstd, h->s_bold, h->s_ga, h->pred, h->pred_cnt, h->dbg, h->cass, h->tables, h->mt, h->zig, h->desc, h->partials, h->totals, h->ticket, h->sums, h->scratch, h->carry, h->ahead_raw, h->apartials, h->aticket, h->res_acc, h->res_msg, h->res_state, h->res_trace};
+                    h->adaV, h->covX, h->s_mave, h->s_mstd, h->s_bold, h->s_ga, h->pred, h->pred_cnt, h->dbg, h->cass, h->tables, h->mt, h->zig, h->desc, h->partials, h->totals, h->ticket, h->sums, h->scratch, h->carry, h->ahead_raw, h->apartials, h->aticket, h->res_acc, h->res_msg, h->res_state, h->res_trace, h->order_bad};
     for (void* p : ptrs)
         if (p) (void)hipFree(p);
     if (h->desc_host) (void)hipHostFree(h->desc_host);
@@ -663,6 +683,10 @@
     if (h->res_progress_host) (void)hipHostFree(h->res_progress_host);
     if (h->aux_stream) (void)hipStreamDestroy(h->aux_stream);
     if (h->beta_host) (void)hipHostFree(h->beta_host);
+    if (h->bsq_idx_host) (void)hipHostFree(h->bsq_idx_host);
+    if (h->order_host) (void)hipHostFree(h->order_host);
+    if (h->adaV_host) (void)hipHostFree(h->adaV_host);
+    if (h->sweep_io_host) (void)hipHostFree(h->sweep_io_host);
     (void)hipEventDestroy(h->ev0);
     (void)hipEventDestroy(h->ev1);
     (void)hipStreamDestroy(h->stream);
@@ -773,6 +797,7 @@
     HIP_TRY(hipMalloc(&h->acum, (size_t)M * sizeof(double)));
     HIP_TRY(hipMalloc(&h->order, (size_t)M * sizeof(int32_t)));
     HIP_TRY(hipMalloc(&h->adaV, (size_t)M));
+    HIP_TRY(hipMalloc(&h->order_bad, sizeof(uint32_t)));
     HIP_TRY(hipMalloc(&h->s_mave, (size_t)M * sizeof(double)));
     HIP_TRY(hipMalloc(&h->s_mstd, (size_t)M * sizeof(double)));
     HIP_TRY(hipMalloc(&h->s_bold, (size_t)M * sizeof(double)));
@@ -1141,11 +1166,34 @@
 {
     if (!h || !h->bed || h->G < 1) return fail("hgibbs_beta_sqnorm: model not set");
     HIP_TRY(hipSetDevice(h->device));
-    if (!h->beta_host) HIP_TRY(hipHostMalloc(&h->beta_host, (size_t)h->M * sizeof(double)));
-    HIP_TRY(hipMemcpyAsync(h->beta_host, h->beta, (size_t)h->M * sizeof(double), hipMemcpyDeviceToHost, h->stream));
+    const uint32_t M = h->M, nchunk = (M + PRED_CHUNK - 1) / PRED_CHUNK;
+    if (!h->beta_host) HIP_TRY(hipHostMalloc(&h->beta_host, (size_t)M * sizeof(double)));
+    if (!h->bsq_idx_host) HIP_TRY(hipHostMalloc(&h->bsq_idx_host, ((size_t)M + 1) * sizeof(uint32_t)));
+    k_pred_count<<<nchunk, 256, 0, h->stream>>>(h->beta, M, h->pred_cnt);
+    k_pred_scan<<<1, 1024, 0, h->stream>>>(h->pred_cnt, nchunk);
+    k_pred_scatter<<<nchunk, 256, 0, h->stream>>>(h->beta, M, h->pred_cnt, nchunk, h->pred, h->s_bold);
+    HIP_TRY(hipGetLastError());
+    const uint32_t got = std::min(M, h->bsq_guess);
+    HIP_TRY(hipMemcpyAsync(h->bsq_idx_host + M, h->pred_cnt + nchunk, sizeof(uint32_t), hipMemcpyDeviceToHost, h->stream));
+    HIP_TRY(hipMemcpyAsync(h->bsq_idx_host, h->pred, (size_t)got * sizeof(uint32_t), hipMemcpyDeviceToHost, h->stream));
+    HIP_TRY(hipMemcpyAsync(h->beta_host, h->s_bold, (size_t)got * sizeof(double), hipMemcpyDeviceToHost, h->stream));
     HIP_TRY(hipStreamSynchronize(h->stream));
+    const uint32_t n = h->bsq_idx_host[M];
+    if (n > M) return fail("hgibbs_beta_sqnorm: list of %u non-zero effects among %u markers", n, M);
+    h->bsq_guess = n + n / 8 + 1024;
     for (int g = 0; g < h->G; ++g) bsq_host[g] = 0.0;
-    for (uint32_t i = 0; i < h->M; ++i) bsq_host[h->groups_host[i]] += h->beta_host[i] * h->beta_host[i];
+    if (n > M / 2) {
+        HIP_TRY(hipMemcpyAsync(h->beta_host, h->beta, (size_t)M * sizeof(double), hipMemcpyDeviceToHost, h->stream));
+        HIP_TRY(hipStreamSynchronize(h->stream));
+        for (uint32_t i = 0; i < M; ++i) bsq_host[h->groups_host[i]] += h->beta_host[i] * h->beta_host[i];
+        return 0;
+    }
+    if (n > got) {
+        HIP_TRY(hipMemcpyAsync(h->bsq_idx_host + got, h->pred + got, (size_t)(n - got) * sizeof(uint32_t), hipMemcpyDeviceToHost, h->stream));
+        HIP_TRY(hipMemcpyAsync(h->beta_host + got, h->s_bold + got, (size_t)(n - got) * sizeof(double), hipMemcpyDeviceToHost, h->stream));
+        HIP_TRY(hipStreamSynchronize(h->stream));
+    }
+    for (uint32_t i = 0; i < n; ++i) bsq_host[h->groups_host[h->bsq_idx_host[i]]] += h->beta_host[i] * h->beta_host[i];
     return 0;
 }
 
@@ -1477,7 +1525,7 @@
         const uint32_t nchunk = (h->M + PRED_CHUNK - 1) / PRED_CHUNK;
         k_pred_count<<<nchunk, 256, 0, h->stream>>>(h->s_bold, h->M, h->pred_cnt);
         k_pred_scan<<<1, 1024, 0, h->stream>>>(h->pred_cnt, nchunk);
-        k_pred_scatter<<<nchunk, 256, 0, h->stream>>>(h->s_bold, h->M, h->pred_cnt, nchunk, h->pred);
+        k_pred_scatter<<<nchunk, 256, 0, h->stream>>>(h->s_bold, h->M, h->pred_cnt, nchunk, h->pred, nullptr);
         HIP_TRY(hipGetLastError());
     }
     p.sweep_id = ++h->res_sweep_id;
@@ -1490,8 +1538,12 @@
     HIP_TRY(hipMemsetAsync(h->res_state, 0, sizeof(ResState), h->stream));
     if (res_opt_in(h, pl)) return 1;
     {
-        int per_cu = 0;
-        HIP_TRY(hipOccupancyMaxActiveBlocksPerMultiprocessor(&per_cu, pl.kern, RS_BLOCK, pl.lds));
+        if (h->occ_kern != (const void*)pl.kern || h->occ_lds != pl.lds) {
+            HIP_TRY(hipOccupancyMaxActiveBlocksPerMultiprocessor(&h->occ_per_cu, pl.kern, RS_BLOCK, pl.lds));
+            h->occ_kern = (const void*)pl.kern;
+            h->occ_lds = pl.lds;
+        }
+        const int per_cu = h->occ_per_cu;
         if (per_cu < 1 || (uint64_t)per_cu * (uint64_t)h->num_cu < (uint64_t)pl.W + 1)
             return fail("hgibbs_sweep: the resident grid of %u workgroups does not fit the device (%d per compute unit, %d units)", pl.W + 1, per_cu, h->num_cu);
     }
@@ -1506,6 +1558,9 @@
     HIP_TRY(hipGetLastError());
     HIP_TRY(hipEventRecord(h->ev1, h->stream));
     HIP_TRY(hipMemcpyAsync(h->res_state_host, h->res_state, sizeof(ResState), hipMemcpyDeviceToHost, h->stream));
+    HIP_TRY(hipMemcpyAsync(h->sweep_io_host, h->mt, MT_N * sizeof(uint32_t), hipMemcpyDeviceToHost, h->stream));
+    HIP_TRY(hipMemcpyAsync(h->sweep_io_host + MT_N, h->cass, (size_t)h->G * h->K * sizeof(int32_t), hipMemcpyDeviceToHost, h->stream));
+    const auto t_launch = std::chrono::steady_clock::now();
     {
         auto t_start = std::chrono::steady_clock::now();
         auto t_probe = t_start;
@@ -1562,8 +1617,8 @@
     float ms = 0.f;
     HIP_TRY(hipEventElapsedTime(&ms, h->ev0, h->ev1));
     rng->idx = st.rng_idx;
-    HIP_TRY(hipMemcpy(rng->x, h->mt, MT_N * sizeof(uint32_t), hipMemcpyDeviceToHost));
-    if (cass_host) HIP_TRY(hipMemcpy(cass_host, h->cass, (size_t)h->G * h->K * sizeof(int32_t), hipMemcpyDeviceToHost));
+    std::memcpy(rng->x, h->sweep_io_host, MT_N * sizeof(uint32_t));
+    if (cass_host) std::memcpy(cass_host, h->sweep_io_host + MT_N, (size_t)h->G * h->K * sizeof(int32_t));
     if (nnz_updates) *nnz_updates = st.nnz;
     hgibbs_sweep_stats& s = h->stats;
     s = hgibbs_sweep_stats{};
@@ -1594,8 +1649,8 @@
     }
     if (timing) {
         auto ms = [](auto a, auto b) { return std::chrono::duration<double, std::milli>(b - a).count(); };
-        std::fprintf(stderr, "[hgibbs] resident sweep: host until the kernel is back %.3f ms (device %.3f), results + drift %.3f\n", ms(t_0, t_kernel), (double)s.device_ms,
-                     ms(t_kernel, std::chrono::steady_clock::now()));
+        std::fprintf(stderr, "[hgibbs] resident sweep: launch preparation %.3f ms, kernel wait %.3f ms (device %.3f), results + drift %.3f\n", ms(t_0, t_launch), ms(t_launch, t_kernel),
+                     (double)s.device_ms, ms(t_kernel, std::chrono::steady_clock::now()));
     }
     return 0;
 }
@@ -1806,8 +1861,6 @@
     if (compute_stats(h)) return 1;
     const int G = h->G, K = h->K;
     const uint32_t M = h->M;
-    for (uint32_t i = 0; i < M; ++i)
-        if (order_host[i] < 0 || (uint32_t)order_host[i] >= M) return fail("hgibbs_sweep: order[%u]=%d outside [0,%u)", i, order_host[i], M);
     if (rng->idx > (uint32_t)MT_N) return fail("hgibbs_sweep: rng idx %u > 624", rng->idx);
 
     const double dNm1 = (double)(h->n_global - 1);
@@ -1828,24 +1881,45 @@
             }
         }
     }
+    const size_t io_words = (size_t)MT_N + (size_t)G * K + 1;
+    if (h->sweep_io_words != io_words) {
+        if (h->sweep_io_host) HIP_TRY(hipHostFree(h->sweep_io_host));
+        h->sweep_io_host = nullptr;
+        HIP_TRY(hipHostMalloc(&h->sweep_io_host, io_words * sizeof(uint32_t)));
+        h->sweep_io_words = io_words;
+    }
+    if (!h->order_host) HIP_TRY(hipHostMalloc(&h->order_host, (size_t)M * sizeof(int32_t)));
+    if (!h->adaV_host) HIP_TRY(hipHostMalloc(&h->adaV_host, (size_t)M));
+    uint32_t* const order_bad_host = h->sweep_io_host + MT_N + (size_t)G * K;
     HIP_TRY(hipMemcpyAsync(h->tables, tab.data(), tab.size() * sizeof(double), hipMemcpyHostToDevice, h->stream));
-    HIP_TRY(hipMemcpyAsync(h->order, order_host, (size_t)M * sizeof(int32_t), hipMemcpyHostToDevice, h->stream));
-    HIP_TRY(hipMemcpyAsync(h->adaV, adaV_host, (size_t)M, hipMemcpyHostToDevice, h->stream));
+    std::memcpy(h->order_host, order_host, (size_t)M * sizeof(int32_t));
+    HIP_TRY(hipMemcpyAsync(h->order, h->order_host, (size_t)M * sizeof(int32_t), hipMemcpyHostToDevice, h->stream));
+    if (!h->adaV_on_device || std::memcmp(h->adaV_host, adaV_host, (size_t)M) != 0) {
+        std::memcpy(h->adaV_host, adaV_host, (size_t)M);
+        HIP_TRY(hipMemcpyAsync(h->adaV, h->adaV_host, (size_t)M, hipMemcpyHostToDevice, h->stream));
+        h->res_all_ada = std::memchr(adaV_host, 0, (size_t)M) == nullptr;
+        h->adaV_on_device = true;
+    }
     HIP_TRY(hipMemcpyAsync(h->mt, rng->x, MT_N * sizeof(uint32_t), hipMemcpyHostToDevice, h->stream));
     HIP_TRY(hipMemsetAsync(h->cass, 0, (size_t)G * K * sizeof(int32_t), h->stream));
     HIP_TRY(hipMemsetAsync(h->ticket, 0, (16 + MAX_GROUPS + 256) * sizeof(uint32_t), h->stream));
     HIP_TRY(hipMemsetAsync(h->aticket, 0, (AHEAD_MAX / 2 + 4) * sizeof(uint32_t), h->stream));
+    HIP_TRY(hipMemsetAsync(h->order_bad, 0xff, sizeof(uint32_t), h->stream));
     k_gather_meta<<<(M + 255) / 256, 256, 0, h->stream>>>(h->order, h->mave, h->mstd, h->beta, h->groups, h->adaV, h->counts, h->s_mave, h->s_mstd,
-                                                       h->s_bold, h->s_ga, M);
+                                                       h->s_bold, h->s_ga, M, h->order_bad);
     HIP_TRY(hipGetLastError());
-    HIP_TRY(hipStreamSynchronize(h->stream));
-    h->res_all_ada = std::memchr(adaV_host, 0, (size_t)M) == nullptr;
-    if (std::getenv("HGIBBS_TIMING"))
-        std::fprintf(stderr, "[hgibbs] sweep preparation (checks, tables, order / adaV upload, metadata gather) %.3f ms\n",
-                     std::chrono::duration<double, std::milli>(std::chrono::steady_clock::now() - t_prep0).count());
+    HIP_TRY(hipMemcpyAsync(order_bad_host, h->order_bad, sizeof(uint32_t), hipMemcpyDeviceToHost, h->stream));
+    const auto t_prep1 = std::chrono::steady_clock::now();
 
     double r0[2];
     if (reduce_eps_all(h, r0)) return 1;
+    if (*order_bad_host != 0xffffffffu) {
+        const uint32_t i = *order_bad_host;
+        return fail("hgibbs_sweep: order[%u]=%d outside [0,%u)", i, order_host[i], M);
+    }
+    if (std::getenv("HGIBBS_TIMING"))
+        std::fprintf(stderr, "[hgibbs] sweep preparation: host work and enqueue (tables, order / adaV staging) %.3f ms, wait for uploads, metadata gather and opening reduction %.3f ms\n",
+                     std::chrono::duration<double, std::milli>(t_prep1 - t_prep0).count(), std::chrono::duration<double, std::milli>(std::chrono::steady_clock::now() - t_prep1).count());
 
     SweepPlan plan = plan_sweep(h);
     {
diff --git a/hydra_amd/csrc/hydra_chain.cpp b/hydra_amd/csrc/hydra_chain.cpp
--- a/hydra_amd/csrc/hydra_chain.cpp
+++ b/hydra_amd/csrc/hydra_chain.cpp
@@ -171,7 +171,7 @@
 
     const auto t_mu = tnow();
     if (c->shuffle) {
-        hg::shuffle_libstdcxx6(c->order.data(), c->order.size(), gen);
+        hg::shuffle_libstdcxx6_fast(c->order.data(), c->order.size(), gen);
     }
     std::fill(c->m0.begin(), c->m0.end(), 0);
     const auto t_shuffle = tnow();
@@ -206,7 +206,7 @@
     }
 
     if (c->C > 0) {
-        hg::shuffle_libstdcxx6(c->xI.data(), c->xI.size(), gen);
+        hg::shuffle_libstdcxx6_fast(c->xI.data(), c->xI.size(), gen);
         const double sigmaF = 1.0;
         const double sigE_sigF = c->sigmaE / sigmaF;
         const double dNm1 = (double)(c->N - 1);
@@ -300,6 +300,16 @@
     return 0;
 }
 
+int hydra_rng_shuffle(hgibbs_rng_state* st, int32_t* v, uint32_t n)
+{
+    if (!st || (n && !v)) return cfail("hydra_rng_shuffle: null argument");
+    if (st->idx > (uint32_t)hg::MT_N) return cfail("hydra_rng_shuffle: rng idx > 624");
+    hg::Mt gen{st->x, st->idx};
+    hg::shuffle_libstdcxx6_fast(v, (size_t)n, gen);
+    st->idx = gen.idx;
+    return 0;
+}
+
 int hydra_chain_gamma(hydra_chain_t c, double* gamma_out, int32_t* xI_out)
 {
     if (!c) return cfail("hydra_chain_gamma: null chain");
diff --git a/hydra_amd/csrc/hydraw_chain.cpp b/hydra_amd/csrc/hydraw_chain.cpp
--- a/hydra_amd/csrc/hydraw_chain.cpp
+++ b/hydra_amd/csrc/hydraw_chain.cpp
@@ -220,7 +220,7 @@
         if (hgibbs_add_scalar(c->dev, -c->mu)) return 1;
     }
     if (c->C > 0) {
-        hg::shuffle_libstdcxx6(c->xI.data(), c->xI.size(), gen);
+        hg::shuffle_libstdcxx6_fast(c->xI.data(), c->xI.size(), gen);
         for (int i = 0; i < c->C; ++i) {
             const int col = (int)c->xI[i];
             const double gamma_old = c->gamma[col];
@@ -246,7 +246,7 @@
     if (hgibbs_w_refresh_vi(c->dev, c->alpha)) return 1;
 
     if (c->shuffle) {
-        hg::shuffle_libstdcxx6(c->order.data(), c->order.size(), gen);
+        hg::shuffle_libstdcxx6_fast(c->order.data(), c->order.size(), gen);
     }
     std::fill(c->m0.begin(), c->m0.end(), 0);
     c->rng.idx = gen.idx;
diff --git a/include/hgibbs.h b/include/hgibbs.h
--- a/include/hgibbs.h
+++ b/include/hgibbs.h
@@ -218,6 +218,7 @@
 int hydra_chain_restore(hydra_chain_t c, const hydra_restart_state* st);
 int hydra_rng_to_boost_words(const hgibbs_rng_state* st, uint32_t* words624);
 int hydra_rng_from_boost_words(const uint32_t* words624, hgibbs_rng_state* st);
+int hydra_rng_shuffle(hgibbs_rng_state* st, int32_t* v, uint32_t n);
 uint64_t hydra_chain_last_nnz(hydra_chain_t c);
 
 #ifdef __cplusplus
```
